# mheinz757/AgglomerationMultigrid1D

Hardware: AMD Instinct MI355X
Metric: fine_level_dof_updates_per_s_per_vcycle (higher is better)
Workload: dtype f64; 1 GPU; config 3/4 hierarchy: V(3,3) cycle, alpha=2/3, DG p=3 n=2^24 -> AggDG pAgg=1 4:1 -> 2:1 -> 2:1 (4 levels), uniform mesh, Neumann/Dirichlet, CDir=1000n (north-star 1-vs-8-GPU size; config 3's own 2^22 in config3_2p22); fine_dofs=67108864, nPre=3, nPost=3, parallelism=single GPU

## Files before the change

### agglomerationmultigrid1d_amd/_lib.py

```python
import ctypes
import os
from ctypes import POINTER, c_char_p, c_double, c_int, c_int32, c_int64, c_void_p

_HERE = os.path.dirname(os.path.abspath(__file__))
LIB_PATH = os.environ.get("AGGMG_HIP_LIB") or os.path.join(_HERE, "libaggmg_hip.so")

AGGMG_OK = 0
ERR_ARGUMENT, ERR_DIMENSION, ERR_SINGULAR, ERR_HIP, ERR_UNSUPPORTED = -1, -2, -3, -4, -5
OP_STIFFNESS, OP_TRANSFER = 0, 1
OPT_SYMMETRIC_PACKING = 1
OPT_COARSE_CHUNK_LOG2 = 2
OPT_DETECT_CHAIN = 3
OPT_PAIR_LEVELS = 4
OPT_MG_CHECKPOINT = 5
OPT_SYMMETRIC_RESIDUAL = 6
OPT_OPERATOR_DICTIONARY = 7
OPT_ELEMENT_THREADS = 8
OPT_PAIR_ELEMENT_THREADS = 9
OPT_REPLAY_PRESMOOTH = 10
OPT_PATCH_MULTI = 11
OPT_CHAIN_MULTI = 12
OPT_ELEMENT_RECORDS_LDS = 13
OPT_PATCH_SCHWARZ_MULTI = 14
PROFILE_NTAGS = 256
KIND_FUSED_DOWN, KIND_FUSED_UP, KIND_SMOOTH, KIND_RESIDUAL, KIND_RESTRICT, KIND_PROLONG, \
    KIND_JACOBI, KIND_BLOCK_APPLY, KIND_COARSE, KIND_FUSED_MID = range(10)
KIND_REPLAY_DOWN, KIND_REPLAY_UP = 10, 11
KIND_NAMES = ["fused_down", "fused_up", "smooth", "residual", "restrict", "prolong", "jacobi",
              "block_apply", "coarse", "fused_mid"]
COARSE_HOST_BANDED, COARSE_DEVICE_CR, COARSE_AUTO, COARSE_EXTERNAL = 0, 1, 2, 3
COARSE_DEVICE_CHAIN = 4
RESTRICT_EXPLICIT, RESTRICT_PRECONDITIONED = 0, 1
RESTRICT_PRECONDITIONED_MAX_ELEMS = 1 << 21
LEVEL_GENERIC, LEVEL_FUSED_BTD, LEVEL_FUSED_CHAIN, LEVEL_COARSEST = 0, 1, 2, 3
MAX_SWEEP_WEIGHTS = 8
FGMRES_MAX_RESTART = 64
RCCL_ID_BYTES = 128
DIST_X0_GHOSTS_VALID, DIST_OVERLAP_NEXT, DIST_GRAPH = 1, 2, 4
ALLGATHER_FN = ctypes.CFUNCTYPE(c_int, c_void_p, c_void_p, c_void_p, c_int64, c_void_p)
SENDRECV_FN = ctypes.CFUNCTYPE(c_int, c_void_p, c_int, POINTER(c_int), POINTER(c_int), POINTER(c_void_p), POINTER(c_int64),
                               c_void_p)
LEVEL_KIND_NAMES = ["generic", "fused_btd", "fused_chain", "coarsest"]


class AggmgError(RuntimeError):
    status = None


class ArgumentError(AggmgError, ValueError):
    status = ERR_ARGUMENT


class DimensionMismatch(AggmgError, ValueError):
    status = ERR_DIMENSION


class SingularException(AggmgError, ArithmeticError):
    status = ERR_SINGULAR


class HipError(AggmgError):
    status = ERR_HIP


class UnsupportedError(AggmgError):
    status = ERR_UNSUPPORTED


_ERR = {c.status: c for c in (ArgumentError, DimensionMismatch, SingularException, HipError,
                              UnsupportedError)}

_P = c_void_p
_PD = POINTER(c_double)
SYMBOLS = {
    "aggmg_create": (c_int, [c_int, POINTER(_P)]),
    "aggmg_destroy": (c_int, [_P]),
    "aggmg_last_error": (c_char_p, [_P]),
    "aggmg_set_stream": (c_int, [_P, _P]),
    "aggmg_reset_stream": (c_int, [_P]),
    "aggmg_synchronize": (c_int, [_P]),
    "aggmg_set_option": (c_int, [_P, c_int, c_int]),
    "aggmg_element_thread_launches": (c_int, [_P, POINTER(c_int64)]),
    "aggmg_pair_element_thread_launches": (c_int, [_P, POINTER(c_int64)]),
    "aggmg_replay_launches": (c_int, [_P, POINTER(c_int64)]),
    "aggmg_element_record_lds_launches": (c_int, [_P, POINTER(c_int64)]),
    "aggmg_element_record_lds_cap": (c_int, [_P, POINTER(c_int), POINTER(c_int)]),
    "aggmg_element_record_pack": (c_int, [c_int, _P, _P, _P, _P, _P, _P, c_int, _P, POINTER(c_int)]),
    "aggmg_patch_multi_launches": (c_int, [_P, POINTER(c_int64)]),
    "aggmg_patch_schwarz_multi_launches": (c_int, [_P, POINTER(c_int64)]),
    "aggmg_chain_multi_launches": (c_int, [_P, POINTER(c_int64)]),
    "aggmg_chain_multi_tile_plan": (c_int, [c_int, c_int, c_int, c_int, c_int, POINTER(c_int), POINTER(c_int), POINTER(c_int),
                                            POINTER(c_int), POINTER(c_int)]),
    "aggmg_dev_alloc": (c_int, [_P, c_int64, POINTER(_P)]),
    "aggmg_dev_free": (c_int, [_P, _P]),
    "aggmg_memcpy_h2d": (c_int, [_P, _P, _P, c_int64]),
    "aggmg_memcpy_d2h": (c_int, [_P, _P, _P, c_int64]),
    "aggmg_csc_upload": (c_int, [_P, c_int64, c_int64, POINTER(c_int64), POINTER(c_int64), _PD,
                                 c_int, c_int, POINTER(_P)]),
    "aggmg_op_free": (c_int, [_P, _P]),
    "aggmg_op_shape": (c_int, [_P, _P, POINTER(c_int64), POINTER(c_int64), POINTER(c_int64)]),
    "aggmg_op_download": (c_int, [_P, _P, c_int, POINTER(c_int32), POINTER(c_int32), _PD]),
    "aggmg_op_release_host": (c_int, [_P, _P]),
    "aggmg_bd_sp_apply": (c_int, [_P, _P, _P, c_int, POINTER(_P)]),
    "aggmg_sp_matmul": (c_int, [_P, _P, _P, c_int, POINTER(_P)]),
    "aggmg_sp_sub": (c_int, [_P, _P, _P, c_int, POINTER(_P)]),
    "aggmg_op_transpose": (c_int, [_P, _P, c_int, POINTER(_P)]),
    "aggmg_op_download_csc": (c_int, [_P, _P, POINTER(c_int32), POINTER(c_int32), _PD]),
    "aggmg_smoother_download_blocks": (c_int, [_P, _P, _PD]),
    "aggmg_debug_device_memory": (c_int, [POINTER(c_int64), POINTER(c_int64)]),
    "aggmg_debug_scan_counts": (c_int, [_P, POINTER(c_int32), c_int64, POINTER(c_int64)]),
    "aggmg_debug_stream_copy": (c_int, [_P, _P, _P, c_int64, c_int, c_int, POINTER(c_double)]),
    "aggmg_blockjacobi_setup": (c_int, [_P, _P, c_int64, c_int64, POINTER(c_int64), c_int, c_int,
                                        POINTER(_P)]),
    "aggmg_blockdiag_setup": (c_int, [_P, c_int64, c_int64, _PD, c_int, POINTER(_P)]),
    "aggmg_patch_schwarz_setup": (c_int, [_P, _P, c_int64, c_int64, c_int, c_int, POINTER(_P)]),
    "aggmg_smoother_patch_info": (c_int, [_P, _P, POINTER(c_int), POINTER(c_int), POINTER(c_int)]),
    "aggmg_smoother_patch_dictionary": (c_int, [_P, _P, POINTER(c_int)]),
    "aggmg_patch_tile_plan": (c_int, [c_int, c_int, POINTER(c_int), POINTER(c_int), POINTER(c_int)]),
    "aggmg_patch_gs_setup": (c_int, [_P, _P, c_int64, c_int64, POINTER(_P)]),
    "aggmg_smoother_patch_kind": (c_int, [_P, _P, POINTER(c_int)]),
    "aggmg_patch_gs_tile_plan": (c_int, [c_int, c_int, POINTER(c_int), POINTER(c_int), POINTER(c_int), POINTER(c_int)]),
    "aggmg_patch_gs_multi_tile_plan": (c_int, [c_int, c_int, c_int, POINTER(c_int), POINTER(c_int), POINTER(c_int),
                                               POINTER(c_int)]),
    "aggmg_patch_schwarz_multi_tile_plan": (c_int, [c_int, c_int, c_int, POINTER(c_int), POINTER(c_int), POINTER(c_int),
                                                    POINTER(c_int)]),
    "aggmg_jacobi_setup": (c_int, [_P, _P, POINTER(_P)]),
    "aggmg_jacobi_setup_elements": (c_int, [_P, _P, c_int64, c_int64, POINTER(c_int64), c_int, POINTER(_P)]),
    "aggmg_smoother_free": (c_int, [_P, _P]),
    "aggmg_smoother_apply": (c_int, [_P, _P, _PD, c_int64, c_int64, c_double, _PD]),
    "aggmg_smoother_is_structured": (c_int, [_P, _P, POINTER(c_int)]),
    "aggmg_smooth": (c_int, [_P, _P, _P, _PD, _PD, c_double, c_int]),
    "aggmg_residual": (c_int, [_P, _P, _PD, _PD, _PD]),
    "aggmg_restrict": (c_int, [_P, _P, _PD, _PD]),
    "aggmg_prolong_add": (c_int, [_P, _P, _PD, _PD]),
    "aggmg_smooth_dev": (c_int, [_P, _P, _P, _P, _P, c_double, c_int, _P]),
    "aggmg_smooth_weighted_dev": (c_int, [_P, _P, _P, _P, _P, _PD, c_int, _P]),
    "aggmg_smooth_multi_dev": (c_int, [_P, _P, _P, _P, _P, c_int64, c_int64, _PD, c_int, c_int, _P]),
    "aggmg_residual_dev": (c_int, [_P, _P, _P, _P, _P]),
    "aggmg_restrict_dev": (c_int, [_P, _P, _P, _P]),
    "aggmg_prolong_add_dev": (c_int, [_P, _P, _P, _P]),
    "aggmg_hier_create": (c_int, [_P, c_int, POINTER(_P), POINTER(_P), POINTER(_P), c_int,
                                  POINTER(_P)]),
    "aggmg_hier_free": (c_int, [_P, _P]),
    "aggmg_vcycle": (c_int, [_P, _P, _PD, _PD, c_int, c_int, c_double, _PD]),
    "aggmg_vcycle_dev": (c_int, [_P, _P, _P, _P, c_int, c_int, c_double, _P]),
    "aggmg_vcycle_multi_dev": (c_int, [_P, _P, _P, _P, c_int64, c_int64, c_int, c_int, c_double, _P]),
    "aggmg_hier_coarse_solve_multi_dev": (c_int, [_P, _P, _P, c_int64, c_int64, _P]),
    "aggmg_hier_multi_info": (c_int, [_P, _P, c_int64, c_int, c_int, POINTER(c_int), POINTER(c_int)]),
    "aggmg_vcycles_dev": (c_int, [_P, _P, _P, _P, c_int, c_int, c_int, c_double, _P]),
    "aggmg_hier_set_restriction": (c_int, [_P, _P, c_int]),
    "aggmg_hier_get_restriction": (c_int, [_P, _P, POINTER(c_int)]),
    "aggmg_vcycle_down_dev": (c_int, [_P, _P, _P, _P, c_int, c_double]),
    "aggmg_vcycle_up_dev": (c_int, [_P, _P, _P, c_int, c_double, _P]),
    "aggmg_vcycle_up_coarse_dev": (c_int, [_P, _P, _P, c_int, c_double, c_int, c_int64, c_int64]),
    "aggmg_vcycle_up_split_dev": (c_int, [_P, _P, _P, c_int, c_double, _P, c_int64, c_int64, c_int]),
    "aggmg_vcycle_up_split_ok": (c_int, [_P, _P, c_int, POINTER(c_int)]),
    "aggmg_hier_coarse_buffers": (c_int, [_P, _P, POINTER(_P), POINTER(_P), POINTER(c_int64)]),
    "aggmg_coarse_plan": (c_int, [_P, _P, POINTER(c_int), POINTER(c_int64), POINTER(c_int), POINTER(c_int64)]),
    "aggmg_coarse_chunk_forward_dev": (c_int, [_P, _P, _P, c_int64, c_int64, _P, _P]),
    "aggmg_coarse_boundary_solve_dev": (c_int, [_P, _P, _P, _P, _P]),
    "aggmg_coarse_chunk_backward_dev": (c_int, [_P, _P, _P, c_int64, c_int64, _P, _P]),
    "aggmg_hier_level_kind": (c_int, [_P, _P, c_int, POINTER(c_int)]),
    "aggmg_host_register": (c_int, [_P, _P, c_int64]),
    "aggmg_host_unregister": (c_int, [_P, _P]),
    "aggmg_host_alloc": (c_int, [_P, c_int64, POINTER(_P)]),
    "aggmg_host_free": (c_int, [_P, _P]),
    "aggmg_hier_level_paired": (c_int, [_P, _P, c_int, c_int, POINTER(c_int)]),
    "aggmg_hier_level_paired_up": (c_int, [_P, _P, c_int, c_int, POINTER(c_int)]),
    "aggmg_hier_level_sym_residual": (c_int, [_P, _P, c_int, POINTER(c_int)]),
    "aggmg_hier_level_dictionary": (c_int, [_P, _P, c_int, POINTER(c_int)]),
# ... 91 lines not shown
```

### agglomerationmultigrid1d_amd/api.py

```python
import ctypes

import numpy as np
import scipy.sparse as sp
import scipy.sparse.linalg as spla

from . import _lib
from ._lib import (ArgumentError, DimensionMismatch, check)

_PD = ctypes.POINTER(ctypes.c_double)
_PI64 = ctypes.POINTER(ctypes.c_int64)


def _f64(x):
    return np.ascontiguousarray(x, dtype=np.float64)


def _pd(a):
    return a.ctypes.data_as(_PD)


def device_memory():
    n, b = ctypes.c_int64(), ctypes.c_int64()
    check(_lib.load().aggmg_debug_device_memory(ctypes.byref(n), ctypes.byref(b)), None)
    return n.value, b.value


class Context:

    def __init__(self, device=0):
        self.lib = _lib.load()
        h = ctypes.c_void_p()
        check(self.lib.aggmg_create(int(device), ctypes.byref(h)), None)
        self.handle = h
        self.device = int(device)

    def close(self):
        if getattr(self, "handle", None):
            self.lib.aggmg_destroy(self.handle)
            self.handle = None

    def __del__(self):
        try:
            self.close()
        except Exception:
            pass

    def check(self, status):
        check(status, self.handle)

    def synchronize(self):
        self.check(self.lib.aggmg_synchronize(self.handle))

    def set_option(self, option, value):
        self.check(self.lib.aggmg_set_option(self.handle, int(option), int(value)))
        self.__dict__.setdefault("_options", {})[int(option)] = int(value)

    def element_thread_launches(self):
        n = ctypes.c_int64(0)
        self.check(self.lib.aggmg_element_thread_launches(self.handle, ctypes.byref(n)))
        return int(n.value)

    def pair_element_thread_launches(self):
        n = ctypes.c_int64(0)
        self.check(self.lib.aggmg_pair_element_thread_launches(self.handle, ctypes.byref(n)))
        return int(n.value)

    def replay_launches(self):
        n = ctypes.c_int64(0)
        self.check(self.lib.aggmg_replay_launches(self.handle, ctypes.byref(n)))
        return int(n.value)

    def element_record_lds_launches(self):
        n = ctypes.c_int64(0)
        self.check(self.lib.aggmg_element_record_lds_launches(self.handle, ctypes.byref(n)))
        return int(n.value)

    def element_record_lds_cap(self):
        c, m = ctypes.c_int(0), ctypes.c_int(0)
        self.check(self.lib.aggmg_element_record_lds_cap(self.handle, ctypes.byref(c), ctypes.byref(m)))
        return int(c.value), int(m.value)

    def patch_multi_launches(self):
        n = ctypes.c_int64(0)
        self.check(self.lib.aggmg_patch_multi_launches(self.handle, ctypes.byref(n)))
        return int(n.value)

    def patch_schwarz_multi_launches(self):
        n = ctypes.c_int64(0)
        self.check(self.lib.aggmg_patch_schwarz_multi_launches(self.handle, ctypes.byref(n)))
        return int(n.value)

    def chain_multi_launches(self):
        n = ctypes.c_int64(0)
        self.check(self.lib.aggmg_chain_multi_launches(self.handle, ctypes.byref(n)))
        return int(n.value)

    def option(self, option, default):
        return self.__dict__.get("_options", {}).get(int(option), default)

    def set_stream(self, hip_stream):
        self.check(self.lib.aggmg_set_stream(self.handle, ctypes.c_void_p(hip_stream or None)))

    def reset_stream(self):
        self.check(self.lib.aggmg_reset_stream(self.handle))

    def alloc(self, n):
        return DeviceVector(self, n)

    def to_device(self, x):
        x = _f64(x)
        v = DeviceVector(self, x.size)
        v.upload(x)
        return v

    def pin(self, x):
        x = np.asarray(x)
        if x.dtype != np.float64 or not x.flags["C_CONTIGUOUS"]:
            raise ArgumentError("Context.pin: a C-contiguous float64 array")
        self.check(self.lib.aggmg_host_register(self.handle, ctypes.c_void_p(x.ctypes.data), x.nbytes))
        self._pinned = getattr(self, "_pinned", {})
        self._pinned[x.ctypes.data] = x
        return x

    def unpin(self, x):
        self.check(self.lib.aggmg_host_unregister(self.handle, ctypes.c_void_p(x.ctypes.data)))
        getattr(self, "_pinned", {}).pop(x.ctypes.data, None)

    def pinned_empty(self, n):
        p = ctypes.c_void_p()
        self.check(self.lib.aggmg_host_alloc(self.handle, int(n) * 8, ctypes.byref(p)))
        buf = (ctypes.c_double * int(n)).from_address(p.value)
        return np.frombuffer(buf, dtype=np.float64, count=int(n))

    def dot_cols(self, X, Y, n=None, ncols=None, ld=None):
        n, ncols, ld = _cols_shape("dot_cols", X, n, ncols, ld)
        if isinstance(Y, DeviceMatrix) and Y.shape != (n, ncols):
            raise DimensionMismatch("dot_cols: X and Y differ in shape")
        out = np.zeros(max(1, int(ncols)))
        self.check(self.lib.aggmg_dot_cols_dev(self.handle, _ptr(X), _ptr(Y), int(n), int(ncols), int(ld), _pd(out)))
        return out

    def norm2_cols(self, X, n=None, ncols=None, ld=None):
        n, ncols, ld = _cols_shape("norm2_cols", X, n, ncols, ld)
        out = np.zeros(max(1, int(ncols)))
        self.check(self.lib.aggmg_norm2_cols_dev(self.handle, _ptr(X), int(n), int(ncols), int(ld), _pd(out)))
        return out

    def multi_dot(self, V, w, n=None, nvec=None, ld=None):
        n, nvec, ld = _cols_shape("multi_dot", V, n, nvec, ld)
        if isinstance(w, DeviceVector) and w.n < n:
            raise DimensionMismatch("multi_dot: w is shorter than the columns of V")
        out = np.zeros(max(1, int(nvec)))
        self.check(self.lib.aggmg_multi_dot_dev(self.handle, _ptr(V), int(n), int(nvec), int(ld), _ptr(w), _pd(out)))
        return out

    def multi_axpy_norm(self, V, coef, w, n=None, nvec=None, ld=None, norm=True):
        n, nvec, ld = _cols_shape("multi_axpy_norm", V, n, nvec, ld)
        if isinstance(w, DeviceVector) and w.n < n:
            raise DimensionMismatch("multi_axpy_norm: w is shorter than the columns of V")
        c = _f64(coef).ravel()
        if c.size != nvec:
            raise DimensionMismatch("multi_axpy_norm: one coefficient per column of V")
# ... 937 lines not shown

    def can_split_up(self, nPost=3):
        ok = ctypes.c_int(0)
        c = self.ctx
        c.check(c.lib.aggmg_vcycle_up_split_ok(c.handle, self.handle, int(nPost), ctypes.byref(ok)))
        return bool(ok.value)

    def set_restriction(self, mode):
        c = self.ctx
        c.check(c.lib.aggmg_hier_set_restriction(c.handle, self.handle, int(mode)))

    def set_sweep_weights(self, level, pre, post=None):
        pre = np.ascontiguousarray(np.atleast_1d(np.asarray(pre, dtype=np.float64)))
        post = pre[::-1].copy() if post is None else np.ascontiguousarray(np.atleast_1d(np.asarray(post, dtype=np.float64)))
        if pre.ndim != 1 or post.ndim != 1:
            raise ArgumentError("set_sweep_weights: pre and post are sequences of numbers")
        c = self.ctx
        c.check(c.lib.aggmg_hier_set_sweep_weights(c.handle, self.handle, int(level), _pd(pre), pre.size, _pd(post), post.size))

    def clear_sweep_weights(self, level=None):
        c = self.ctx
        for k in (range(self.nlevels - 1) if level is None else [int(level)]):
            c.check(c.lib.aggmg_hier_set_sweep_weights(c.handle, self.handle, k, None, 0, None, 0))

    def sweep_weights(self, level):
        pre, post = np.zeros(_lib.MAX_SWEEP_WEIGHTS), np.zeros(_lib.MAX_SWEEP_WEIGHTS)
        npre, npost = ctypes.c_int(0), ctypes.c_int(0)
        c = self.ctx
        c.check(c.lib.aggmg_hier_get_sweep_weights(c.handle, self.handle, int(level), _pd(pre), ctypes.byref(npre), _pd(post),
                                                   ctypes.byref(npost)))
        if npre.value + npost.value == 0:
            return None
        return pre[:npre.value].copy(), post[:npost.value].copy()

    def estimate_lambda_max(self, level, iters=40, v0=None):
        c = self.ctx
        keep = None
        if v0 is not None and isinstance(v0, (np.ndarray, list, tuple)):
            keep = c.to_device(v0)
            v0 = keep
        lam = ctypes.c_double(0.0)
        try:
            c.check(c.lib.aggmg_hier_estimate_lambda_max(c.handle, self.handle, int(level), None if v0 is None else _ptr(v0),
                                                         int(iters), ctypes.byref(lam)))
        finally:
            if keep is not None:
                keep.free()
        return lam.value

    def set_chebyshev_smoothing(self, levels=(0,), degree=3, ratio=10.0, iters=40):
        out = {}
        for k in levels:
            lam = self.estimate_lambda_max(k, iters=iters)
            self.set_sweep_weights(k, chebyshev_weights(lam, degree=degree, ratio=ratio))
            out[int(k)] = lam
        return out

    def get_restriction(self):
        v = ctypes.c_int(0)
        self.ctx.check(self.ctx.lib.aggmg_hier_get_restriction(self.ctx.handle, self.handle, ctypes.byref(v)))
        return v.value

    def coarse_buffers(self):
        r, s_, n = ctypes.c_void_p(), ctypes.c_void_p(), ctypes.c_int64(0)
        self.ctx.check(self.ctx.lib.aggmg_hier_coarse_buffers(self.ctx.handle, self.handle, ctypes.byref(r),
                                                              ctypes.byref(s_), ctypes.byref(n)))
        return r.value, s_.value, n.value

    def coarse_info(self):
        a, b, c = ctypes.c_int(0), ctypes.c_int(0), ctypes.c_double(0.0)
        self.ctx.check(self.ctx.lib.aggmg_hier_coarse_info(self.ctx.handle, self.handle, ctypes.byref(a),
                                                           ctypes.byref(b), ctypes.byref(c)))
        e = ctypes.c_double(0.0)
        self.ctx.check(self.ctx.lib.aggmg_hier_coarse_probe(self.ctx.handle, self.handle, ctypes.byref(e)))
        k, nb = ctypes.c_int(0), ctypes.c_int64(0)
        self.ctx.check(self.ctx.lib.aggmg_hier_coarse_tail(self.ctx.handle, self.handle, ctypes.byref(k), ctypes.byref(nb)))
        on, cm, cb = ctypes.c_int(0), ctypes.c_int(0), ctypes.c_int64(0)
        self.ctx.check(self.ctx.lib.aggmg_hier_coarse_chain(self.ctx.handle, self.handle, ctypes.byref(on), ctypes.byref(cm),
                                                            ctypes.byref(cb)))
        return dict(on_device=bool(a.value), block_size=b.value, cond_est=c.value, probe_backward_error=e.value,
                    tail=("none", "cyclic reduction", "parallel cyclic reduction")[k.value], tail_blocks=nb.value,
                    order="element chain" if on.value else "operator")

    def last_coarse_ms(self):
        ms = ctypes.c_double(0.0)
        self.ctx.check(self.ctx.lib.aggmg_hier_last_coarse_ms(self.ctx.handle, self.handle, ctypes.byref(ms)))
        return ms.value

    def free(self):
        if getattr(self, "handle", None) and self.ctx.handle:
            self.ctx.lib.aggmg_hier_free(self.ctx.handle, self.handle)
        self.handle = None

    def __del__(self):
        try:
            self.free()
        except Exception:
            pass


def multigrid_v_cycle(H, x0, b, nPre=3, nPost=3, alpha=2.0 / 3.0, out=None):
    if not isinstance(nPre, (int, np.integer)) or not isinstance(nPost, (int, np.integer)):
        raise TypeError("nPre / nPost must be integers (nPre::Integer, src/solvers.jl:20)")
    if isinstance(b, DeviceMatrix) or (not isinstance(b, DeviceVector) and np.ndim(b) == 2):
        return _multigrid_v_cycle_multi(H, x0, b, int(nPre), int(nPost), float(alpha))
    if x0 is None and isinstance(b, DeviceVector):
        out = H.ctx.alloc(b.n)
        H.vcycle_dev(None, b, out, int(nPre), int(nPost), float(alpha))
        return out
    if isinstance(x0, DeviceVector) and isinstance(b, DeviceVector):
        N = H._ops[0].shape[0]
        if x0.n != N or b.n != N:
            raise DimensionMismatch("multigrid_v_cycle: x0 / b do not match the fine operator")
        out = H.ctx.alloc(N)
        H.vcycle_dev(x0, b, out, int(nPre), int(nPost), float(alpha))
        return out
    x0 = None if x0 is None else _f64(x0)
    b = _f64(b)
    N = H._ops[0].shape[0]
    if (x0 is not None and x0.shape != (N,)) or b.shape != (N,):
        raise DimensionMismatch("multigrid_v_cycle: x0 / b do not match the fine operator")
    if out is None:
        out = np.empty(N)
    elif not (isinstance(out, np.ndarray) and out.dtype == np.float64 and out.shape == (N,) and out.flags["C_CONTIGUOUS"]):
        raise DimensionMismatch("multigrid_v_cycle: out must be a contiguous float64 array of the fine operator's size")
    elif (x0 is not None and np.shares_memory(out, x0)) or np.shares_memory(out, b):
        raise ArgumentError("multigrid_v_cycle: out must not alias x0 or b (they are not modified)")
    c = H.ctx
    c.check(c.lib.aggmg_vcycle(c.handle, H.handle, None if x0 is None else _pd(x0), _pd(b), int(nPre), int(nPost), float(alpha),
                               _pd(out)))
    return out


def _multigrid_v_cycle_multi(H, X0, B, nPre, nPost, alpha):
    N = H._ops[0].shape[0]
    c = H.ctx
    if isinstance(B, DeviceMatrix):
        if X0 is not None and not isinstance(X0, DeviceMatrix):
            raise ArgumentError("multigrid_v_cycle: X0 must be a DeviceMatrix (or None) when B is one")
        K = B.k
        if B.n != N or (X0 is not None and X0.shape != B.shape):
            raise DimensionMismatch("multigrid_v_cycle: X0 / B do not match (N, K) of the fine operator")
        X = DeviceMatrix(c, N, K)
        H.vcycle_multi_dev(X0, B, X, K, N, nPre, nPost, alpha)
        return X
    if isinstance(X0, (DeviceVector, DeviceMatrix)):
        raise ArgumentError("multigrid_v_cycle: X0 is on the device but B is a host array")
    B = np.asarray(B, dtype=np.float64)
    if B.ndim != 2 or B.shape[0] != N:
        raise DimensionMismatch(f"multigrid_v_cycle: B has shape {B.shape}, expected ({N}, K)")
    K = B.shape[1]
    if K < 1:
        raise ArgumentError("multigrid_v_cycle: B has no columns")
    if X0 is not None:
        X0 = np.asarray(X0, dtype=np.float64)
        if X0.shape != B.shape:
            raise DimensionMismatch(f"multigrid_v_cycle: X0 has shape {X0.shape}, B {B.shape}")
    dB = DeviceMatrix(c, N, K)
    dB.upload(B)
    dX0 = None
    if X0 is not None:
        dX0 = DeviceMatrix(c, N, K)
        dX0.upload(X0)
    dX = DeviceMatrix(c, N, K)
    H.vcycle_multi_dev(dX0, dB, dX, K, N, nPre, nPost, alpha)
    return dX.download()
# ... 374 lines not shown
```

### agglomerationmultigrid1d_amd/csrc/aggmg_hip.hip

```cpp
#include "internal.hpp"
#include "multi_kernels.hpp"
#include "multi_solve_kernels.hpp"
#include "pair_kernels.hpp"
#include "patch_kernels.hpp"
#include "patch_multi_kernels.hpp"
#include "patch_schwarz_multi_kernels.hpp"
#include "elem_kernels.hpp"
#include "pair_elem_kernels.hpp"
#include "krylov_kernels.hpp"
#include "host_gmres.hpp"
#include "host_gmres_cols.hpp"

extern "C" const char* aggmg_version(void) { return "aggmg_hip 0.1 gfx950 fp64"; }

extern "C" int aggmg_debug_device_memory(int64_t* live_allocations, int64_t* live_bytes) {
  if (live_allocations) *live_allocations = DevMemLive::allocations.load();
  if (live_bytes) *live_bytes = DevMemLive::bytes.load();
  return AGGMG_OK;
}

extern "C" int aggmg_create(int device_id, aggmg_ctx** out) {
  if (!out) return fail(nullptr, AGGMG_ERR_ARGUMENT, "aggmg_create: out is NULL");
  *out = nullptr;
  int ndev = 0;
// ... 70 lines not shown
    }
  return fail(ctx, AGGMG_ERR_ARGUMENT, "aggmg_host_unregister: not a range registered with this context");
}

extern "C" int aggmg_host_alloc(aggmg_ctx* ctx, int64_t nbytes, void** out) {
  if (!ctx || !out) return AGGMG_ERR_ARGUMENT;
  if (nbytes < 0) return fail(ctx, AGGMG_ERR_ARGUMENT, "aggmg_host_alloc: negative size");
  HIPCHK(hipSetDevice(ctx->device));
  void* p = nullptr;
  HIPCHK(hipHostMalloc(&p, (size_t)std::max<int64_t>(nbytes, 8), hipHostMallocDefault));
  ctx->pinned.push_back({static_cast<char*>(p), (size_t)std::max<int64_t>(nbytes, 8), true});
  *out = p;
  return AGGMG_OK;
}

extern "C" int aggmg_host_free(aggmg_ctx* ctx, void* ptr) {
  if (!ctx) return AGGMG_ERR_ARGUMENT;
  if (!ptr) return AGGMG_OK;
  for (size_t i = 0; i < ctx->pinned.size(); ++i)
    if (ctx->pinned[i].base == static_cast<char*>(ptr) && ctx->pinned[i].owned) {
      HIPCHK(hipStreamSynchronize(ctx->stream));
      HIPCHK(hipHostFree(ptr));
      ctx->pinned.erase(ctx->pinned.begin() + (long)i);
      return AGGMG_OK;
    }
  return fail(ctx, AGGMG_ERR_ARGUMENT, "aggmg_host_free: not an allocation of this context");
}

extern "C" const char* aggmg_last_error(aggmg_ctx* ctx) {
  return ctx ? ctx->err.c_str() : g_create_error.c_str();
}

extern "C" int aggmg_set_stream(aggmg_ctx* ctx, void* hip_stream) {
  if (!ctx) return AGGMG_ERR_ARGUMENT;
  ctx->stream = (hipStream_t)hip_stream;
  return AGGMG_OK;
}

extern "C" int aggmg_reset_stream(aggmg_ctx* ctx) {
  if (!ctx) return AGGMG_ERR_ARGUMENT;
  ctx->stream = ctx->own_stream;
  return AGGMG_OK;
}

extern "C" int aggmg_set_option(aggmg_ctx* ctx, int option, int value) {
  if (!ctx) return AGGMG_ERR_ARGUMENT;
  switch (option) {
    case AGGMG_OPT_SYMMETRIC_PACKING:
      ctx->sym_packing = value != 0;
      return AGGMG_OK;
    case AGGMG_OPT_COARSE_CHUNK_LOG2:
      if (value < 1 || value > kCrMaxStageLevels)
        return fail(ctx, AGGMG_ERR_ARGUMENT, "aggmg_set_option: AGGMG_OPT_COARSE_CHUNK_LOG2 takes 1 .. 12");
      ctx->cr_max_q = value;
      return AGGMG_OK;
    case AGGMG_OPT_DETECT_CHAIN:
      ctx->detect_chain = value != 0;
      return AGGMG_OK;
    case AGGMG_OPT_PAIR_LEVELS:
      ctx->pair_levels = value != 0;
      return AGGMG_OK;
    case AGGMG_OPT_MG_CHECKPOINT:
      ctx->mg_checkpoint = value != 0;
      return AGGMG_OK;
    case AGGMG_OPT_SYMMETRIC_RESIDUAL:
      ctx->sym_residual = value != 0;
      return AGGMG_OK;
    case AGGMG_OPT_OPERATOR_DICTIONARY:
      ctx->op_dict = value != 0;
      return AGGMG_OK;
    case AGGMG_OPT_ELEMENT_THREADS:
      ctx->elem_threads = value != 0;
      return AGGMG_OK;
    case AGGMG_OPT_PAIR_ELEMENT_THREADS:
      ctx->pair_elem_threads = value != 0;
      return AGGMG_OK;
    case AGGMG_OPT_REPLAY_PRESMOOTH:
      ctx->replay_presmooth = value != 0;
      return AGGMG_OK;
    case AGGMG_OPT_ELEMENT_RECORDS_LDS:
      if (value < 0 || value > kElemRecMaxClasses)
        return fail(ctx, AGGMG_ERR_ARGUMENT, "aggmg_set_option: AGGMG_OPT_ELEMENT_RECORDS_LDS takes 0 .. " + std::to_string(kElemRecMaxClasses));
      ctx->elem_rec_cap = value;
      return AGGMG_OK;
    case AGGMG_OPT_PATCH_MULTI:
      ctx->patch_multi = value != 0;
      return AGGMG_OK;
    case AGGMG_OPT_CHAIN_MULTI:
      ctx->chain_multi = value != 0;
      return AGGMG_OK;
    case AGGMG_OPT_PATCH_SCHWARZ_MULTI:
      ctx->patch_schwarz_multi = value != 0;
      return AGGMG_OK;
  }
  return fail(ctx, AGGMG_ERR_ARGUMENT, "aggmg_set_option: unknown option");
}

extern "C" int aggmg_synchronize(aggmg_ctx* ctx) {
  if (!ctx) return AGGMG_ERR_ARGUMENT;
  HIPCHK(hipStreamSynchronize(ctx->stream));
  return AGGMG_OK;
}

extern "C" int aggmg_dev_alloc(aggmg_ctx* ctx, int64_t nbytes, void** out) {
  if (!ctx || !out || nbytes < 0) return fail(ctx, AGGMG_ERR_ARGUMENT, "aggmg_dev_alloc: bad argument");
  HIPCHK(hipSetDevice(ctx->device));
  HIPCHK(hipMalloc(out, (size_t)std::max<int64_t>(nbytes, 8)));
  HIPCHK(hipMemsetAsync(*out, 0, (size_t)std::max<int64_t>(nbytes, 8), ctx->stream));
  return AGGMG_OK;
}

extern "C" int aggmg_dev_free(aggmg_ctx* ctx, void* ptr) {
  if (!ctx) return AGGMG_ERR_ARGUMENT;
  if (ptr) {
    HIPCHK(hipStreamSynchronize(ctx->stream));
    HIPCHK(hipFree(ptr));
  }
  return AGGMG_OK;
}

extern "C" int aggmg_memcpy_h2d(aggmg_ctx* ctx, void* dst, const void* src, int64_t nbytes) {
  if (!ctx) return AGGMG_ERR_ARGUMENT;
  HIPCHK(hipMemcpyAsync(dst, src, (size_t)nbytes, hipMemcpyHostToDevice, ctx->stream));
  HIPCHK(hipStreamSynchronize(ctx->stream));
  return AGGMG_OK;
}

extern "C" int aggmg_memcpy_d2h(aggmg_ctx* ctx, void* dst, const void* src, int64_t nbytes) {
  if (!ctx) return AGGMG_ERR_ARGUMENT;
  HIPCHK(hipMemcpyAsync(dst, src, (size_t)nbytes, hipMemcpyDeviceToHost, ctx->stream));
  HIPCHK(hipStreamSynchronize(ctx->stream));
  return AGGMG_OK;
}

extern "C" int aggmg_profile_enable(aggmg_ctx* ctx, int on) {
  if (!ctx) return AGGMG_ERR_ARGUMENT;
  ctx->profiling = on < 0 ? 0 : (on > 2 ? 1 : on);
  return AGGMG_OK;
}

extern "C" int aggmg_profile_collect(aggmg_ctx* ctx, double* total_ms, int64_t* counts) {
  if (!ctx || !total_ms || !counts) return fail(ctx, AGGMG_ERR_ARGUMENT, "aggmg_profile_collect: NULL");
  for (int t = 0; t < AGGMG_PROFILE_NTAGS; ++t) {
    total_ms[t] = 0.0;
    counts[t] = 0;
  }
  HIPCHK(hipStreamSynchronize(ctx->stream));
  for (auto& pe : ctx->prof) {
    float ms = 0.f;
    HIPCHK(hipEventElapsedTime(&ms, pe.a, pe.b));
    total_ms[pe.tag] += ms;
    counts[pe.tag] += 1;
    ctx->ev_pool.push_back(pe.a);
    ctx->ev_pool.push_back(pe.b);
  }
  ctx->prof.clear();
  return AGGMG_OK;
}

extern "C" int aggmg_csc_upload(aggmg_ctx* ctx, int64_t m, int64_t n, const int64_t* colptr,
                                const int64_t* rowval, const double* nzval, int one_based, int kind,
                                aggmg_op** out) {
  if (!ctx || !out || !colptr) return fail(ctx, AGGMG_ERR_ARGUMENT, "aggmg_csc_upload: NULL argument");
  *out = nullptr;
  if (m < 0 || n < 0) return fail(ctx, AGGMG_ERR_ARGUMENT, "aggmg_csc_upload: negative dimension");
  const int64_t base = one_based ? 1 : 0;
// ... 1400 lines not shown
  const CrDev& cr = h->cr;
  std::vector<CrMultiStage> ws;
  CrMultiStage wt;
  cr_multi_layout(cr.st, cr.tail, cr.m, h->crw_cols, &ws, &wt);
  double* const w = h->crw;
  auto at = [&](int64_t stride, int64_t off) -> double* { return stride ? w + off : nullptr; };
  CrRun run;
  run.kc = kc;
  run.st.reserve(ws.size());
  for (const CrMultiStage& W : ws) {
    double* const part = w + W.part_off;
    run.st.push_back({part, part + W.part / 3, part + 2 * (W.part / 3), at(W.stack, W.stack_off), at(W.mid, W.mid_off), W.part,
                      W.stack, W.mid});
  }
  run.tail.mid = at(wt.mid, wt.mid_off);
  run.tail.cs_mid = wt.mid;
  return run;
}

enum CrKind { kCrForward = 0, kCrTail = 1, kCrBackward = 2 };
static CrStageArgs cr_make_args(const CrDev& cr, const CrStagePlan& S, const CrRunStage& R, CrKind kind) {
  CrStageArgs A;
  std::memset(&A, 0, sizeof(A));
#ifdef AGGMG_CR_TRACE
  A.trace = g_cr_trace;
  A.trace_kind = kind;
#endif
  A.q = S.q;
  for (int l = 0; l < S.q; ++l) A.lv[l] = cr.lv[S.l0 + l];
  A.nsteps = S.nsteps;
  for (int s = 0; s <= kCrMaxSteps; ++s) {
    A.step_a[s] = S.step_a[s];
    A.lds_off[s] = S.lds_off[s];
    A.lds_xoff[s] = S.lds_xoff[s];
  }
  A.lds_total = S.lds_total;
  A.n_out = S.n_out;
  A.stack = R.stack;
  A.stack_stride = S.stack_stride;
  A.mid = R.mid;
  for (int s = 0; s <= kCrMaxSteps; ++s) A.mid_off[s] = S.mid_off[s];
  A.tail = kind == kCrTail ? 1 : 0;
  A.lu_last = cr.lu_last;
  A.perm_last = cr.perm_last;
  A.cs_o = A.cs_xq = R.cs_part;
  A.cs_stack = R.cs_stack;
  A.cs_mid = R.cs_mid;
  return A;
}

template <int M>
static void cr_launch_tail(aggmg_ctx* ctx, CrDev& cr, const CrStageArgs& T, size_t tail_lds, const double* d, const double* db,
                           double* x, int kc = 1) {
  if constexpr (M <= 2) {
    if (cr.pcr.valid) {
      PcrArgs P;
      std::memset(&P, 0, sizeof(P));
      P.mult = cr.pcr.mult;
      P.lu = cr.pcr.lu;
      P.perm = cr.pcr.perm;
      P.n = cr.pcr.n;
      P.L = cr.pcr.L;
      P.dstride = T.dstride;
      P.cs_d = T.cs_d;
      P.cs_x = T.cs_x;
#ifdef AGGMG_CR_TRACE
      P.trace = g_cr_trace;
#endif
      const unsigned threads = (unsigned)((cr.pcr.n + 63) / 64 * 64);
      const size_t lds = (size_t)2 * (cr.pcr.n + 1) * M * sizeof(double);
      if (cr.pcr.pre) {
        P.lv0 = cr.lv[cr.tail.l0];
        P.n_full = (int)cr.tail.n_in;
        hipLaunchKernelGGL((cr_pcr_tail_kernel<M, true>), dim3(1, kc), dim3(threads), lds, ctx->stream, P, d, db, x);
      } else {
        hipLaunchKernelGGL((cr_pcr_tail_kernel<M, false>), dim3(1, kc), dim3(threads), lds, ctx->stream, P, d, db, x);
      }
      return;
    }
  }
  hipLaunchKernelGGL((cr_tail_kernel<M>), dim3(1, kc), dim3(kCrThreads), tail_lds, ctx->stream, T, d, db, x);
}

template <int M, bool FUSE_TAIL = false>
static void cr_launch_forward(aggmg_ctx* ctx, const CrStageArgs& A, unsigned grid, int kc, const double* d, const double* db,
                              double* partR, double* partL, const CrStageArgs& T, size_t tail_lds = 0, double* xt = nullptr,
                              unsigned int* ticket = nullptr) {
  hipLaunchKernelGGL((cr_stage_forward_kernel<M, FUSE_TAIL>), dim3(grid, kc), dim3(cr_stage_threads()),
                     std::max((size_t)A.lds_total * sizeof(double), tail_lds), ctx->stream, A, d, db, partR, partL, T, xt, ticket);
}
template <int M>
static void cr_launch_backward(aggmg_ctx* ctx, const CrStageArgs& A, unsigned grid, int kc, const double* d, const double* db,
                               const double* xq, double* x) {
  hipLaunchKernelGGL((cr_stage_backward_kernel<M>), dim3(grid, kc), dim3(cr_stage_threads()), (size_t)A.lds_total * sizeof(double),
                     ctx->stream, A, d, db, xq, x);
}

template <int M>
static int cr_walk(aggmg_ctx* ctx, CrDev& cr, const CrRun& run, int s0, const double* d, const double* db, double* x,
                   int64_t cs_in, int64_t cs_out, int dstride) {
  const int ns = (int)cr.st.size(), kc = run.kc;
  CrStageArgs T = cr_make_args(cr, cr.tail, run.tail, kCrTail);
  const size_t tail_lds = (size_t)cr.tail.lds_total * sizeof(double);
  if (s0 >= ns) {
    T.dstride = dstride;
    T.cs_d = cs_in;
    T.cs_x = cs_out;
    cr_launch_tail<M>(ctx, cr, T, tail_lds, d, db, x, kc);
    HIPCHK(hipGetLastError());
    return AGGMG_OK;
  }
  struct Io {
    const double *d, *db;
    double* x;
    int64_t cs_d, cs_x;
    int dstride;
  };
  auto io = [&](int s) -> Io {
    if (s == s0) return {d, db, x, cs_in, cs_out, dstride};
    const CrRunStage& P = run.st[s - 1];
    return {P.partR, P.partL, P.xq, P.cs_part, P.cs_part, 0};
  };
  const bool fuse_tail = kc == 1 && cr_fuse_tail();
  for (int s = s0; s < ns; ++s) {
    const CrRunStage& R = run.st[s];
    const Io in = io(s);
    CrStageArgs A = cr_make_args(cr, cr.st[s], R, kCrForward);
    A.cs_d = in.cs_d;
    A.dstride = in.dstride;
    const unsigned grid = (unsigned)std::max<int64_t>(A.n_out, 1);
    if (s == ns - 1 && fuse_tail) {
      cr_launch_forward<M, true>(ctx, A, grid, kc, in.d, in.db, R.partR, R.partL, T, tail_lds, R.xq, cr.ticket);
    } else {
      cr_launch_forward<M>(ctx, A, grid, kc, in.d, in.db, R.partR, R.partL, T);
      if (s == ns - 1) {
        T.cs_d = T.cs_x = R.cs_part;
        cr_launch_tail<M>(ctx, cr, T, tail_lds, R.partR, R.partL, R.xq, kc);
      }
    }
  }
  for (int s = ns - 1; s >= s0; --s) {
    const Io in = io(s);
    CrStageArgs A = cr_make_args(cr, cr.st[s], run.st[s], kCrBackward);
    A.cs_d = in.cs_d;
    A.cs_x = in.cs_x;
    A.dstride = in.dstride;
    cr_launch_backward<M>(ctx, A, (unsigned)std::max<int64_t>(A.n_out, 1), kc, in.d, in.db, run.st[s].xq, in.x);
  }
  HIPCHK(hipGetLastError());
  return AGGMG_OK;
}

template <int M>
static int cr_chunks(aggmg_ctx* ctx, CrDev& cr, bool backward, const double* d_owned, int64_t blk_lo, int64_t blk_hi,
                     double* partR, double* partL, const double* xq, double* x_owned, int ostride) {
  const CrStage& S = cr.st[0];
  CrStageArgs A = cr_make_args(cr, S, cr_run_stage(S), backward ? kCrBackward : kCrForward);
  A.ostride = ostride;
  A.c0 = blk_lo >> S.q;
  const int64_t c1 = (blk_hi + ((int64_t)1 << S.q) - 1) >> S.q;
  const unsigned grid = (unsigned)std::max<int64_t>(c1 - A.c0, 0);
  if (!grid) return AGGMG_OK;
  const double* d0 = d_owned - blk_lo * M;
  if (backward) {
    cr_launch_backward<M>(ctx, A, grid, 1, d0, nullptr, xq, x_owned - blk_lo * M);
  } else {
    CrStageArgs T;
    std::memset(&T, 0, sizeof(T));
    cr_launch_forward<M>(ctx, A, grid, 1, d0, nullptr, partR, partL, T);
  }
  HIPCHK(hipGetLastError());
  return AGGMG_OK;
}

template <class F>
static int cr_with_m(aggmg_ctx* ctx, const CrDev& cr, F&& f) {
  int rc = AGGMG_OK;
  if (!with_block_size<cr_form>(cr.m, [&](auto m) { rc = f(m); }))
    return fail(ctx, AGGMG_ERR_UNSUPPORTED, "cyclic reduction block size not instantiated");
  return rc;
}

static int cr_phase(aggmg_ctx* ctx, CrDev& cr, int phase, const double* d_owned, int64_t blk_lo, int64_t blk_hi,
                    double* partR, double* partL, const double* xq, double* x_owned, int pstride = 0) {
  ProfScope ps(ctx, AGGMG_KIND_COARSE, 0);
  return cr_with_m(ctx, cr, [&](auto m) {
    constexpr int M = decltype(m)::value;
    if (phase == 1) return cr_walk<M>(ctx, cr, cr.run, 1, partR, partL, const_cast<double*>(xq), 0, 0, pstride);
    return cr_chunks<M>(ctx, cr, phase == 2, d_owned, blk_lo, blk_hi, partR, partL, xq, x_owned, pstride);
  });
}

static int cr_multi_workspace(aggmg_ctx* ctx, aggmg_hier* h, int64_t cols, bool staging) {
  const CrDev& cr = h->cr;
  if (h->crw_cols < cols) {
    HIPCHK(hipStreamSynchronize(ctx->stream));
    h->crw_cols = 0;
    std::vector<CrMultiStage> st;
    CrMultiStage tail;
    CHECK(h->crw.alloc(ctx, cr_multi_layout(cr.st, cr.tail, cr.m, cols, &st, &tail), true));
    h->crw_cols = cols;
  }
  if (staging && h->crw_stage_cols < cols) {
    HIPCHK(hipStreamSynchronize(ctx->stream));
    h->crw_stage_cols = 0;
    CHECK(h->crw_stage.alloc(ctx, 2 * cols * cr_even(cr.n0 * cr.m), true));
    h->crw_stage_cols = cols;
  }
  return AGGMG_OK;
}

static dim3 cr_cols_grid(int64_t n, int kc) { return dim3((unsigned)((n + kCrThreads - 1) / kCrThreads), kc); }
static void cr_chain_gather(aggmg_ctx* ctx, const CgtDev& g, int64_t n, int kc, const double* B, int64_t ldb, double* d0, int64_t sp) {
  hipLaunchKernelGGL(cr_chain_gather_kernel<kCrThreads>, cr_cols_grid(n, kc), dim3(kCrThreads), 0, ctx->stream, B, ldb,
                     (const int32_t*)g.perm, d0, sp, n);
}
static void cr_chain_scatter(aggmg_ctx* ctx, const CgtDev& g, int kc, const double* x0, int64_t sp, double* X, int64_t ldx) {
  hipLaunchKernelGGL(cr_chain_scatter_kernel<kCrThreads>, cr_cols_grid(g.N, kc), dim3(kCrThreads), 0, ctx->stream, x0, sp,
                     (const int32_t*)g.inv, X, ldx, g.N);
}
static void cr_cols_copy(aggmg_ctx* ctx, int64_t n, int kc, const double* src, int64_t ld_src, double* dst, int64_t ld_dst) {
  hipLaunchKernelGGL(cr_cols_copy_kernel<kCrThreads>, cr_cols_grid(n, kc), dim3(kCrThreads), 0, ctx->stream, src, ld_src, dst, ld_dst, n);
}

template <int M>
static int cr_solve_cols(aggmg_ctx* ctx, aggmg_hier* h, const double* B, int64_t ldb, double* X, int64_t ldx, int kc) {
  CrDev& cr = h->cr;
  const int64_t Npad = cr.n0 * M;
  const bool aligned = kc == 1 || ((((uintptr_t)B | (uintptr_t)X) & 15) == 0 && ldb % 2 == 0 && ldx % 2 == 0);
  const bool overlap = kc == 1 ? B == X : B < X + ((kc - 1) * ldx + cr.N) && X < B + ((kc - 1) * ldb + cr.N);
  const bool direct = !cr.chain && Npad == cr.N && aligned && !overlap;
  if (kc > 1) {
    CHECK(cr_multi_workspace(ctx, h, kc, !direct));
  } else if (!direct && !cr.d0) {
    for (DevArray<double>* p : {&cr.d0, &cr.x0}) CHECK(p->alloc(ctx, Npad));
  }
  const double* d = B;
  double* x = X;
  int64_t cs_in = ldb, cs_out = ldx;
  if (!direct) {
    const int64_t sp = kc == 1 ? 0 : cr_even(Npad);
    double* d0 = kc == 1 ? cr.d0.get() : h->crw_stage.get();
    x = kc == 1 ? cr.x0.get() : h->crw_stage + h->crw_stage_cols * sp;
    if (cr.chain) {
      cr_chain_gather(ctx, *cr.chain, Npad, kc, B, ldb, d0, sp);
    } else if (kc == 1) {
      if (Npad > cr.N) HIPCHK(hipMemsetAsync(d0 + cr.N, 0, (Npad - cr.N) * sizeof(double), ctx->stream));
      HIPCHK(hipMemcpyAsync(d0, B, cr.N * sizeof(double), hipMemcpyDeviceToDevice, ctx->stream));
    } else {
      cr_cols_copy(ctx, cr.N, kc, B, ldb, d0, sp);
    }
    d = d0;
// ... 387 lines not shown
                          int64_t gh_hi = 0) {
  const int n = (int)h->lv.size();
  Level& a = h->lv[k];
  Level& b = h->lv[k + 1];
  Level& c = h->lv[k + 2];
  PairArgs p = pair_args(h, k, nPost);
  const SweepWeights wa = a.damp_post(alpha).launch(nPost), wb = b.damp_post(alpha).launch(nPost);
  PairTilePlan plan = pair_up_plan(nPost, p.ab.rho, kPairTEA, kPairTEB);
  if (plan.own <= 0) return fail(ctx, AGGMG_ERR_UNSUPPORTED, "internal: paired tile too small");
  p.hb = plan.hb;
  p.own = plan.own;
  p.te_a = plan.te_a;
  p.te_b = plan.te_b;
  p.rhs_a = a.rhs;
  p.rhs_b_in = b.rhs;
  p.ua_in = a.u[0];
  p.ub_in = b.u[0];
  p.uc = (k + 2 == n - 1) ? c.u[0] : c.u[1];
  p.u_a = dst;
  p.ub_out = nullptr;
  int64_t ntiles = (p.A.ne + plan.own - 1) / plan.own;
  if (part != 0) {
    pair_up_split(&plan, nPost, p.ab.rho, p.bc.rho, p.A.ne, p.bc.nec, gh_lo, gh_hi);
    if (part == 1) {
      p.tile_split = (int)plan.tA;
      p.tile_skip = plan.all - plan.tA - plan.tB;
      ntiles = plan.tA + plan.tB;
    } else {
      p.tile_skip = plan.tA;
      ntiles = plan.all - plan.tA - plan.tB;
    }
  }
  if (ntiles == 0) return AGGMG_OK;
  const size_t lds = ((size_t)2 * (kPairTEA + 2) * kPairM + (size_t)kPairTEB * 2) * sizeof(double);
  PairDict d;
  const bool dict = part == 0 && pair_dictionary(p, d, a, b);
  PairElemDict ed;
  const bool elem = dict && pair_element_threads(ctx, p, ed, a, b, pair_up_plan(nPost, p.ab.rho, kPairElemTEA, kPairElemTEB));
  ProfScope ps(ctx, AGGMG_KIND_FUSED_UP, k);
  if (elem) {
    ntiles = (p.A.ne + p.own - 1) / p.own;
    hipLaunchKernelGGL((btd_pair_up_elem_kernel<kPairElemThreads>), dim3((unsigned)ntiles), dim3(kPairElemThreads),
                       pair_elem_lds_bytes(ed.nca, ed.ncb), ctx->stream, p, wa, wb, ed);
    ++ctx->pair_elem_launches;
  } else if (dict)
    hipLaunchKernelGGL((btd_pair_up_dict_kernel<kPairM, kPairNSA, kPairNSB, kThreads>), dim3((unsigned)ntiles), dim3(kThreads),
                       lds, ctx->stream, p, wa, wb, d);
  else
    hipLaunchKernelGGL((btd_pair_up_kernel<kPairM, kPairNSA, kPairNSB, kThreads>), dim3((unsigned)ntiles), dim3(kThreads), lds,
                       ctx->stream, p, wa, wb);
  HIPCHK(hipGetLastError());
  return AGGMG_OK;
}

extern "C" int aggmg_hier_level_paired(aggmg_ctx* ctx, const aggmg_hier* h, int level, int nsweeps, int* paired) {
  if (!ctx || !h || !paired) return fail(ctx, AGGMG_ERR_ARGUMENT, "aggmg_hier_level_paired: NULL argument");
  *paired = pair_ok(ctx, h, level, nsweeps, false) ? 1 : 0;
  return AGGMG_OK;
}

extern "C" int aggmg_hier_level_paired_up(aggmg_ctx* ctx, const aggmg_hier* h, int level, int nsweeps, int* paired) {
  if (!ctx || !h || !paired) return fail(ctx, AGGMG_ERR_ARGUMENT, "aggmg_hier_level_paired_up: NULL argument");
  *paired = pair_ok(ctx, h, level, nsweeps, true) ? 1 : 0;
  return AGGMG_OK;
}

extern "C" int aggmg_hier_level_sym_residual(aggmg_ctx* ctx, const aggmg_hier* h, int level, int* on) {
  if (!ctx || !h || !on) return fail(ctx, AGGMG_ERR_ARGUMENT, "aggmg_hier_level_sym_residual: NULL argument");
  if (level < 0 || level >= (int)h->lv.size()) return fail(ctx, AGGMG_ERR_ARGUMENT, "aggmg_hier_level_sym_residual: level out of range");
  const Level& l = h->lv[level];
  *on = (l.S && l.S->btd && l.S->btd->dup) ? 1 : 0;
  return AGGMG_OK;
}

extern "C" int aggmg_element_thread_launches(aggmg_ctx* ctx, int64_t* count) {
  if (!ctx || !count) return fail(ctx, AGGMG_ERR_ARGUMENT, "aggmg_element_thread_launches: NULL argument");
  *count = ctx->elem_launches;
  return AGGMG_OK;
}

extern "C" int aggmg_pair_element_thread_launches(aggmg_ctx* ctx, int64_t* count) {
  if (!ctx || !count) return fail(ctx, AGGMG_ERR_ARGUMENT, "aggmg_pair_element_thread_launches: NULL argument");
  *count = ctx->pair_elem_launches;
  return AGGMG_OK;
}

extern "C" int aggmg_element_record_lds_launches(aggmg_ctx* ctx, int64_t* count) {
  if (!ctx || !count) return fail(ctx, AGGMG_ERR_ARGUMENT, "aggmg_element_record_lds_launches: NULL argument");
  *count = ctx->elem_rec_launches;
  return AGGMG_OK;
}

extern "C" int aggmg_element_record_lds_cap(aggmg_ctx* ctx, int* cap, int* max_cap) {
  if (!ctx || !cap) return fail(ctx, AGGMG_ERR_ARGUMENT, "aggmg_element_record_lds_cap: NULL argument");
  *cap = ctx->elem_rec_cap;
  if (max_cap) *max_cap = kElemRecMaxClasses;
  return AGGMG_OK;
}

extern "C" int aggmg_element_record_pack(int nclasses, const double* bsym, const double* qrow, const double* qmir, const double* dup,
                                         const uint32_t* corr, const double* lf, int lf_unit, double* rec, int* words) {
  if (words) *words = kElemRecWords;
  if (nclasses < 0 || (nclasses > 0 && (!bsym || !qrow || !qmir || !lf || !rec || !dup != !corr))) return AGGMG_ERR_ARGUMENT;
  elem_record_pack(nclasses, bsym, qrow, qmir, dup, corr, lf, lf_unit != 0, rec);
  return AGGMG_OK;
}

extern "C" int aggmg_replay_launches(aggmg_ctx* ctx, int64_t* count) {
  if (!ctx || !count) return fail(ctx, AGGMG_ERR_ARGUMENT, "aggmg_replay_launches: NULL argument");
  *count = ctx->replay_launches;
  return AGGMG_OK;
}

extern "C" int aggmg_hier_level_dictionary(aggmg_ctx* ctx, const aggmg_hier* h, int level, int* nclasses) {
  if (!ctx || !h || !nclasses) return fail(ctx, AGGMG_ERR_ARGUMENT, "aggmg_hier_level_dictionary: NULL argument");
  if (level < 0 || level >= (int)h->lv.size()) return fail(ctx, AGGMG_ERR_ARGUMENT, "aggmg_hier_level_dictionary: level out of range");
  const Level& l = h->lv[level];
  *nclasses = l.dict ? l.dict->nclasses : (l.cdict ? l.cdict->nclasses : (l.pdict ? l.pdict->nclasses : 0));
  return AGGMG_OK;
}

extern "C" int aggmg_hier_set_sweep_weights(aggmg_ctx* ctx, aggmg_hier* h, int level, const double* pre, int npre,
                                            const double* post, int npost) {
  if (!ctx) return AGGMG_ERR_ARGUMENT;
  if (!h) return fail(ctx, AGGMG_ERR_ARGUMENT, "aggmg_hier_set_sweep_weights: NULL argument");
  if (level < 0 || level >= (int)h->lv.size() - 1)
    return fail(ctx, AGGMG_ERR_ARGUMENT, "aggmg_hier_set_sweep_weights: level out of range (the coarsest level is solved, not smoothed)");
  if (npre < 0 || npost < 0 || npre > AGGMG_MAX_SWEEP_WEIGHTS || npost > AGGMG_MAX_SWEEP_WEIGHTS)
    return fail(ctx, AGGMG_ERR_ARGUMENT, "aggmg_hier_set_sweep_weights: between 0 and AGGMG_MAX_SWEEP_WEIGHTS weights per half");
  if ((npre > 0 && !pre) || (npost > 0 && !post)) return fail(ctx, AGGMG_ERR_ARGUMENT, "aggmg_hier_set_sweep_weights: NULL argument");
  for (int i = 0; i < npre; ++i)
    if (!std::isfinite(pre[i])) return fail(ctx, AGGMG_ERR_ARGUMENT, "aggmg_hier_set_sweep_weights: weight is not finite");
  for (int i = 0; i < npost; ++i)
    if (!std::isfinite(post[i])) return fail(ctx, AGGMG_ERR_ARGUMENT, "aggmg_hier_set_sweep_weights: weight is not finite");
  Level& l = h->lv[level];
  l.scheduled = npre + npost > 0;
  l.w_pre.assign(pre, pre + npre);
  l.w_post.assign(post, post + npost);
  l.w_mid = l.w_post;
  l.w_mid.insert(l.w_mid.end(), l.w_pre.begin(), l.w_pre.end());
  l.w_replay = l.w_pre;
  l.w_replay.insert(l.w_replay.end(), l.w_post.begin(), l.w_post.end());
  return AGGMG_OK;
}

extern "C" int aggmg_hier_get_sweep_weights(aggmg_ctx* ctx, const aggmg_hier* h, int level, double* pre, int* npre,
                                            double* post, int* npost) {
  if (!ctx) return AGGMG_ERR_ARGUMENT;
  if (!h || !pre || !npre || !post || !npost) return fail(ctx, AGGMG_ERR_ARGUMENT, "aggmg_hier_get_sweep_weights: NULL argument");
  if (level < 0 || level >= (int)h->lv.size() - 1)
    return fail(ctx, AGGMG_ERR_ARGUMENT, "aggmg_hier_get_sweep_weights: level out of range");
  const Level& l = h->lv[level];
  *npre = (int)l.w_pre.size();
  *npost = (int)l.w_post.size();
  std::copy(l.w_pre.begin(), l.w_pre.end(), pre);
  std::copy(l.w_post.begin(), l.w_post.end(), post);
  return AGGMG_OK;
}

static int schedule_check(aggmg_ctx* ctx, const aggmg_hier* h, int nPre, int nPost, int k_first = 0) {
  for (int k = k_first; k < (int)h->lv.size() - 1; ++k) {
    const Level& l = h->lv[k];
    if (!l.scheduled) continue;
    if ((nPre >= 0 && nPre != (int)l.w_pre.size()) || (nPost >= 0 && nPost != (int)l.w_post.size()))
      return fail(ctx, AGGMG_ERR_ARGUMENT, "level " + std::to_string(k) + " has a sweep-weight schedule of " +
                  std::to_string(l.w_pre.size()) + " pre- and " + std::to_string(l.w_post.size()) +
// ... 2530 lines not shown
```

### agglomerationmultigrid1d_amd/csrc/cr_kernels.hpp

```cpp
#pragma once
#include <hip/hip_runtime.h>
#include <stdint.h>

#include "host_plan.hpp"

namespace aggmg {

constexpr int kCrThreads = 256;
#ifndef CR_WAVES_ATTR
#define CR_WAVES_ATTR
#endif

struct CrLevel {
  const double* fe;
  const double* fo;
  const double* lu;
  const int32_t* perm;
  int64_t n, n_even, n_odd;
};

template <int M>
struct CrRadix {
  static constexpr int Q = M <= 4 ? 3 : 2;
};
// ... 319 lines not shown
        double& r = v[(CrOff<QS, I>::blocks + 2 * jj + 1) * M + e];
        double& g = mid[(CrMidOff<QS, I>::blocks + jj) * M + e];
        if constexpr (STORE) g = r; else r = g;
      }
    cr_mid_move<M, QS, I + 1, STORE>(mid, v);
  }
}

template <int M, int QS>
struct CrSubFactorsB {
  double fo[CrOddOff<QS, QS>::rows][2 * M * M];
  double lu[CrOddOff<QS, QS>::rows][M * M];
  int32_t perm[CrOddOff<QS, QS>::rows][M];
};

template <int M, int QS, int I>
__device__ __forceinline__ void cr_pre_load_b(const CrLevel* lv, int64_t b, CrSubFactorsB<M, QS>& F) {
  if constexpr (I < QS) {
    const CrLevel& L = lv[I];
    constexpr int NB1 = 1 << (QS - I - 1);
    const int64_t tlo1 = b << (QS - I - 1);
#pragma unroll
    for (int jj = 0; jj < NB1; ++jj) {
      int64_t idx = tlo1 + jj;
      if (idx > L.n_odd - 1) idx = L.n_odd - 1;
      const double* lu = L.lu + idx * (M * M);
      const int32_t* pm = L.perm + idx * M;
      constexpr int o = CrOddOff<QS, I>::rows;
      cr_load_pair<M>(L.fo + idx * (2 * M * M), F.fo[o + jj]);
      if constexpr (M == 2) {
        const double2 t0 = reinterpret_cast<const double2*>(lu)[0], t1 = reinterpret_cast<const double2*>(lu)[1];
        const int2 pp = *reinterpret_cast<const int2*>(pm);
        F.lu[o + jj][0] = t0.x, F.lu[o + jj][1] = t0.y, F.lu[o + jj][2] = t1.x, F.lu[o + jj][3] = t1.y;
        F.perm[o + jj][0] = pp.x, F.perm[o + jj][1] = pp.y;
      } else {
#pragma unroll
        for (int k = 0; k < M * M; ++k) F.lu[o + jj][k] = lu[k];
#pragma unroll
        for (int k = 0; k < M; ++k) F.perm[o + jj][k] = pm[k];
      }
    }
    cr_pre_load_b<M, QS, I + 1>(lv, b, F);
  }
}

template <int M, int QS, int I>
__device__ __forceinline__ void cr_loc_bwd_pre(const CrLevel* lv, const CrSubFactorsB<M, QS>& F, int64_t b, double* v) {
  if constexpr (I >= 0) {
    const CrLevel& L = lv[I];
    constexpr int NB1 = 1 << (QS - I - 1);
    const int64_t tlo = b << (QS - I);
    double* d = v + CrOff<QS, I>::blocks * M;
    const double* xn = v + CrOff<QS, I + 1>::blocks * M;
#pragma unroll
    for (int jj = 0; jj < NB1; ++jj) {
      const int64_t r = tlo + 2 * jj + 1;
      const double* ac = F.fo[CrOddOff<QS, I>::rows + jj];
      double rhs[M], x[M];
      const bool has_next = r + 1 < L.n;
      double xr[M];
#pragma unroll
      for (int k = 0; k < M; ++k) xr[k] = has_next ? xn[(jj + 1) * M + k] : 0.0;
#pragma unroll
      for (int i = 0; i < M; ++i) {
        double s = d[(2 * jj + 1) * M + i];
#pragma unroll
        for (int k = 0; k < M; ++k) s -= ac[i * M + k] * xn[jj * M + k];
#pragma unroll
        for (int k = 0; k < M; ++k) s -= ac[M * M + i * M + k] * xr[k];
        rhs[i] = s;
      }
      cr_lu_solve_reg<M>(F.lu[CrOddOff<QS, I>::rows + jj], F.perm[CrOddOff<QS, I>::rows + jj], rhs, x);
#pragma unroll
      for (int e = 0; e < M; ++e) d[(2 * jj + 1) * M + e] = x[e];
    }
#pragma unroll
    for (int jj = 0; jj <= NB1; ++jj)
#pragma unroll
      for (int e = 0; e < M; ++e) d[(2 * jj) * M + e] = xn[jj * M + e];
    cr_loc_bwd_pre<M, QS, I - 1>(lv, F, b, v);
  }
}

struct CrStepGeom {
  int a, a1;
  int64_t lo_in, lo_out;
  int64_t n_in, n_out;
  int nb;
};

template <int QS>
__device__ __forceinline__ CrStepGeom cr_step_geom(const CrStageArgs& A, int s, int64_t c, bool wg_shared) {
  CrStepGeom g;
  g.a = A.step_a[s];
  g.a1 = g.a + QS;
  g.lo_in = c << (A.q - g.a);
  g.lo_out = c << (A.q - g.a1);
  g.n_in = cr_level_n(A, g.a);
  g.n_out = cr_level_n(A, g.a1);
  int64_t hi_out = (c + 1) << (A.q - g.a1);
  if (hi_out > g.n_out - 1) hi_out = g.n_out - 1;
  g.nb = (int)(hi_out - g.lo_out + 1) - (wg_shared ? 1 : 0);
  return g;
}

template <int M, int QS>
__device__ __forceinline__ void cr_loc_load(const CrStageArgs& A, int s, const CrStepGeom& g, int64_t b,
                                            const double* __restrict__ d0, const double* __restrict__ d0b,
                                            const double* sh, double* v, int64_t& thi, bool& tshared,
                                            bool carry_rb) {
  constexpr int NB = 1 << QS;
  const int64_t tlo = b << QS;
  thi = (b + 1) << QS;
  tshared = thi <= g.n_in - 1;
  if (!tshared) thi = g.n_in - 1;
  if (s == 0) {
    const int ds = A.dstride ? A.dstride : M;
    if (tshared && ds == M) {
      const double2* p = reinterpret_cast<const double2*>(d0 + tlo * M);
      if (d0b) {
        const double2* pb = reinterpret_cast<const double2*>(d0b + tlo * M);
#pragma unroll
        for (int k = 0; k < NB * M / 2; ++k) {
          const double2 t = p[k], u = pb[k];
          v[2 * k] = t.x + u.x;
          v[2 * k + 1] = t.y + u.y;
        }
      } else {
#pragma unroll
        for (int k = 0; k < NB * M / 2; ++k) {
          const double2 t = p[k];
          v[2 * k] = t.x;
          v[2 * k + 1] = t.y;
        }
      }
#pragma unroll
      for (int e = 0; e < M; ++e) v[NB * M + e] = 0.0;
    } else {
#pragma unroll
      for (int k = 0; k <= NB; ++k) {
        const int64_t gk = tlo + k <= thi ? tlo + k : thi;
#pragma unroll
        for (int e = 0; e < M; ++e) v[k * M + e] = d0[gk * ds + e];
      }
      if (d0b) {
#pragma unroll
        for (int k = 0; k <= NB; ++k) {
          const int64_t gk = tlo + k <= thi ? tlo + k : thi;
#pragma unroll
          for (int e = 0; e < M; ++e) v[k * M + e] += d0b[gk * ds + e];
        }
      }
#pragma unroll
      for (int k = 0; k <= NB; ++k) {
        const bool ok = tlo + k <= thi && !(tshared && k == NB);
#pragma unroll
        for (int e = 0; e < M; ++e) v[k * M + e] = ok ? v[k * M + e] : 0.0;
      }
    }
  } else {
    const int cnt = ((1 << (A.q - g.a)) + 1) * M;
    const double* R = sh + A.lds_off[s];
    const double* Lp = R + cnt;
#pragma unroll
    for (int k = 0; k <= NB; ++k) {
      const bool ok = tlo + k <= thi && !(tshared && k == NB && !carry_rb);
      const int idx = (int)((tlo + k <= thi ? tlo + k : thi) - g.lo_in) * M;
#pragma unroll
      for (int e = 0; e < M; ++e) {
        const double x = R[idx + e] + Lp[idx + e];
        v[k * M + e] = ok ? x : 0.0;
      }
    }
  }
}

template <int M, int QS>
__device__ __forceinline__ void cr_step_forward(const CrStageArgs& A, int s, int64_t c, bool wg_shared,
                                                const double* __restrict__ d0, const double* __restrict__ d0b,
                                                double* sh) {
  const CrStepGeom g = cr_step_geom<QS>(A, s, c, wg_shared);
  const int cnt_out = ((1 << (A.q - g.a1)) + 1) * M;
  double* Rout = sh + A.lds_off[s + 1];
  double* Lout = Rout + cnt_out;
  for (int i = threadIdx.x; i < g.nb; i += blockDim.x) {
    const int64_t b = g.lo_out + i;
    double v[CrOff<QS, QS + 1>::blocks * M];
    int64_t thi;
    bool tshared;
    if constexpr (M <= 2) {
      CrSubFactors<M, QS> F;
      cr_pre_load<M, QS, 0>(&A.lv[g.a], b, F);
      __builtin_amdgcn_sched_barrier(0);
      cr_loc_load<M, QS>(A, s, g, b, d0, d0b, sh, v, thi, tshared, wg_shared && s > 0 && i == g.nb - 1);
#ifdef AGGMG_CR_TRACE
      if (s == 0 && i == (int)threadIdx.x) CR_STAMP_WAIT(A, 2);
#endif
      cr_loc_fwd_pre<M, QS, 0>(&A.lv[g.a], F, b, v);
    } else {
      cr_loc_load<M, QS>(A, s, g, b, d0, d0b, sh, v, thi, tshared, wg_shared && s > 0 && i == g.nb - 1);
      cr_loc_fwd<M, QS, 0>(&A.lv[g.a], b, v);
    }
    if constexpr (QS >= 2) cr_mid_move<M, QS, 1, true>(cr_col_mid(A) + A.mid_off[s] + b * (cr_mid_blocks<QS>() * M), v);
    const double* top = v + CrOff<QS, QS>::blocks * M;
#ifdef AGGMG_CR_TRACE
    if (s == 0 && i == (int)threadIdx.x) {
      double t0 = top[0];
      asm volatile("" : "+v"(t0));
      CR_STAMP_WAIT(A, 3);
    }
#endif
#pragma unroll
    for (int e = 0; e < M; ++e) Rout[i * M + e] = top[e];
    if (b + 1 <= g.n_out - 1) {
#pragma unroll
      for (int e = 0; e < M; ++e) Lout[(i + 1) * M + e] = top[M + e];
    }
  }
}

template <int M, int QS>
__device__ __forceinline__ void cr_step_backward(const CrStageArgs& A, int s, int64_t c, bool wg_shared,
                                                 const double* __restrict__ d0, const double* __restrict__ d0b,
                                                 const double* xtop, int64_t xtop_lo, double* xout, int64_t xout_lo,
                                                 double* sh) {
  constexpr int NB = 1 << QS;
  const CrStepGeom g = cr_step_geom<QS>(A, s, c, wg_shared);
  for (int i = threadIdx.x; i < g.nb; i += blockDim.x) {
    const int64_t b = g.lo_out + i;
    double v[CrOff<QS, QS + 1>::blocks * M];
    int64_t thi;
    bool tshared;
    double* top = v + CrOff<QS, QS>::blocks * M;
    const bool has_right = b + 1 <= g.n_out - 1;
    const int64_t br = has_right ? b + 1 : b;
    if constexpr (M <= 2) {
      CrSubFactorsB<M, QS> F;
      cr_pre_load_b<M, QS, 0>(&A.lv[g.a], b, F);
      __builtin_amdgcn_sched_barrier(0);
      cr_loc_load<M, QS>(A, s, g, b, d0, d0b, sh, v, thi, tshared, wg_shared && s > 0 && i == g.nb - 1);
      if constexpr (QS >= 2) cr_mid_move<M, QS, 1, false>(cr_col_mid(A) + A.mid_off[s] + b * (cr_mid_blocks<QS>() * M), v);
#pragma unroll
      for (int e = 0; e < M; ++e) {
        top[e] = xtop[(b - xtop_lo) * M + e];
        const double xr = xtop[(br - xtop_lo) * M + e];
        top[M + e] = has_right ? xr : 0.0;
      }
      cr_loc_bwd_pre<M, QS, QS - 1>(&A.lv[g.a], F, b, v);
    } else {
      cr_loc_load<M, QS>(A, s, g, b, d0, d0b, sh, v, thi, tshared, wg_shared && s > 0 && i == g.nb - 1);
      if constexpr (QS >= 2) cr_mid_move<M, QS, 1, false>(cr_col_mid(A) + A.mid_off[s] + b * (cr_mid_blocks<QS>() * M), v);
#pragma unroll
      for (int e = 0; e < M; ++e) {
        top[e] = xtop[(b - xtop_lo) * M + e];
        const double xr = xtop[(br - xtop_lo) * M + e];
        top[M + e] = has_right ? xr : 0.0;
      }
      cr_loc_bwd<M, QS, QS - 1>(&A.lv[g.a], b, v);
    }
    const int64_t tlo = b << QS;
    double* o = xout + (tlo - xout_lo) * M;
    if (tshared && s == 0) {
      double2* o2 = reinterpret_cast<double2*>(o);
#pragma unroll
      for (int k = 0; k < NB * M / 2; ++k) o2[k] = make_double2(v[2 * k], v[2 * k + 1]);
    } else {
      const bool write_rb = tshared && s > 0 && i == g.nb - 1;
#pragma unroll
      for (int k = 0; k <= NB; ++k) {
        const bool w = k < NB ? (tlo + k <= thi) : (tshared ? write_rb : (tlo + k <= thi));
        if (w) {
#pragma unroll
          for (int e = 0; e < M; ++e) o[k * M + e] = v[k * M + e];
        }
      }
    }
  }
}

template <int M>
__device__ __forceinline__ void cr_forward_steps(const CrStageArgs& A, int64_t c, bool wg_shared,
                                                 const double* __restrict__ d0, const double* __restrict__ d0b,
                                                 double* sh) {
  constexpr int Q = CrRadix<M>::Q;
  for (int s = 0; s < A.nsteps; ++s) {
    const int qs = A.step_a[s + 1] - A.step_a[s];
    if (qs == 1) {
      cr_step_forward<M, 1>(A, s, c, wg_shared, d0, d0b, sh);
    } else if (qs == 2) {
      cr_step_forward<M, 2>(A, s, c, wg_shared, d0, d0b, sh);
    } else {
      if constexpr (Q >= 3) cr_step_forward<M, 3>(A, s, c, wg_shared, d0, d0b, sh);
    }
    __syncthreads();
    CR_STAMP(A, 4 + s);
  }
}

template <int M>
__device__ __forceinline__ void cr_backward_steps(const CrStageArgs& A, int64_t c, bool wg_shared,
                                                  const double* __restrict__ d0, const double* __restrict__ d0b,
                                                  const double* __restrict__ xq, double* __restrict__ x0, double* sh) {
  constexpr int Q = CrRadix<M>::Q;
  for (int s = A.nsteps - 1; s >= 0; --s) {
    const int a = A.step_a[s], a1 = A.step_a[s + 1];
    const int qs = a1 - a;
    const bool top_global = xq && s == A.nsteps - 1;
    const double* xtop = top_global ? xq : sh + A.lds_xoff[s + 1];
    const int64_t xtop_lo = top_global ? 0 : (c << (A.q - a1));
    double* xout = s ? sh + A.lds_xoff[s] : x0;
    const int64_t xout_lo = s ? (c << (A.q - a)) : 0;
    if (qs == 1) {
      cr_step_backward<M, 1>(A, s, c, wg_shared, d0, d0b, xtop, xtop_lo, xout, xout_lo, sh);
    } else if (qs == 2) {
      cr_step_backward<M, 2>(A, s, c, wg_shared, d0, d0b, xtop, xtop_lo, xout, xout_lo, sh);
    } else {
      if constexpr (Q >= 3) cr_step_backward<M, 3>(A, s, c, wg_shared, d0, d0b, xtop, xtop_lo, xout, xout_lo, sh);
    }
    __syncthreads();
    CR_STAMP(A, 8 + s);
  }
}

template <int M>
__device__ __forceinline__ void cr_tail_body(const CrStageArgs& T, const double* __restrict__ d0,
                                             const double* __restrict__ d0b, double* __restrict__ x0, double* sh) {
  CR_TRACE_BEGIN();
  CR_STAMP(T, 0);
  for (int t = threadIdx.x; t < T.lds_total; t += blockDim.x) sh[t] = 0.0;
  __syncthreads();
  CR_STAMP(T, 1);
  if (T.nsteps == 0) {
    if (threadIdx.x == 0) {
      double r[M], y[M];
#pragma unroll
      for (int e = 0; e < M; ++e) r[e] = d0b ? d0[e] + d0b[e] : d0[e];
      cr_lu_solve_reg<M>(T.lu_last, T.perm_last, r, y);
#pragma unroll
      for (int e = 0; e < M; ++e) x0[e] = y[e];
    }
    return;
  }
  cr_forward_steps<M>(T, 0, false, d0, d0b, sh);
  if (threadIdx.x == 0) {
    const double* R = sh + T.lds_off[T.nsteps];
    double r[M], y[M];
#pragma unroll
    for (int e = 0; e < M; ++e) r[e] = R[e] + R[2 * M + e];
    cr_lu_solve_reg<M>(T.lu_last, T.perm_last, r, y);
    double* X = sh + T.lds_xoff[T.nsteps];
#pragma unroll
    for (int e = 0; e < M; ++e) X[e] = y[e];
  }
  __syncthreads();
  CR_STAMP(T, 12);
  cr_backward_steps<M>(T, 0, false, d0, d0b, nullptr, x0, sh);
  CR_STAMP_WAIT(T, 15);
  CR_TRACE_FLUSH(T);
}

template <int M>
__global__ __launch_bounds__(kCrThreads) CR_WAVES_ATTR void cr_tail_kernel(CrStageArgs T, const double* __restrict__ d0,
                                                             const double* __restrict__ d0b,
                                                             double* __restrict__ x0) {
  extern __shared__ double sh[];
  const int64_t col = blockIdx.y;
  d0 += col * T.cs_d;
  if (d0b) d0b += col * T.cs_d;
  x0 += col * T.cs_x;
  cr_tail_body<M>(T, d0, d0b, x0, sh);
}

template <int M, bool FUSE_TAIL>
__global__ __launch_bounds__(kCrThreads) CR_WAVES_ATTR void cr_stage_forward_kernel(CrStageArgs A, const double* __restrict__ d0,
                                                                      const double* __restrict__ d0b, double* partR,
                                                                      double* partL, CrStageArgs T, double* xq,
                                                                      unsigned int* ticket) {
  extern __shared__ double sh[];
  __shared__ unsigned int s_ticket;
  const int64_t c = A.c0 + blockIdx.x;
  const int64_t col = blockIdx.y;
  d0 += col * A.cs_d;
  if (d0b) d0b += col * A.cs_d;
  partR += col * A.cs_o;
  partL += col * A.cs_o;
  const bool wg_shared = ((c + 1) << A.q) <= A.lv[0].n - 1;
  CR_TRACE_BEGIN();
  CR_STAMP(A, 0);
  for (int t = threadIdx.x; t < A.lds_total; t += blockDim.x) sh[t] = 0.0;
  __syncthreads();
  CR_STAMP(A, 1);
  cr_forward_steps<M>(A, c, wg_shared, d0, d0b, sh);
  {
    const double* R = sh + A.lds_off[A.nsteps];
    if (threadIdx.x < M) {
      const int os = A.ostride ? A.ostride : M;
      partR[c * os + threadIdx.x] = R[threadIdx.x];
      if (c + 1 <= A.n_out - 1) partL[(c + 1) * os + threadIdx.x] = R[2 * M + M + threadIdx.x];
    }
  }
  if (A.stack) {
    double* st = A.stack + col * A.cs_stack + c * (int64_t)A.stack_stride;
    int o = 0;
    for (int s = 1; s < A.nsteps; ++s) {
      const int cnt = ((1 << (A.q - A.step_a[s])) + 1) * M;
      const double* R = sh + A.lds_off[s];
      for (int t = threadIdx.x; t < cnt; t += blockDim.x) st[o + t] = R[t] + R[cnt + t];
      o += cnt;
    }
  }
  CR_STAMP_WAIT(A, 15);
  CR_TRACE_FLUSH(A);
  if constexpr (FUSE_TAIL) {
    __threadfence();
    __syncthreads();
    if (threadIdx.x == 0) s_ticket = atomicAdd(ticket, 1u);
    __syncthreads();
    if (s_ticket != gridDim.x - 1) return;
    __threadfence();
    cr_tail_body<M>(T, partR, partL, xq, sh);
    if (threadIdx.x == 0) *ticket = 0u;
  }
}

template <int M>
__global__ __launch_bounds__(kCrThreads) CR_WAVES_ATTR void cr_stage_backward_kernel(CrStageArgs A, const double* __restrict__ d0,
                                                                       const double* __restrict__ d0b,
                                                                       const double* __restrict__ xq,
                                                                       double* __restrict__ x0) {
  extern __shared__ double sh[];
  const int64_t c = A.c0 + blockIdx.x;
  const int64_t col = blockIdx.y;
  d0 += col * A.cs_d;
  if (d0b) d0b += col * A.cs_d;
  xq += col * A.cs_xq;
  x0 += col * A.cs_x;
  const bool wg_shared = ((c + 1) << A.q) <= A.lv[0].n - 1;
  CR_TRACE_BEGIN();
  CR_STAMP(A, 0);
  for (int t = threadIdx.x; t < A.lds_total; t += blockDim.x) sh[t] = 0.0;
  __syncthreads();
  CR_STAMP(A, 1);
  if (A.nsteps > 1) {
    if (A.stack) {
      const double* st = A.stack + col * A.cs_stack + c * (int64_t)A.stack_stride;
      int o = 0;
      for (int s = 1; s < A.nsteps; ++s) {
        const int cnt = ((1 << (A.q - A.step_a[s])) + 1) * M;
        double* R = sh + A.lds_off[s];
        for (int t = threadIdx.x; t < cnt; t += blockDim.x) R[t] = st[o + t];
        o += cnt;
      }
      __syncthreads();
      CR_STAMP(A, 2);
    } else {
      cr_forward_steps<M>(A, c, wg_shared, d0, d0b, sh);
    }
  }
  cr_backward_steps<M>(A, c, wg_shared, d0, d0b, xq, x0, sh);
  CR_STAMP_WAIT(A, 15);
  CR_TRACE_FLUSH(A);
}

constexpr int kPcrMaxLevels = 9;
struct PcrArgs {
  const double* mult;
  const double* lu;
  const int32_t* perm;
  int n, L;
  int dstride;
  int64_t cs_d, cs_x;
  CrLevel lv0;
  int n_full;
#ifdef AGGMG_CR_TRACE
  unsigned long long* trace;
#endif
};

template <int M, bool PRE>
__global__ __launch_bounds__(512) void cr_pcr_tail_kernel(PcrArgs P, const double* __restrict__ d0,
                                                           const double* __restrict__ d0b, double* __restrict__ x0) {
  extern __shared__ double sh[];
  constexpr int W = 2 * M * M, D = kPcrMaxLevels;
  const int i = threadIdx.x, n = P.n;
  d0 += (int64_t)blockIdx.y * P.cs_d;
  if (d0b) d0b += (int64_t)blockIdx.y * P.cs_d;
  x0 += (int64_t)blockIdx.y * P.cs_x;
  const bool act = i < n;
  const int ic = act ? i : n - 1;
#ifdef AGGMG_CR_TRACE
  unsigned long long t_in = 0;
  if (i == 0) t_in = wall_clock64();
#endif
  double f[D][W];
#pragma unroll
  for (int j = 0; j < D; ++j) {
    const int lv = j < P.L ? j : 0;
    const double* src = P.mult + ((int64_t)lv * n + ic) * W;
#pragma unroll
    for (int k = 0; k < W / 2; ++k) {
      const double2 t = reinterpret_cast<const double2*>(src)[k];
      f[j][2 * k] = t.x, f[j][2 * k + 1] = t.y;
    }
  }
  double luf[M * M];
  int32_t pf[M];
#pragma unroll
  for (int k = 0; k < M * M; ++k) luf[k] = P.lu[(int64_t)ic * (M * M) + k];
#pragma unroll
  for (int k = 0; k < M; ++k) pf[k] = P.perm[(int64_t)ic * M + k];
  const int ds = P.dstride ? P.dstride : M;
  double v[M];
  double fe0[PRE ? W : 1], fo0[PRE ? W : 1], lu0[PRE ? M * M : 1], dodd[M];
  int32_t p0[M];
  bool has_odd = false;
  if constexpr (PRE) {
    const int nf = P.n_full;
    const int64_t io = 2 * ic + 1 < nf ? ic : (P.lv0.n_odd > 0 ? P.lv0.n_odd - 1 : 0);
    has_odd = act && 2 * i + 1 < nf;
    cr_load_pair<M>(P.lv0.fe + (int64_t)ic * W, fe0);
    cr_load_pair<M>(P.lv0.fo + io * W, fo0);
#pragma unroll
    for (int k = 0; k < M * M; ++k) lu0[k] = P.lv0.lu[io * (M * M) + k];
#pragma unroll
    for (int k = 0; k < M; ++k) p0[k] = P.lv0.perm[io * M + k];
    const int64_t rl = 2 * ic - 1 >= 0 ? 2 * ic - 1 : 0, rr = 2 * ic + 1 < nf ? 2 * ic + 1 : nf - 1;
    double dl[M], dr[M];
#pragma unroll
    for (int e = 0; e < M; ++e) {
      v[e] = d0[(int64_t)(2 * ic) * ds + e];
      dl[e] = d0[rl * ds + e];
      dr[e] = d0[rr * ds + e];
    }
    if (d0b) {
#pragma unroll
      for (int e = 0; e < M; ++e) {
        v[e] += d0b[(int64_t)(2 * ic) * ds + e];
        dl[e] += d0b[rl * ds + e];
        dr[e] += d0b[rr * ds + e];
      }
    }
#pragma unroll
    for (int e = 0; e < M; ++e) dodd[e] = dr[e];
#pragma unroll
    for (int r = 0; r < M; ++r) {
      double t = v[r];
// ... 124 lines not shown
```

### agglomerationmultigrid1d_amd/csrc/forms.hpp

```cpp
#pragma once
#include <type_traits>
#include <utility>

namespace aggmg {

constexpr int kMaxBlock = 9;

constexpr bool btd_form(int m, bool cmp) { return cmp ? (m >= 2 && m <= 9) : (m >= 1 && m <= 5); }
constexpr bool btd_sym_form(int m, bool cmp) { return cmp ? (m == 2 || m == 4 || m == 8) : (m == 2 || m == 4); }
constexpr bool btd_sres_form(int m, bool cmp) { return cmp && m <= 4 && btd_sym_form(m, cmp); }
constexpr bool patch_form(int m, bool cmp) { return m <= 8 && btd_form(m, cmp); }
constexpr bool multi_form(int m, bool cmp) { return cmp ? (m == 2 || m == 4) : m == 2; }
constexpr bool multi_block_size(int m) { return multi_form(m, true) || multi_form(m, false); }
constexpr bool chain_form(int m) { return m >= 1 && m <= 8; }
constexpr bool chain_dict_form(int m) { return m == 1 || m == 2 || m == 4; }
constexpr bool cr_form(int m) { return m >= 1 && m <= 8; }
constexpr bool invert_form(int m) { return m >= 1 && m <= 8; }
constexpr bool csr_lanes_form(int l) { return l >= 1 && l <= 64 && (l & (l - 1)) == 0; }

constexpr int col_group(int kc, int ceiling = 8) {
  return kc <= 1 ? 1 : (kc <= 2 || ceiling == 2) ? 2 : (kc <= 4 || ceiling == 4) ? 4 : 8;
}
constexpr bool is_col_group(int kb) { return kb >= 1 && kb <= 8 && col_group(kb) == kb; }

template <int M, bool CMP>
struct Form {
  static constexpr int kM = M;
  static constexpr bool kCmp = CMP;
};

template <auto Pred, int M, class F>
bool with_block_size_at(int m, F& f) {
  if constexpr (Pred(M)) {
    if (m == M) {
      f(std::integral_constant<int, M>{});
      return true;
    }
  }
  return false;
}
template <auto Pred, class F, int... I>
bool with_block_size_in(int m, F& f, std::integer_sequence<int, I...>) {
  return (with_block_size_at<Pred, (int)sizeof...(I) - I>(m, f) || ...);
}
template <auto Pred, int Max = kMaxBlock, class F>
bool with_block_size(int m, F&& f) {
  return with_block_size_in<Pred>(m, f, std::make_integer_sequence<int, Max>{});
}

template <auto Pred, int M, bool CMP, class F>
bool with_form_at(int m, bool cmp, F& f) {
  if constexpr (Pred(M, CMP)) {
    if (m == M && cmp == CMP) {
      f(Form<M, CMP>{});
      return true;
    }
  }
  return false;
}
template <auto Pred, class F, int... I>
bool with_form_in(int m, bool cmp, F& f, std::integer_sequence<int, I...>) {
  return ((with_form_at<Pred, I + 1, true>(m, cmp, f) || with_form_at<Pred, I + 1, false>(m, cmp, f)) || ...);
}
template <auto Pred, class F>
bool with_form(int m, bool cmp, F&& f) {
  return with_form_in<Pred>(m, cmp, f, std::make_integer_sequence<int, kMaxBlock>{});
}

template <class F>
void with_col_group(int kc, int ceiling, F&& f) {
  with_block_size<is_col_group, 8>(col_group(kc, ceiling), f);
}
template <class F>
void with_col_group(int kc, F&& f) {
  with_col_group(kc, 8, f);
}

constexpr unsigned form_mask(bool (*pred)(int, bool), bool cmp) {
  unsigned s = 0;
  for (int m = 0; m < 32; ++m) s |= pred(m, cmp) ? 1u << m : 0u;
  return s;
}
constexpr unsigned size_mask(bool (*pred)(int)) {
  unsigned s = 0;
  for (int m = 0; m < 32; ++m) s |= pred(m) ? 1u << m : 0u;
  return s;
}
constexpr int count_bits(unsigned s) { return s ? (int)(s & 1u) + count_bits(s >> 1) : 0; }
constexpr int count_forms(bool (*pred)(int, bool)) { return count_bits(form_mask(pred, true)) + count_bits(form_mask(pred, false)); }

static_assert(form_mask(btd_form, true) == 0b1111111100 && form_mask(btd_form, false) == 0b111110 && count_forms(btd_form) == 13,
              "btd_form: compressed 2..9 and dense 1..5");
static_assert(form_mask(btd_sym_form, true) == 0b100010100 && form_mask(btd_sym_form, false) == 0b10100, "btd_sym_form: compressed 2, 4, 8; dense 2, 4");
static_assert(form_mask(btd_sres_form, true) == 0b10100 && form_mask(btd_sres_form, false) == 0, "btd_sres_form: compressed 2, 4");
static_assert(form_mask(patch_form, true) == 0b111111100 && form_mask(patch_form, false) == 0b111110 && count_forms(patch_form) == 12,
              "patch_form: compressed 2..8 and dense 1..5");
static_assert(form_mask(multi_form, true) == 0b10100 && form_mask(multi_form, false) == 0b100 && count_forms(multi_form) == 3,
              "multi_form: compressed 2, 4; dense 2");
static_assert(size_mask(multi_block_size) == 0b10100, "the K-column lane groups: 2, 4");
static_assert(size_mask(chain_form) == 0b111111110 && size_mask(cr_form) == 0b111111110 && size_mask(invert_form) == 0b111111110,
              "chain_form, cr_form, invert_form: 1..8");
static_assert(size_mask(chain_dict_form) == 0b10110 && count_bits(size_mask(chain_dict_form)) == 3, "chain_dict_form: 1, 2, 4");
static_assert(size_mask(is_col_group) == 0b100010110, "column groups: 1, 2, 4, 8");
static_assert(col_group(1) == 1 && col_group(2) == 2 && col_group(3) == 4 && col_group(4) == 4 && col_group(5) == 8 && col_group(8) == 8 &&
                  col_group(3, 2) == 2 && col_group(8, 4) == 4 && col_group(3, 4) == 4,
              "col_group: the smallest of 1, 2, 4, 8 that holds kc, never above a ceiling of 2 or 4");

}
```

### agglomerationmultigrid1d_amd/csrc/host_plan.hpp

```cpp
#pragma once
#include <algorithm>
#include <cmath>
#include <cstddef>
#include <cstdint>
#include <cstring>
#include <vector>

#include "forms.hpp"

namespace aggmg {

constexpr int kCrTailRows = 4096;
constexpr int kCrMaxLevels = 40;
constexpr int kCrMaxStageLevels = 12;
constexpr int kCrMaxSteps = 8;

struct CrStagePlan {
  int l0 = 0, q = 0;
  int64_t n_in = 0, n_out = 0;
  int nsteps = 0;
  int step_a[kCrMaxSteps + 1] = {0};
  int lds_off[kCrMaxSteps + 1] = {0}, lds_xoff[kCrMaxSteps + 1] = {0};
  int lds_total = 0;
  int stack_stride = 0;
// ... 41 lines not shown
  return (size_t)S.lds_total * sizeof(double);
}
inline int cr_max_stage_levels(int m) {
  int q = kCrMaxStageLevels;
  while (q > 1 && cr_stage_lds_bytes(q, m) > kCrLdsBudgetBytes) --q;
  return q;
}

struct CrSolvePlan {
  std::vector<CrStagePlan> stages;
  CrStagePlan tail;
};
inline bool cr_plan_solve(const std::vector<int64_t>& level_n, int m, int tail_rows, int max_q, int fill_max,
                          int min_workgroups, CrSolvePlan* out) {
  const int nl = (int)level_n.size();
  auto ln = [&](int l) -> int64_t { return l < nl ? level_n[l] : 1; };
  out->stages.clear();
  max_q = std::min(max_q, cr_max_stage_levels(m));
  int l0 = 0;
  while (l0 < nl && ln(l0) * m > tail_rows) {
    int need = 0;
    while (l0 + need < nl && ln(l0 + need) * m > tail_rows) ++need;
    int fill = 0;
    while (fill < fill_max && (ln(l0) >> (fill + 1)) >= min_workgroups) ++fill;
    CrStagePlan S;
    S.l0 = l0;
    S.q = std::min({max_q, std::max(need, fill), nl - l0});
    if (S.q < 1) break;
    S.n_in = ln(l0);
    S.n_out = ln(l0 + S.q);
    cr_plan_steps(&S, m);
    out->stages.push_back(S);
    l0 += S.q;
  }
  if (nl - l0 > kCrMaxStageLevels || ln(l0) * m > tail_rows) return false;
  out->tail = CrStagePlan();
  out->tail.l0 = l0;
  out->tail.q = nl - l0;
  out->tail.n_in = ln(l0);
  out->tail.n_out = 1;
  cr_plan_steps(&out->tail, m);
  return true;
}

struct CrStageBuffers {
  int64_t part = 0, stack = 0, mid = 0;
};
inline CrStageBuffers cr_stage_buffers(const CrStagePlan& S, int m) {
  CrStageBuffers b;
  b.part = (S.n_out * m + 31) & ~(int64_t)31;
  b.stack = S.stack_stride > 0 ? (S.n_out + 1) * (int64_t)S.stack_stride : 0;
  b.mid = S.mid_total;
  return b;
}

inline int64_t cr_even(int64_t v) { return (v + 1) & ~(int64_t)1; }
struct CrMultiStage {
  int64_t part = 0, stack = 0, mid = 0;
  int64_t part_off = 0, stack_off = 0, mid_off = 0;
};
template <class Stage>
inline int64_t cr_multi_layout(const std::vector<Stage>& stages, const CrStagePlan& tail_plan, int m, int64_t cols,
                               std::vector<CrMultiStage>* st, CrMultiStage* tail) {
  int64_t o = 0;
  auto region = [&](int64_t stride, int64_t* off) {
    *off = o;
    o += cols * stride;
  };
  st->assign(stages.size(), CrMultiStage());
  for (size_t s = 0; s < stages.size(); ++s) {
    const CrStageBuffers b = cr_stage_buffers(stages[s], m);
    CrMultiStage& W = (*st)[s];
    W.part = 3 * b.part;
    W.stack = cr_even(b.stack);
    W.mid = cr_even(b.mid);
    region(W.part, &W.part_off);
    region(W.stack, &W.stack_off);
    region(W.mid, &W.mid_off);
  }
  *tail = CrMultiStage();
  tail->mid = cr_even(cr_stage_buffers(tail_plan, m).mid);
  region(tail->mid, &tail->mid_off);
  return o;
}

inline std::vector<int32_t> stream_row_blocks(const int32_t* rowptr, int64_t nrows, int max_nnz, int max_rows) {
  std::vector<int32_t> blk;
  blk.push_back(0);
  int64_t r = 0;
  while (r < nrows) {
    int64_t e = r + 1;
    const int64_t b0 = rowptr[r];
    while (e < nrows && e - r < max_rows && rowptr[e + 1] - b0 <= max_nnz) ++e;
    if (rowptr[r + 1] - b0 > max_nnz) e = r + 1;
    blk.push_back((int32_t)e);
    r = e;
  }
  return blk;
}

inline bool band_row_blocks(const int32_t* rowptr, int64_t nrows, int bw, int sweeps, int max_nnz, int window, int max_rows,
                            std::vector<int32_t>* out) {
  const int64_t H = (int64_t)(sweeps - 1) * bw;
  out->clear();
  out->push_back(0);
  int64_t r = 0;
  while (r < nrows) {
    const int64_t lo = std::max<int64_t>(0, r - H);
    auto fits = [&](int64_t e) {
      const int64_t hi = std::min(nrows, e + H);
      return rowptr[hi] - rowptr[lo] <= max_nnz && (e - r) + 2 * (int64_t)sweeps * bw <= window;
    };
    int64_t e = r + 1;
    if (!fits(e)) return false;
    while (e < nrows && e - r < max_rows && fits(e + 1)) ++e;
    out->push_back((int32_t)e);
    r = e;
  }
  return true;
}

struct TileSubset {
  int64_t ntiles = 0;
  int split = 0;
  int64_t skip = 0;
};
inline TileSubset fused_tile_subset(int64_t ne, int owned, int mode, int64_t head_in, int64_t tail_in) {
  TileSubset t;
  t.ntiles = (ne + owned - 1) / owned;
  if (mode == 0) return t;
  const int64_t head = std::min(std::max<int64_t>(head_in, 0), ne);
  const int64_t tail = std::min(std::max(tail_in, head), ne);
  const int64_t all = t.ntiles;
  const int64_t tA = std::min(all, (head + owned - 1) / owned);
  const int64_t tB = std::min(all - tA, all - tail / owned);
  if (mode == 1) {
    t.split = (int)tA;
    t.skip = all - tA - tB;
    t.ntiles = tA + tB;
  } else {
    t.skip = tA;
    t.ntiles = all - tA - tB;
  }
  return t;
}


struct FusedTilePlan {
  int owned = 0, halo_left = 0;
  int agg_shift = -1;
};
inline FusedTilePlan fused_tile_plan(int te, int halo, int align, bool var_agg, int agg_shift) {
  FusedTilePlan p;
  const bool aligned = var_agg && agg_shift >= 0 && te - 2 * halo - agg_shift >= te / 2;
  const int shift = aligned ? agg_shift : 0;
  if (aligned) p.agg_shift = agg_shift;
  p.owned = std::max(0, ((te - 2 * halo - shift) / align) * align);
  p.halo_left = halo + shift;
  return p;
}

inline int multi_tile_owned(int te, int halo, int align) { return std::max(0, ((te - 2 * halo) / align) * align); }

struct PairTilePlan {
  int own = 0;
  int te_a = 0, te_b = 0;
// ... 273 lines not shown
```

### agglomerationmultigrid1d_amd/csrc/internal.hpp

```cpp
#pragma once
#include "../../include/aggmg_hip.h"

#include <hip/hip_runtime.h>

#include <algorithm>
#include <array>
#include <atomic>
#include <chrono>
#include <cmath>
#include <cstdio>
#include <cstdlib>
#include <cstring>
#include <memory>
#include <string>
#include <type_traits>
#include <vector>

#include "kernels.hpp"
#include "cr_kernels.hpp"
#include "cgt_kernels.hpp"

using namespace aggmg;

struct aggmg_ctx;
inline int fail(aggmg_ctx* ctx, int code, const std::string& msg);

#define HIPCHK(expr)                                                                        \
  do {                                                                                      \
    hipError_t _e = (expr);                                                                 \
    if (_e != hipSuccess)                                                                   \
      return fail(ctx, AGGMG_ERR_HIP,                                                       \
                  std::string(#expr) + ": " + hipGetErrorString(_e) + " (" + __FILE__ + ":" + \
                      std::to_string(__LINE__) + ")");                                      \
  } while (0)

#define CHECK(expr)             \
  do {                          \
    int _s = (expr);            \
    if (_s != AGGMG_OK) return _s; \
  } while (0)

#include "devmem.hpp"
#include "workspace.hpp"

inline thread_local std::string g_create_error;

struct ProfEvent {
  hipEvent_t a, b;
  int tag;
};

struct aggmg_ctx {
  int device = 0;
  hipStream_t own_stream = nullptr;
  hipStream_t stream = nullptr;
  std::string err;
  bool sym_packing = true;
  int cr_max_q = 12;
  bool detect_chain = true;
  bool mg_checkpoint = [] { const char* e = std::getenv("AGGMG_MG_CHECKPOINT"); return !(e && e[0] == '0'); }();
  bool pair_levels = [] { const char* e = std::getenv("AGGMG_PAIR"); return !(e && e[0] == '0'); }();
  bool sym_residual = [] { const char* e = std::getenv("AGGMG_SYM_RESIDUAL"); return !(e && e[0] == '0'); }();
  bool op_dict = [] { const char* e = std::getenv("AGGMG_OP_DICT"); return !(e && e[0] == '0'); }();
  bool elem_threads = [] { const char* e = std::getenv("AGGMG_ELEM_THREADS"); return !(e && e[0] == '0'); }();
  int64_t elem_launches = 0;
  bool pair_elem_threads = [] { const char* e = std::getenv("AGGMG_PAIR_ELEM_THREADS"); return !(e && e[0] == '0'); }();
  int64_t pair_elem_launches = 0;
  int elem_rec_cap = [] { const char* e = std::getenv("AGGMG_ELEM_RECORDS_LDS"); return (e && e[0] == '0') ? 0 : kElemRecMaxClasses; }();
  int64_t elem_rec_launches = 0;
  bool replay_presmooth = [] { const char* e = std::getenv("AGGMG_REPLAY_PRESMOOTH"); return !(e && e[0] == '0'); }();
  int64_t replay_launches = 0;
  bool patch_multi = [] { const char* e = std::getenv("AGGMG_PATCH_MULTI"); return e && e[0] == '1'; }();
  int64_t patch_multi_launches = 0;
  bool chain_multi = [] { const char* e = std::getenv("AGGMG_CHAIN_MULTI"); return e && e[0] == '1'; }();
  int64_t chain_multi_launches = 0;
  bool patch_schwarz_multi = [] { const char* e = std::getenv("AGGMG_PATCH_SCHWARZ_MULTI"); return e && e[0] == '1'; }();
  int64_t patch_schwarz_multi_launches = 0;
  int patch_schwarz_multi_cols = [] {
    const char* e = std::getenv("AGGMG_PATCH_SCHWARZ_MULTI_COLS");
    return e && e[0] == '4' && !e[1] ? 4 : e && e[0] == '8' && !e[1] ? 8 : kPatchSchwarzMultiCols;
  }();
  int profiling = 0;
  std::vector<ProfEvent> prof;
  std::vector<hipEvent_t> ev_pool;
  WorkVectors<kScratchSlots> scratch;
  WorkVectors<kSolvSlots> solv;
  DevArray<double> solv_part, solv_sc;
  DevArray<double> cols_part, cols_sc;
  DevArray<int> cols_map;
  int64_t cols_cap = 0;
  DevArray<double> kry_part, kry_sc, kry_work;
  DevArray<double> kryc_part, kryc_sc;
  DevArray<int> kryc_map;
  int64_t kryc_cap = 0;
  DevArray<double> own_part;
  struct StageLane {
    hipStream_t stream = nullptr;
    void* pin[2] = {nullptr, nullptr};
    hipEvent_t ev[2] = {nullptr, nullptr};
  };
  std::vector<StageLane> stage;
  bool stage_failed = false;
  struct Pinned {
    char* base;
    size_t bytes;
    bool owned;
  };
  std::vector<Pinned> pinned;
};

inline int fail(aggmg_ctx* ctx, int code, const std::string& msg) {
  if (ctx)
    ctx->err = msg;
  else
    g_create_error = msg;
  return code;
}

inline hipStream_t HipMem::stream_of(aggmg_ctx* ctx) { return ctx->stream; }

struct CsrDev {
  int64_t nrows = 0, ncols = 0, nnz = 0;
  DevArray<int32_t> rowptr, colind;
  DevArray<double> vals;
  int lpr = 1;
  DevArray<int32_t> rowblk;
  int64_t nblk = 0;
  DevArray<int32_t> bandblk;
  int64_t nbandblk = 0;
  int band_sweeps = 1;
  int bw = -1;
  int maxrow = -1;
  CsrView view() const { return CsrView{rowptr, colind, vals, nrows}; }
};

struct HostCsr {
  std::vector<int32_t> rowptr, colind;
  std::vector<double> vals;
};

struct BtdDev {
  int m = 0;
  int64_t ne = 0;
  bool cmp = false;
  int c_sub = 0, r_sup = 0;
  DevArray<double> binv, dblk, scol, pcol, qrow;
  DevArray<double> bsym;
  DevArray<double> dup;
  DevArray<uint32_t> corr;
  DevArray<double> sub, sup, P, Q;
};

// ... 68 lines not shown

struct DictDev {
  int nclasses = 0;
  DevArray<uint16_t> cls;
  DevArray<double> bsym, qrow, qmir, dup, scol, dblk;
  DevArray<uint32_t> corr;
  DevArray<double> lf;
  bool lf_unit = false;
  DevArray<double> rec;
};

struct PairDictDev {
  int nclasses = 0;
  DevArray<uint16_t> cls;
  DevArray<double> bsym, sup, sback, sub, dblk;
  DevArray<double> lf;
  bool lf_unit = false;
  DevArray<double> rec;
};

struct TransferCgt {
  int type = 0, mc = 0, rho = 1;
  int64_t nec = 0;
  DevArray<double> l, lp;
  DevArray<int32_t> cperm;
};

struct CgtDictDev {
  int nclasses = 0;
  DevArray<uint16_t> cls;
  DevArray<double> dblk, subrow, supcol;
  DevArray<double> l;
  DevArray<double> lp;
};

struct Damping {
  double alpha;
  const double* w;
  Damping(double a, const double* w_ = nullptr) : alpha(a), w(w_) {}
  double at(int s) const { return w ? w[s] : alpha; }
  Damping from(int s) const { return Damping(alpha, w ? w + s : nullptr); }
  SweepWeights launch(int n) const {
    SweepWeights r;
    for (int i = 0; i < kSweepWeights; ++i) r.w[i] = w ? (i < n ? w[i] : 0.0) : alpha;
    return r;
  }
};
static_assert(kSweepWeights == AGGMG_MAX_SWEEP_WEIGHTS, "the documented limit is the kernels' array");

struct Level {
  aggmg_op* A = nullptr;
  aggmg_smoother* S = nullptr;
  aggmg_op* L = nullptr;
  int64_t N = 0;
  DevArray<double> u[2], rhs, tmp;
  std::unique_ptr<TransferBtd> tb;
  std::unique_ptr<TransferCgt> tc;
  std::unique_ptr<DictDev> dict;
  std::unique_ptr<CgtDictDev> cdict;
  std::unique_ptr<PairDictDev> pdict;
  bool cgt_fused = false;
  bool native_io = false;
  int64_t Nalloc = 0;
  bool scheduled = false;
  std::vector<double> w_pre, w_post, w_mid, w_replay;
  Damping damp_pre(double alpha) const { return scheduled ? Damping(alpha, w_pre.data()) : Damping(alpha); }
  Damping damp_post(double alpha) const { return scheduled ? Damping(alpha, w_post.data()) : Damping(alpha); }
  Damping damp_mid(double alpha) const { return scheduled ? Damping(alpha, w_mid.data()) : Damping(alpha); }
  Damping damp_replay(double alpha) const { return scheduled ? Damping(alpha, w_replay.data()) : Damping(alpha); }
};

struct BandedLU {
  int64_t n = 0;
  int kl = 0, ku = 0, ldab = 0;
  std::vector<double> ab;
  std::vector<int32_t> ipiv;
};

struct CrStage : CrStagePlan {
  DevArray<double> partR;
  double *partL = nullptr, *xq = nullptr;
  DevArray<double> stack;
  DevArray<double> mid;
};

struct CrRunStage {
  double *partR = nullptr, *partL = nullptr, *xq = nullptr, *stack = nullptr, *mid = nullptr;
  int64_t cs_part = 0, cs_stack = 0, cs_mid = 0;
};
struct CrRun {
  int kc = 1;
  std::vector<CrRunStage> st;
  CrRunStage tail;
};
inline CrRunStage cr_run_stage(const CrStage& S) { return {S.partR, S.partL, S.xq, S.stack, S.mid}; }

struct CrDev {
  bool valid = false;
  int m = 0;
  int64_t n0 = 0, N = 0;
  std::vector<CrLevel> lv;
  struct Factors {
    DevArray<double> fe, fo, lu;
    DevArray<int32_t> perm;
  };
  std::vector<Factors> owned;
  DevArray<char> arena;
  const double* lu_last = nullptr;
  const int32_t* perm_last = nullptr;
  std::vector<CrStage> st;
  CrStage tail;
  CrRun run;
  DevArray<double> d0, x0;
  std::shared_ptr<CgtDev> chain;
  DevArray<unsigned int> ticket;
  double cond_est = 0.0;
  struct Pcr {
    bool valid = false;
    bool pre = false;
    int n = 0, L = 0;
    DevArray<double> mult, lu;
    DevArray<int32_t> perm;
  } pcr;
  struct Raw {
    int level;
    int64_t n;
    DevArray<double> a, b, c;
  };
  std::vector<Raw> raw;
};

struct aggmg_hier {
  std::vector<Level> lv;
  int coarse_mode = 0;
  BandedLU coarse;
  CrDev cr;
  DevArray<double> cyc[2];
  DevArray<double> io[3];
  std::vector<std::array<DevArray<double>, 4>> mu;
  int64_t multi_cols = 0;
  DevArray<double> crw;
  int64_t crw_cols = 0;
  DevArray<double> crw_stage;
  int64_t crw_stage_cols = 0;
  int restriction = 0;
  bool halves_used = false, fine_iterate_absent = false;
  std::vector<double> h_coarse;
  double last_coarse_ms = 0.0;
  double cr_probe_backward_error = -1.0;
};

inline int default_restriction() { return AGGMG_RESTRICT_EXPLICIT; }

enum class LevelPath {
  Coarsest,
  FusedChain,
  FusedBtd,
  BtdTransfer,
  Patch,
  Generic
};
inline const BtdDev* level_btd(const Level& l) {
  if (!l.S || l.S->A != l.A) return nullptr;
  if (l.S->btd) return l.S->btd.get();
  return l.S->patch ? l.S->patch->btd.get() : nullptr;
}
inline LevelPath level_path(const aggmg_hier* h, int k) {
  const Level& l = h->lv[k];
  if (k == (int)h->lv.size() - 1) return LevelPath::Coarsest;
  if (l.cgt_fused) return LevelPath::FusedChain;
  if (l.S && l.S->patch && l.S->A == l.A) return LevelPath::Patch;
  if (l.S && l.S->btd && l.S->A == l.A) return l.tb ? LevelPath::FusedBtd : LevelPath::BtdTransfer;
  return LevelPath::Generic;
}

template <int NSLOT>
inline int lease_work(aggmg_ctx* ctx, WorkVectors<NSLOT>& w, const char* family, int slot, int64_t len, const char* who,
                      WorkLease* lease) {
  const WorkTake t = w.take(ctx, slot, len, who, lease);
  if (t.refused())
    return fail(ctx, AGGMG_ERR_UNSUPPORTED, std::string("internal: work vector ") + family + "[" + std::to_string(slot) +
                                                "] wanted by " + t.wanted_by + " is held by " + t.held_by);
  return t.code;
}
inline int scratch_lease(aggmg_ctx* ctx, ScratchSlot slot, int64_t len, const char* who, WorkLease* lease) {
  return lease_work(ctx, ctx->scratch, "scratch", slot, len, who, lease);
}
inline int solv_lease(aggmg_ctx* ctx, SolvSlot slot, int64_t len, const char* who, WorkLease* lease) {
  return lease_work(ctx, ctx->solv, "solv", slot, len, who, lease);
}

inline bool any_schedule(const aggmg_hier* h) {
  for (const Level& l : h->lv)
// ... 86 lines not shown
```

### agglomerationmultigrid1d_amd/csrc/setup.hip

```cpp
#include <functional>

#include <hipcub/hipcub.hpp>

#include "internal.hpp"
#include "setup_kernels.hpp"
#include "pair_elem_kernels.hpp"

namespace {

inline unsigned grid_for(int64_t n) { return (unsigned)((n + kSetupThreads - 1) / kSetupThreads); }

struct Flags {
  DevArray<int> d;
  int n = 0;
  int init(aggmg_ctx* ctx, int count) {
    n = count;
    return d.alloc(ctx, count, true);
  }
  int read(aggmg_ctx* ctx, int* host) {
    HIPCHK(hipMemcpyAsync(host, d, n * sizeof(int), hipMemcpyDeviceToHost, ctx->stream));
    HIPCHK(hipStreamSynchronize(ctx->stream));
    return AGGMG_OK;
  }
  int clear(aggmg_ctx* ctx) {
// ... 400 lines not shown
    if (Nc % mc) continue;
    const int64_t nec = Nc / mc;
    if (nec == 0 || nef % nec) continue;
    const int64_t rho = nef / nec;
    if (rho > 64) continue;
    DevArray<double> lf;
    CHECK(lf.alloc(ctx, Nf * mc, true));
    CHECK(bad.clear(ctx));
    LAUNCH(transfer_scatter_kernel, Nc, Nc, mf, mc, rho, (const int32_t*)L->csc.rowptr, (const int32_t*)L->csc.colind,
           (const double*)L->csc.vals, lf, bad.d);
    int bf[2] = {0, 0};
    CHECK(bad.read(ctx, bf));
    const int b1 = bf[0];
    if (b1) continue;
    out->lf = std::move(lf);
    if (Abtd && Abtd->dblk) {
      CHECK(out->ld.alloc(ctx, Nf * mc));
      LAUNCH(transfer_ld_kernel, Nf, nef, mf, mc, (const double*)out->lf, (const double*)Abtd->dblk, out->ld);
    }
    out->mc = mc;
    out->rho = (int)rho;
    out->nec = nec;
    CHECK(setup_unit_column(ctx, out, Nf));
    *ok = true;
    HIPCHK(hipStreamSynchronize(ctx->stream));
    return AGGMG_OK;
  }
  if (nef >= ((int64_t)1 << 31)) return AGGMG_OK;
  for (int mc = 1; mc <= 16; ++mc) {
    if (hint_mc > 0 && mc != hint_mc) continue;
    if (Nc % mc) continue;
    const int64_t nec = Nc / mc;
    if (nec == 0 || nec > nef) continue;
    DevArray<double> lf;
    DevArray<int32_t> first, parent;
    CHECK(lf.alloc(ctx, Nf * mc, true));
    CHECK(first.alloc(ctx, nec + 1, true));
    CHECK(parent.alloc(ctx, nef, true));
    CHECK(bad.clear(ctx));
    LAUNCH(transfer_vr_kernel, nec, nec, nef, mf, mc, 64, (const int32_t*)L->csc.rowptr, (const int32_t*)L->csc.colind,
           (const double*)L->csc.vals, first, parent, lf, bad.d);
    int bf[2] = {0, 0};
    CHECK(bad.read(ctx, bf));
    const int b1 = bf[0];
    if (b1) continue;
    out->lf = std::move(lf);
    out->first = std::move(first);
    out->parent = std::move(parent);
    if (Abtd && Abtd->dblk) {
      CHECK(out->ld.alloc(ctx, Nf * mc));
      LAUNCH(transfer_ld_kernel, Nf, nef, mf, mc, (const double*)out->lf, (const double*)Abtd->dblk, out->ld);
    }
    out->mc = mc;
    out->rho = 0;
    out->maxagg = bf[1];
    out->nec = nec;
    CHECK(setup_unit_column(ctx, out, Nf));
    *ok = true;
    HIPCHK(hipStreamSynchronize(ctx->stream));
    return AGGMG_OK;
  }
  return AGGMG_OK;
}

namespace {
struct DictFields {
  DictView v;
  std::function<int(aggmg_ctx*, int64_t)> make[kDictMaxFields];
  DictFields(int64_t ne) {
    std::memset(&v, 0, sizeof(v));
    v.ne = ne;
  }
  template <typename T>
  void add(const DevArray<T>& full, DevArray<T>* dict, int n, bool back = false) {
    static_assert(sizeof(T) == 8 || sizeof(T) == 4, "records are made of 64- and 32-bit words");
    const int k = v.nf++;
    make[k] = [this, k, dict](aggmg_ctx* ctx, int64_t count) {
      CHECK(dict->alloc(ctx, count));
      v.f[k].dict = dict->get();
      return (int)AGGMG_OK;
    };
    v.f[k] = DictField{full.get(), nullptr, n, (int)sizeof(T), back ? 1 : 0};
  }
};

int dict_build(aggmg_ctx* ctx, DictFields& F, DevArray<uint16_t>* cls, int* nclasses) {
  *nclasses = 0;
  DictView& v = F.v;
  const int64_t ne = v.ne;
  DevArray<unsigned long long> table;
  CHECK(table.alloc(ctx, kDictSlots, true));
  Flags stat;
  CHECK(stat.init(ctx, 2));
  LAUNCH(dict_collect_kernel, ne, v, table.get(), stat.d);
  int st[2] = {0, 0};
  CHECK(stat.read(ctx, st));
  if (st[1] || st[0] > kDictMaxClasses || st[0] < 1) return AGGMG_OK;
  std::vector<unsigned long long> slots(kDictSlots), hashes;
  HIPCHK(hipMemcpyAsync(slots.data(), table, slots.size() * sizeof(unsigned long long), hipMemcpyDeviceToHost, ctx->stream));
  HIPCHK(hipStreamSynchronize(ctx->stream));
  for (unsigned long long s : slots)
    if (s) hashes.push_back(s);
  std::sort(hashes.begin(), hashes.end());
  const int nc = (int)hashes.size();
  if (nc != st[0]) return AGGMG_OK;
  DevArray<unsigned long long> sorted, rep;
  CHECK(sorted.alloc(ctx, nc));
  CHECK(rep.alloc(ctx, nc));
  HIPCHK(hipMemcpyAsync(sorted, hashes.data(), (size_t)nc * sizeof(unsigned long long), hipMemcpyHostToDevice, ctx->stream));
  const std::vector<unsigned long long> none((size_t)nc, (unsigned long long)ne);
  HIPCHK(hipMemcpyAsync(rep, none.data(), (size_t)nc * sizeof(unsigned long long), hipMemcpyHostToDevice, ctx->stream));
  HIPCHK(hipStreamSynchronize(ctx->stream));
  CHECK(cls->alloc(ctx, ne));
  for (int k = 0; k < v.nf; ++k) CHECK(F.make[k](ctx, (int64_t)nc * v.f[k].n));
  Flags bad;
  CHECK(bad.init(ctx, 1));
  LAUNCH(dict_assign_kernel, ne, v, nc, (const unsigned long long*)sorted, cls->get(),
         rep.get(), bad.d);
  LAUNCH(dict_gather_kernel, nc, v, nc, (const unsigned long long*)rep);
  LAUNCH(dict_verify_kernel, ne, v, (const uint16_t*)*cls, bad.d);
  int b1 = 0;
  CHECK(bad.read(ctx, &b1));
  if (!b1) *nclasses = nc;
  return AGGMG_OK;
}
}

int setup_op_dictionary(aggmg_ctx* ctx, const BtdDev& b, const TransferBtd& t, std::unique_ptr<DictDev>* out) {
  out->reset();
  const int m = b.m;
  if (!(btd_sres_form(m, b.cmp) && b.bsym && b.scol && b.dblk && b.qrow)) return AGGMG_OK;
  if (!(t.rho > 0 && t.mc == 2 && t.lf) || b.ne < 1) return AGGMG_OK;
  const int T = m * (m + 1) / 2;
  auto d = std::make_unique<DictDev>();
  d->lf_unit = t.lf1 != nullptr;
  DictFields F(b.ne);
  F.add(b.bsym, &d->bsym, T);
  F.add(b.qrow, &d->qrow, m);
  F.add(b.qrow, &d->qmir, m, true);
  if (b.dup) {
    F.add(b.dup, &d->dup, T);
    F.add(b.corr, &d->corr, m);
  }
  F.add(b.scol, &d->scol, m);
  F.add(b.dblk, &d->dblk, m * m);
  F.add(t.lf1 ? t.lf1 : t.lf, &d->lf, m * (t.lf1 ? 1 : 2));
  CHECK(dict_build(ctx, F, &d->cls, &d->nclasses));
  if (m == 4 && d->nclasses > 0 && d->nclasses <= kElemRecMaxClasses) {
    const int nc = d->nclasses, nl = d->lf_unit ? m : 2 * m;
    std::vector<double> hb((size_t)T * nc), hq((size_t)m * nc), hm((size_t)m * nc), hd(b.dup ? (size_t)T * nc : 0), hl((size_t)nl * nc);
    std::vector<uint32_t> hc(b.dup ? (size_t)m * nc : 0);
    std::vector<double> rec((size_t)nc * kElemRecWords);
    auto down = [&](auto& v, const auto* src) {
      return hipMemcpyAsync(v.data(), src, v.size() * sizeof(v[0]), hipMemcpyDeviceToHost, ctx->stream);
    };
    HIPCHK(down(hb, d->bsym.get()));
    HIPCHK(down(hq, d->qrow.get()));
    HIPCHK(down(hm, d->qmir.get()));
    if (b.dup) {
      HIPCHK(down(hd, d->dup.get()));
      HIPCHK(down(hc, d->corr.get()));
    }
    HIPCHK(down(hl, d->lf.get()));
    HIPCHK(hipStreamSynchronize(ctx->stream));
    elem_record_pack(nc, hb.data(), hq.data(), hm.data(), b.dup ? hd.data() : nullptr, b.dup ? hc.data() : nullptr, hl.data(),
                     d->lf_unit, rec.data());
// ... 124 lines not shown
    CHECK(c2.alloc(ctx, ne * mm2));
    double *lu = F.lu, *fe = nullptr, *fo = nullptr;
    int32_t* perm = F.perm;
    LAUNCH((cr_factor_odd_kernel<M>), no, no, (const double*)a, (const double*)b, (const double*)c, lu, perm, Za.get(), Zc.get(),
           cond_dev, bad_dev);
    LAUNCH((cr_schur_even_kernel<M>), ne, n, ne, (const double*)a, (const double*)b, (const double*)c, (const double*)Za,
           (const double*)Zc, a2, b2, c2);
    HIPCHK(hipStreamSynchronize(ctx->stream));
    CHECK(F.fe.alloc(ctx, ne * 2 * mm2));
    CHECK(F.fo.alloc(ctx, std::max<int64_t>(no, 1) * 2 * mm2));
    fe = F.fe, fo = F.fo;
    LAUNCH(cr_split_kernel, n * 2 * mm2, n, mm2, (const double*)a, (const double*)c, fe, fo);
    LAUNCH((cr_even_multipliers_kernel<M>), no, no, ne, (const double*)lu, (const int32_t*)perm, fe);
    HIPCHK(hipStreamSynchronize(ctx->stream));
    CrLevel L;
    L.n = n;
    L.n_even = ne;
    L.n_odd = no;
    L.fe = fe;
    L.fo = fo;
    L.lu = lu;
    L.perm = perm;
    cr->lv.push_back(L);
    cr->owned.push_back(std::move(F));
    a = std::move(a2);
    b = std::move(b2);
    c = std::move(c2);
    n = ne;
    if ((int)cr->lv.size() > kCrMaxLevels) return AGGMG_ERR_UNSUPPORTED;
  }
  CrDev::Factors F;
  CHECK(F.lu.alloc(ctx, mm2));
  CHECK(F.perm.alloc(ctx, M));
  hipLaunchKernelGGL((cr_factor_last_kernel<M>), dim3(1), dim3(64), 0, ctx->stream, (const double*)b, F.lu.get(), F.perm.get(),
                     cond_dev, bad_dev);
  HIPCHK(hipGetLastError());
  HIPCHK(hipStreamSynchronize(ctx->stream));
  cr->lu_last = F.lu;
  cr->perm_last = F.perm;
  cr->owned.push_back(std::move(F));
  return AGGMG_OK;
}

template <int M>
static int setup_pcr_t(aggmg_ctx* ctx, CrDev* cr, const CrDev::Raw& R) {
  const int64_t n = R.n;
  constexpr int MM = M * M;
  int L = 0;
  while (((int64_t)1 << L) < n) ++L;
  if (L < 1 || L > kPcrMaxLevels) return AGGMG_OK;
  DevArray<double> mult, lu, ta, tb, tc;
  DevArray<int32_t> perm;
  CHECK(mult.alloc(ctx, (int64_t)L * n * 2 * MM, true));
  CHECK(lu.alloc(ctx, n * MM));
  CHECK(perm.alloc(ctx, n * M));
  CHECK(ta.alloc(ctx, n * MM));
  CHECK(tb.alloc(ctx, n * MM));
  CHECK(tc.alloc(ctx, n * MM));
  double *a2 = ta, *b2 = tb, *c2 = tc;
  Flags bad;
  CHECK(bad.init(ctx, 1));
  double *a = R.a, *b = R.b, *c = R.c;
  for (int k = 0; k < L; ++k) {
    LAUNCH((pcr_factor_kernel<M>), n, n, (const double*)b, lu.get(), perm.get(), bad.d);
    LAUNCH((pcr_reduce_kernel<M>), n, n, (int64_t)1 << k, (const double*)a, (const double*)b, (const double*)c,
           (const double*)lu, (const int32_t*)perm, mult.get() + (int64_t)k * n * 2 * MM, a2, b2, c2);
    std::swap(a, a2), std::swap(b, b2), std::swap(c, c2);
  }
  LAUNCH((pcr_factor_kernel<M>), n, n, (const double*)b, lu.get(), perm.get(), bad.d);
  int b1 = 0;
  CHECK(bad.read(ctx, &b1));
  if (b1) return AGGMG_OK;
  cr->pcr.n = (int)n;
  cr->pcr.L = L;
  cr->pcr.mult = std::move(mult);
  cr->pcr.lu = std::move(lu);
  cr->pcr.perm = std::move(perm);
  cr->pcr.valid = true;
  return AGGMG_OK;
}

void cr_discard(CrDev* c) { *c = CrDev(); }

__global__ __launch_bounds__(kSetupThreads) void probe_vector_kernel(int64_t n, double* __restrict__ w) {
  const int64_t i = (int64_t)blockIdx.x * kSetupThreads + threadIdx.x;
  if (i >= n) return;
  uint64_t z = (uint64_t)i * 0x9E3779B97F4A7C15ull + 0xD1B54A32D192ED03ull;
  z = (z ^ (z >> 30)) * 0xBF58476D1CE4E5B9ull;
  z = (z ^ (z >> 27)) * 0x94D049BB133111EBull;
  z ^= z >> 31;
  w[i] = (double)(int64_t)(z >> 11) * (1.0 / 4503599627370496.0) - 1.0;
}

__global__ __launch_bounds__(kSetupThreads) void csc_band_gather_kernel(int64_t n, int m, const int32_t* __restrict__ cp,
                                                                        const int32_t* __restrict__ rv,
                                                                        const double* __restrict__ vv,
                                                                        const double* __restrict__ x, double sign,
                                                                        double* __restrict__ y) {
  const int64_t i = (int64_t)blockIdx.x * kSetupThreads + threadIdx.x;
  if (i >= n) return;
  const int64_t bi = i / m;
  const int64_t j0 = bi > 0 ? (bi - 1) * m : 0;
  const int64_t j1 = (bi + 2) * m < n ? (bi + 2) * m : n;
  double acc = 0.0;
  for (int64_t j = j0; j < j1; ++j) {
    int32_t lo = cp[j], hi = cp[j + 1];
    while (lo < hi) {
      const int32_t mid = lo + (hi - lo) / 2;
      if (rv[mid] < (int32_t)i) lo = mid + 1; else hi = mid;
    }
    if (lo < cp[j + 1] && rv[lo] == (int32_t)i) acc += vv[lo] * x[j];
  }
  y[i] += sign * acc;
}

int setup_probe_vector(aggmg_ctx* ctx, int64_t n, double* w) {
  LAUNCH(probe_vector_kernel, n, n, w);
  return AGGMG_OK;
}

__global__ __launch_bounds__(kSetupThreads) void smooth_vector_kernel(int64_t n, double* __restrict__ w) {
  const int64_t i = (int64_t)blockIdx.x * kSetupThreads + threadIdx.x;
  if (i >= n) return;
  w[i] = 1.0 + 0.5 * cos(3.141592653589793 * (double)i / (double)n);
}

int setup_smooth_vector(aggmg_ctx* ctx, int64_t n, double* w) {
  LAUNCH(smooth_vector_kernel, n, n, w);
  return AGGMG_OK;
}

int setup_band_matvec_add(aggmg_ctx* ctx, const aggmg_op* A, int m, const double* x, double sign, double* y) {
  LAUNCH(csc_band_gather_kernel, A->m, A->m, m, (const int32_t*)A->csc.rowptr, (const int32_t*)A->csc.colind,
         (const double*)A->csc.vals, x, sign, y);
  return AGGMG_OK;
}

static int cr_factor_blocks(aggmg_ctx* ctx, CrDev* cr, DevArray<double> a, DevArray<double> b, DevArray<double> c);

int setup_cr(aggmg_ctx* ctx, const aggmg_op* Ac, int hint_m, CrDev* cr, int* band_out) {
  cr->valid = false;
  if (band_out) band_out[0] = band_out[1] = 0;
  const int64_t N = Ac->m;
  if (N == 0) return AGGMG_OK;
  const int32_t* cp = Ac->csc.rowptr;
  const int32_t* rv = Ac->csc.colind;
  const double* vv = Ac->csc.vals;
  Flags f;
  CHECK(f.init(ctx, 4));
  LAUNCH(band_kernel, N, N, cp, rv, f.d);
  int band[4];
  CHECK(f.read(ctx, band));
  const int kl = band[0], ku = band[1];
  if (band_out) band_out[0] = kl, band_out[1] = ku;
  Flags bad;
  CHECK(bad.init(ctx, 1));
  auto fits = [&](int mm_, bool* out) -> int {
    CHECK(bad.clear(ctx));
    LAUNCH(block_fit_kernel, N, N, mm_, cp, rv, bad.d);
    int b1 = 0;
    CHECK(bad.read(ctx, &b1));
    *out = !b1;
    return AGGMG_OK;
  };
  int m = 0;
  bool okm = false;
// ... 83 lines not shown
  const int tail_rows = env_int("AGGMG_CR_TAIL_ROWS", kCrTailRows, 8, kCrTailRows);
  const int max_q = env_int("AGGMG_CR_MAX_Q", ctx->cr_max_q, 1, kCrMaxStageLevels);
  CrSolvePlan plan;
  {
    const char* e = std::getenv("AGGMG_CR_FILL");
    const int fmax = e && *e ? std::atoi(e) : 12;
    const char* w = std::getenv("AGGMG_CR_MINWG");
    const int minwg = w && *w ? std::atoi(w) : 256;
    std::vector<int64_t> ln(nl);
    for (int l = 0; l < nl; ++l) ln[l] = cr->lv[l].n;
    if (!cr_plan_solve(ln, m, tail_rows, max_q, fmax, minwg, &plan)) {
      cr_discard(cr);
      return AGGMG_OK;
    }
  }
  for (const CrStagePlan& P : plan.stages) {
    CrStage S;
    static_cast<CrStagePlan&>(S) = P;
    const CrStageBuffers b = cr_stage_buffers(P, m);
    CHECK(dz(3 * b.part, &S.partR));
    S.partL = S.partR + b.part;
    S.xq = S.partL + b.part;
    if (b.stack > 0) CHECK(dz(b.stack, &S.stack));
    if (b.mid > 0) CHECK(dz(b.mid, &S.mid));
    cr->st.push_back(std::move(S));
  }
  static_cast<CrStagePlan&>(cr->tail) = plan.tail;
  if (const int64_t mid = cr_stage_buffers(plan.tail, m).mid; mid > 0) CHECK(dz(mid, &cr->tail.mid));
  {
    int pf = cr->tail.l0;
    while (pf > 0 && level_n(pf - 1) * m <= 8 * kCrTailRows) --pf;
    auto al = [](size_t b) { return (b + 255) & ~(size_t)255; };
    const size_t mm = (size_t)m * m;
    size_t total = al(mm * sizeof(double)) + al(m * sizeof(int32_t));
    for (int l = pf; l < nl; ++l) {
      const CrLevel& L = cr->lv[l];
      const size_t no = (size_t)std::max<int64_t>(L.n_odd, 1);
      total += al(L.n_even * 2 * mm * sizeof(double)) + al(no * 2 * mm * sizeof(double)) + al(no * mm * sizeof(double)) +
               al(no * m * sizeof(int32_t));
    }
    DevArray<char>& arena = cr->arena;
    CHECK(arena.alloc(ctx, (int64_t)total));
    size_t off = 0;
    auto move = [&](const void* src, size_t bytes) -> void* {
      void* dst = arena + off;
      (void)hipMemcpyAsync(dst, src, bytes, hipMemcpyDeviceToDevice, ctx->stream);
      off += al(bytes);
      return dst;
    };
    for (int l = pf; l < nl; ++l) {
      CrLevel& L = cr->lv[l];
      const size_t no = (size_t)std::max<int64_t>(L.n_odd, 1);
      L.fe = (const double*)move(L.fe, L.n_even * 2 * mm * sizeof(double));
      L.fo = (const double*)move(L.fo, no * 2 * mm * sizeof(double));
      L.lu = (const double*)move(L.lu, no * mm * sizeof(double));
      L.perm = (const int32_t*)move(L.perm, no * m * sizeof(int32_t));
    }
    cr->lu_last = (const double*)move(cr->lu_last, mm * sizeof(double));
    cr->perm_last = (const int32_t*)move(cr->perm_last, m * sizeof(int32_t));
    HIPCHK(hipGetLastError());
    HIPCHK(hipStreamSynchronize(ctx->stream));
    for (int l = pf; l <= nl; ++l) cr->owned[l] = CrDev::Factors();
  }
  if (m <= 2 && cr->tail.nsteps >= 1 && env_int("AGGMG_CR_PCR", 1, 0, 1)) {
    const bool pre = cr->tail.n_in > 512;
    const int want_level = cr->tail.l0 + (pre ? 1 : 0);
    const int64_t want_n = pre ? (cr->tail.n_in + 1) / 2 : cr->tail.n_in;
    if (cr->tail.n_in <= 1024 && (!pre || cr->tail.q >= 2))
      for (const auto& R : cr->raw)
        if (R.level == want_level && R.n == want_n) {
          if (m == 1) CHECK(setup_pcr_t<1>(ctx, cr, R));
          if (m == 2) CHECK(setup_pcr_t<2>(ctx, cr, R));
          cr->pcr.pre = pre;
        }
  }
  HIPCHK(hipStreamSynchronize(ctx->stream));
  cr->raw.clear();
  if (n * m != N) {
    CHECK(dz(n * m, &cr->d0));
    CHECK(dz(n * m, &cr->x0));
  }
  CHECK(cr->ticket.alloc(ctx, 1, true));
  HIPCHK(hipStreamSynchronize(ctx->stream));
  cr->run = CrRun();
  for (const CrStage& S : cr->st) cr->run.st.push_back(cr_run_stage(S));
  cr->run.tail = cr_run_stage(cr->tail);
  cr->valid = true;
  return AGGMG_OK;
}

static int cgt_build_impl(aggmg_ctx* ctx, aggmg_smoother* sm, const int64_t* elems, int64_t m1, int64_t nel, int one_based,
                          bool generate);

int cgt_build(aggmg_ctx* ctx, aggmg_smoother* sm, const int64_t* elems, int64_t m1, int64_t nel, int one_based) {
  return cgt_build_impl(ctx, sm, elems, m1, nel, one_based, false);
}

int cgt_detect(aggmg_ctx* ctx, aggmg_smoother* sm) {
  const aggmg_op* A = sm->A;
  const int64_t N = A->m;
  if (N < 3 || A->m != A->n) return AGGMG_OK;
  for (int64_t p = 8; p >= 1 && !sm->cgt; --p) {
    if ((N - 1) % p) continue;
    const int64_t nel = (N - 1) / p;
    const double full = (double)nel * (double)((p + 1) * (p + 1));
    if ((double)A->nnz > full || (double)A->nnz < 0.5 * full) continue;
    CHECK(cgt_build_impl(ctx, sm, nullptr, p + 1, nel, 0, true));
  }
  return AGGMG_OK;
}

static int cgt_build_impl(aggmg_ctx* ctx, aggmg_smoother* sm, const int64_t* elems, int64_t m1, int64_t nel, int one_based,
                          bool generate) {
  aggmg_op* A = sm->A;
  const int64_t N = A->m;
  const int64_t p = m1 - 1;
  if (p < 1 || p > 8 || nel < 1) return AGGMG_OK;
  if (N != nel * p + 1) return AGGMG_OK;
  const int64_t base = one_based ? 1 : 0;
  const int m = (int)p;
  const int64_t ne = nel + 1, Np = ne * m;
  if (Np >= ((int64_t)1 << 31)) return AGGMG_OK;
  auto g = std::make_shared<CgtDev>();
  g->m = m;
  g->ne = ne;
  g->N = N;
  DevArray<int64_t> el64;
  CHECK(el64.alloc(ctx, nel * m1));
  if (generate) {
    LAUNCH(chain_generate_elements_kernel, nel, nel, m, el64.get());
  } else {
    HIPCHK(hipMemcpyAsync(el64, elems, (size_t)nel * m1 * 8, hipMemcpyHostToDevice, ctx->stream));
  }
  CHECK(g->perm.alloc(ctx, Np));
  CHECK(g->inv.alloc(ctx, N));
  HIPCHK(hipMemsetAsync(g->perm, 0xFF, (size_t)Np * 4, ctx->stream));
  HIPCHK(hipMemsetAsync(g->inv, 0xFF, (size_t)N * 4, ctx->stream));
  Flags f;
  CHECK(f.init(ctx, 4));
  LAUNCH(chain_perm_kernel, nel, nel, m, N, el64.get(), base, g->perm, f.d);
  LAUNCH(perm_invert_kernel, Np, Np, (const int32_t*)g->perm, g->inv, f.d);
  LAUNCH(perm_cover_kernel, N, N, (const int32_t*)g->inv, f.d);
  LAUNCH(chain_affine_check_kernel, Np, ne, m, (const int32_t*)g->perm, f.d);
  int h[4];
  CHECK(f.read(ctx, h));
  if (h[0]) return fail(ctx, AGGMG_ERR_DIMENSION, "aggmg_jacobi_setup_elements: node index out of range");
  if (h[1]) return AGGMG_OK;
  g->affine = !h[3];
  CHECK(g->dblk.alloc(ctx, Np * m, true));
  CHECK(g->subrow.alloc(ctx, Np, true));
  CHECK(g->supcol.alloc(ctx, Np, true));
  LAUNCH(chain_scatter_kernel, N, N, m, (const int32_t*)g->inv, (const int32_t*)A->csc.rowptr, (const int32_t*)A->csc.colind,
         (const double*)A->csc.vals, g->dblk, g->subrow, g->supcol, f.d);
  LAUNCH(chain_pad_kernel, Np, Np, m, (const int32_t*)g->perm, g->dblk);
  CHECK(f.read(ctx, h));
  if (h[2]) return AGGMG_OK;
  sm->cgt = g;
  A->cgt = g;
  return AGGMG_OK;
}

int cgt_attach_schwarz(aggmg_ctx* ctx, aggmg_smoother* sm, int sw) {
  if (!sm->cgt || !sm->binv) return AGGMG_OK;
  CgtDev& g = *sm->cgt;
  const int M = g.m;
  const int64_t nel = g.ne - 1;
// ... 98 lines not shown
```

### agglomerationmultigrid1d_amd/csrc/setup_kernels.hpp

```cpp
#pragma once
#include <hip/hip_runtime.h>
#include <stdint.h>

namespace aggmg {

constexpr int kSetupThreads = 256;

__global__ __launch_bounds__(kSetupThreads) void csc_convert_colptr_kernel(int64_t n, const int64_t* __restrict__ colptr64,
                                                                           int64_t base, int64_t nnz,
                                                                           int32_t* __restrict__ colptr,
                                                                           int* __restrict__ err) {
  const int64_t j = (int64_t)blockIdx.x * kSetupThreads + threadIdx.x;
  if (j > n) return;
  const int64_t v = colptr64[j] - base;
  if (v < 0 || v > nnz || (j > 0 && v < colptr64[j - 1] - base)) err[0] = 1;
  if (j == 0 && v != 0) err[3] = 1;
  colptr[j] = (int32_t)v;
}

__global__ __launch_bounds__(kSetupThreads) void csc_convert_rows_kernel(int64_t n, int64_t m,
                                                                         const int32_t* __restrict__ colptr,
                                                                         const int64_t* __restrict__ rowval64,
                                                                         int64_t base, int32_t* __restrict__ rowval,
                                                                         int* __restrict__ err) {
// ... 812 lines not shown
  for (int r = 0; r < M; ++r)
#pragma unroll
    for (int q = 0; q < M; ++q) {
      B[r][q] = b[i * M * M + r * M + q];
      tb[r][q] = B[r][q];
      A_[r][q] = a[i * M * M + r * M + q];
      C_[r][q] = c[i * M * M + r * M + q];
    }
  const double nb1 = norm1_block<M>(B);
  if (!lu_invert<M>(tb, tinv) || !lu_perm_dev<M>(B, perm)) {
    bad[0] = 1;
    return;
  }
  atomic_max_pos(cond, nb1 * norm1_block<M>(tinv));
#pragma unroll
  for (int r = 0; r < M; ++r) {
    perm_out[j * M + r] = perm[r];
#pragma unroll
    for (int q = 0; q < M; ++q) lu_out[j * M * M + r * M + q] = r == q ? 1.0 / B[r][r] : B[r][q];
  }
  lu_perm_solve_dev<M>(B, perm, A_, X);
#pragma unroll
  for (int r = 0; r < M; ++r)
#pragma unroll
    for (int q = 0; q < M; ++q) Za[j * M * M + r * M + q] = X[r][q];
  lu_perm_solve_dev<M>(B, perm, C_, X);
#pragma unroll
  for (int r = 0; r < M; ++r)
#pragma unroll
    for (int q = 0; q < M; ++q) Zc[j * M * M + r * M + q] = X[r][q];
}

template <int M>
__global__ __launch_bounds__(kSetupThreads) void cr_even_multipliers_kernel(int64_t n_odd, int64_t n_even,
                                                                            const double* __restrict__ lu,
                                                                            const int32_t* __restrict__ perm,
                                                                            double* __restrict__ fe) {
  const int64_t k = (int64_t)blockIdx.x * kSetupThreads + threadIdx.x;
  if (k >= n_odd) return;
  double F[M][M];
  int pm[M];
#pragma unroll
  for (int r = 0; r < M; ++r) {
    pm[r] = perm[k * M + r];
#pragma unroll
    for (int q = 0; q < M; ++q) F[r][q] = lu[k * M * M + r * M + q];
  }
#pragma unroll
  for (int side = 0; side < 2; ++side) {
    const int64_t row = k + side;
    if (row >= n_even) continue;
    double* blk = fe + row * 2 * M * M + (side == 0 ? M * M : 0);
#pragma unroll
    for (int r = 0; r < M; ++r) {
      double z[M], w[M];
#pragma unroll
      for (int q = 0; q < M; ++q) {
        double t = blk[r * M + q];
#pragma unroll
        for (int p2 = 0; p2 < q; ++p2) t -= z[p2] * F[p2][q];
        z[q] = t * F[q][q];
      }
#pragma unroll
      for (int q = M - 1; q >= 0; --q) {
        double t = z[q];
#pragma unroll
        for (int p2 = q + 1; p2 < M; ++p2) t -= w[p2] * F[p2][q];
        w[q] = t;
      }
      double out[M];
#pragma unroll
      for (int c2 = 0; c2 < M; ++c2) {
        double t = 0.0;
#pragma unroll
        for (int q = 0; q < M; ++q) t = (pm[q] == c2) ? w[q] : t;
        out[c2] = t;
      }
#pragma unroll
      for (int c2 = 0; c2 < M; ++c2) blk[r * M + c2] = out[c2];
    }
  }
}

template <int M>
__device__ __forceinline__ void lu_rowsolve_dev(const double (&F)[M][M], const int (&pm)[M], const double (&blk)[M][M],
                                                double (&out)[M][M]) {
#pragma unroll
  for (int r = 0; r < M; ++r) {
    double z[M], w[M];
#pragma unroll
    for (int q = 0; q < M; ++q) {
      double t = blk[r][q];
#pragma unroll
      for (int p2 = 0; p2 < q; ++p2) t -= z[p2] * F[p2][q];
      z[q] = t * F[q][q];
    }
#pragma unroll
    for (int q = M - 1; q >= 0; --q) {
      double t = z[q];
#pragma unroll
      for (int p2 = q + 1; p2 < M; ++p2) t -= w[p2] * F[p2][q];
      w[q] = t;
    }
#pragma unroll
    for (int c2 = 0; c2 < M; ++c2) {
      double t = 0.0;
#pragma unroll
      for (int q = 0; q < M; ++q) t = (pm[q] == c2) ? w[q] : t;
      out[r][c2] = t;
    }
  }
}

template <int M>
__global__ __launch_bounds__(kSetupThreads) void pcr_factor_kernel(int64_t n, const double* __restrict__ b,
                                                                   double* __restrict__ lu, int32_t* __restrict__ perm,
                                                                   int* __restrict__ bad) {
  const int64_t i = (int64_t)blockIdx.x * kSetupThreads + threadIdx.x;
  if (i >= n) return;
  double B[M][M];
  int pm[M];
#pragma unroll
  for (int r = 0; r < M; ++r)
#pragma unroll
    for (int q = 0; q < M; ++q) B[r][q] = b[i * M * M + r * M + q];
  if (!lu_perm_dev<M>(B, pm)) {
    bad[0] = 1;
    return;
  }
#pragma unroll
  for (int r = 0; r < M; ++r) {
    perm[i * M + r] = pm[r];
#pragma unroll
    for (int q = 0; q < M; ++q) lu[i * M * M + r * M + q] = r == q ? 1.0 / B[r][r] : B[r][q];
  }
}

template <int M>
__global__ __launch_bounds__(kSetupThreads) void pcr_reduce_kernel(int64_t n, int64_t s, const double* __restrict__ a,
                                                                   const double* __restrict__ b, const double* __restrict__ c,
                                                                   const double* __restrict__ lu, const int32_t* __restrict__ perm,
                                                                   double* __restrict__ mult, double* __restrict__ a2,
                                                                   double* __restrict__ b2, double* __restrict__ c2) {
  const int64_t i = (int64_t)blockIdx.x * kSetupThreads + threadIdx.x;
  if (i >= n) return;
  constexpr int MM = M * M;
  double Bn[M][M], An[M][M], Cn[M][M];
#pragma unroll
  for (int r = 0; r < M; ++r)
#pragma unroll
    for (int q = 0; q < M; ++q) {
      Bn[r][q] = b[i * MM + r * M + q];
      An[r][q] = 0.0;
      Cn[r][q] = 0.0;
    }
#pragma unroll
  for (int side = 0; side < 2; ++side) {
    const int64_t j = side == 0 ? i - s : i + s;
    double X[M][M];
#pragma unroll
    for (int r = 0; r < M; ++r)
#pragma unroll
      for (int q = 0; q < M; ++q) X[r][q] = 0.0;
    if (j >= 0 && j < n) {
      double F[M][M], blk[M][M], aj[M][M], cj[M][M];
      int pm[M];
// ... 359 lines not shown
```

### include/aggmg_hip.h

```cpp
#ifndef AGGMG_HIP_H
#define AGGMG_HIP_H

#include <stdint.h>

#ifdef __cplusplus
extern "C" {
#endif

#define AGGMG_OK 0
#define AGGMG_ERR_ARGUMENT (-1)
#define AGGMG_ERR_DIMENSION (-2)
#define AGGMG_ERR_SINGULAR (-3)
#define AGGMG_ERR_HIP (-4)
#define AGGMG_ERR_UNSUPPORTED (-5)

typedef struct aggmg_ctx aggmg_ctx;
typedef struct aggmg_op aggmg_op;
typedef struct aggmg_smoother aggmg_smoother;
typedef struct aggmg_hier aggmg_hier;

int aggmg_create(int device_id, aggmg_ctx** out);
int aggmg_destroy(aggmg_ctx* ctx);
const char* aggmg_last_error(aggmg_ctx* ctx);
int aggmg_set_stream(aggmg_ctx* ctx, void* hip_stream);
int aggmg_reset_stream(aggmg_ctx* ctx);
int aggmg_synchronize(aggmg_ctx* ctx);
#define AGGMG_OPT_SYMMETRIC_PACKING 1
#define AGGMG_OPT_COARSE_CHUNK_LOG2 2
#define AGGMG_OPT_DETECT_CHAIN 3
#define AGGMG_OPT_PAIR_LEVELS 4
#define AGGMG_OPT_MG_CHECKPOINT 5
#define AGGMG_OPT_SYMMETRIC_RESIDUAL 6
#define AGGMG_OPT_OPERATOR_DICTIONARY 7
#define AGGMG_OPT_ELEMENT_THREADS 8
#define AGGMG_OPT_PAIR_ELEMENT_THREADS 9
#define AGGMG_OPT_REPLAY_PRESMOOTH 10
#define AGGMG_OPT_PATCH_MULTI 11
#define AGGMG_OPT_CHAIN_MULTI 12
#define AGGMG_OPT_ELEMENT_RECORDS_LDS 13
#define AGGMG_OPT_PATCH_SCHWARZ_MULTI 14
int aggmg_set_option(aggmg_ctx* ctx, int option, int value);
int aggmg_element_record_lds_launches(aggmg_ctx* ctx, int64_t* count);
int aggmg_element_record_lds_cap(aggmg_ctx* ctx, int* cap, int* max_cap);
int aggmg_element_record_pack(int nclasses, const double* bsym, const double* qrow, const double* qmir, const double* dup,
                              const uint32_t* corr, const double* lf, int lf_unit, double* rec, int* words);
int aggmg_element_thread_launches(aggmg_ctx* ctx, int64_t* count);
int aggmg_pair_element_thread_launches(aggmg_ctx* ctx, int64_t* count);
int aggmg_replay_launches(aggmg_ctx* ctx, int64_t* count);
int aggmg_patch_multi_launches(aggmg_ctx* ctx, int64_t* count);
int aggmg_patch_schwarz_multi_launches(aggmg_ctx* ctx, int64_t* count);
int aggmg_chain_multi_launches(aggmg_ctx* ctx, int64_t* count);
int aggmg_chain_multi_tile_plan(int m, int nsweeps, int restrict_kind, int rho, int kb, int* tile_blocks, int* owned,
                                int* halo_left, int* halo_right, int* max_sweeps);
int aggmg_dev_alloc(aggmg_ctx* ctx, int64_t nbytes, void** out);
int aggmg_dev_free(aggmg_ctx* ctx, void* ptr);
int aggmg_memcpy_h2d(aggmg_ctx* ctx, void* dst_dev, const void* src_host, int64_t nbytes);
int aggmg_memcpy_d2h(aggmg_ctx* ctx, void* dst_host, const void* src_dev, int64_t nbytes);
int aggmg_host_register(aggmg_ctx* ctx, void* ptr, int64_t nbytes);
int aggmg_host_unregister(aggmg_ctx* ctx, void* ptr);
int aggmg_host_alloc(aggmg_ctx* ctx, int64_t nbytes, void** out);
int aggmg_host_free(aggmg_ctx* ctx, void* ptr);

#define AGGMG_OP_STIFFNESS 0
#define AGGMG_OP_TRANSFER 1
int aggmg_csc_upload(aggmg_ctx* ctx, int64_t m, int64_t n, const int64_t* colptr,
                     const int64_t* rowval, const double* nzval, int one_based, int kind,
                     aggmg_op** out);
int aggmg_op_free(aggmg_ctx* ctx, aggmg_op* op);
int aggmg_op_shape(aggmg_ctx* ctx, const aggmg_op* op, int64_t* m, int64_t* n, int64_t* nnz);
int aggmg_op_download(aggmg_ctx* ctx, const aggmg_op* op, int transposed, int32_t* rowptr,
                      int32_t* colind, double* vals);
int aggmg_op_release_host(aggmg_ctx* ctx, aggmg_op* op);

int aggmg_blockjacobi_setup(aggmg_ctx* ctx, aggmg_op* A, int64_t m, int64_t nb,
                            const int64_t* blockinds, int one_based, int kind,
                            aggmg_smoother** out);
int aggmg_jacobi_setup(aggmg_ctx* ctx, aggmg_op* A, aggmg_smoother** out);
int aggmg_jacobi_setup_elements(aggmg_ctx* ctx, aggmg_op* A, int64_t nodes_per_element, int64_t n_elements,
                                const int64_t* element_nodes, int one_based, aggmg_smoother** out);
int aggmg_blockdiag_setup(aggmg_ctx* ctx, int64_t m, int64_t nb, const double* blocks, int factorize,
                          aggmg_smoother** out);
int aggmg_patch_schwarz_setup(aggmg_ctx* ctx, aggmg_op* A, int64_t m, int64_t ne, int width, int hybrid,
                              aggmg_smoother** out);
int aggmg_smoother_patch_info(aggmg_ctx* ctx, const aggmg_smoother* sm, int* width, int* hybrid, int* fused);
int aggmg_smoother_patch_dictionary(aggmg_ctx* ctx, const aggmg_smoother* sm, int* nclasses);
int aggmg_patch_tile_plan(int m, int nsweeps, int* tile_elems, int* owned, int* max_sweeps);
int aggmg_patch_gs_setup(aggmg_ctx* ctx, aggmg_op* A, int64_t m, int64_t ne, aggmg_smoother** out);
int aggmg_smoother_patch_kind(aggmg_ctx* ctx, const aggmg_smoother* sm, int* kind);
int aggmg_patch_gs_tile_plan(int m, int nsweeps, int* tile_elems, int* owned, int* halo, int* max_sweeps);
int aggmg_patch_gs_multi_tile_plan(int m, int nsweeps, int kb, int* tile_elems, int* owned, int* halo, int* max_sweeps);
int aggmg_patch_schwarz_multi_tile_plan(int m, int nsweeps, int kb, int* tile_elems, int* owned, int* halo, int* max_sweeps);
int aggmg_smooth_multi_dev(aggmg_ctx* ctx, aggmg_op* A, aggmg_smoother* sm, const double* U0, const double* B,
                           int64_t ncols, int64_t ld, const double* weights, int nsweeps, int reverse, double* U);
int aggmg_smoother_free(aggmg_ctx* ctx, aggmg_smoother* sm);
int aggmg_smoother_apply(aggmg_ctx* ctx, aggmg_smoother* sm, const double* B, int64_t N,
                         int64_t ncols, double alpha, double* Y);
int aggmg_smoother_is_structured(aggmg_ctx* ctx, const aggmg_smoother* sm, int* out);

int aggmg_bd_sp_apply(aggmg_ctx* ctx, aggmg_smoother* bd, aggmg_op* S, int kind, aggmg_op** out);
int aggmg_sp_matmul(aggmg_ctx* ctx, aggmg_op* A, aggmg_op* B, int kind, aggmg_op** out);
int aggmg_sp_sub(aggmg_ctx* ctx, aggmg_op* A, aggmg_op* B, int kind, aggmg_op** out);
int aggmg_op_transpose(aggmg_ctx* ctx, aggmg_op* A, int kind, aggmg_op** out);
int aggmg_op_download_csc(aggmg_ctx* ctx, const aggmg_op* op, int32_t* colptr, int32_t* rowval, double* nzval);
int aggmg_smoother_download_blocks(aggmg_ctx* ctx, const aggmg_smoother* sm, double* out);
int aggmg_debug_scan_counts(aggmg_ctx* ctx, const int32_t* counts_host, int64_t n, int64_t* total);
int aggmg_debug_stream_copy(aggmg_ctx* ctx, void* dst, const void* src, int64_t nbytes, int workgroups, int mode,
                            double* ms_out);
int aggmg_debug_device_memory(int64_t* live_allocations, int64_t* live_bytes);

int aggmg_smooth(aggmg_ctx* ctx, aggmg_op* A, aggmg_smoother* sm, double* u_inout,
                 const double* b, double alpha, int nsweeps);
int aggmg_residual(aggmg_ctx* ctx, aggmg_op* A, const double* u, const double* b, double* r_out);
int aggmg_restrict(aggmg_ctx* ctx, aggmg_op* L, const double* r, double* rc_out);
int aggmg_prolong_add(aggmg_ctx* ctx, aggmg_op* L, const double* uc, double* u_inout);
int aggmg_smooth_dev(aggmg_ctx* ctx, aggmg_op* A, aggmg_smoother* sm, const double* u_in,
                     const double* b, double alpha, int nsweeps, double* u_out);
int aggmg_smooth_weighted_dev(aggmg_ctx* ctx, aggmg_op* A, aggmg_smoother* sm, const double* u_in,
                              const double* b, const double* w, int nsweeps, double* u_out);
int aggmg_residual_dev(aggmg_ctx* ctx, aggmg_op* A, const double* u, const double* b,
                       double* r_out);
int aggmg_restrict_dev(aggmg_ctx* ctx, aggmg_op* L, const double* r, double* rc_out);
int aggmg_prolong_add_dev(aggmg_ctx* ctx, aggmg_op* L, const double* uc, double* u_inout);

#define AGGMG_COARSE_HOST_BANDED 0
#define AGGMG_COARSE_DEVICE_CR 1
#define AGGMG_COARSE_EXTERNAL 3
#define AGGMG_COARSE_AUTO 2
#define AGGMG_COARSE_DEVICE_CHAIN 4
int aggmg_hier_create(aggmg_ctx* ctx, int nlevels, aggmg_op* const* stiffness,
                      aggmg_smoother* const* smoothers, aggmg_op* const* interpolation,
                      int coarse_mode, aggmg_hier** out);
int aggmg_hier_free(aggmg_ctx* ctx, aggmg_hier* h);
int aggmg_vcycle(aggmg_ctx* ctx, aggmg_hier* h, const double* x0, const double* b, int nPre,
                 int nPost, double alpha, double* x_out);
int aggmg_vcycle_dev(aggmg_ctx* ctx, aggmg_hier* h, const double* x0, const double* b, int nPre,
                     int nPost, double alpha, double* x_out);
int aggmg_vcycle_multi_dev(aggmg_ctx* ctx, aggmg_hier* h, const double* X0, const double* B, int64_t ncols, int64_t ld,
                           int nPre, int nPost, double alpha, double* X);
int aggmg_hier_coarse_solve_multi_dev(aggmg_ctx* ctx, aggmg_hier* h, const double* B, int64_t ncols, int64_t ld, double* X);
int aggmg_hier_multi_info(aggmg_ctx* ctx, const aggmg_hier* h, int64_t ncols, int nPre, int nPost, int* fused, int* group);
int aggmg_residual_multi_dev(aggmg_ctx* ctx, aggmg_op* A, const double* X, const double* B, int64_t ncols, int64_t ld,
                             double* R);
int aggmg_vcycles_dev(aggmg_ctx* ctx, aggmg_hier* h, const double* x0, const double* b, int ncycles,
                      int nPre, int nPost, double alpha, double* x_out);
#define AGGMG_RESTRICT_EXPLICIT 0
#define AGGMG_RESTRICT_PRECONDITIONED 1
#define AGGMG_RESTRICT_PRECONDITIONED_MAX_ELEMS (1 << 21)
int aggmg_hier_set_restriction(aggmg_ctx* ctx, aggmg_hier* h, int mode);
int aggmg_hier_get_restriction(aggmg_ctx* ctx, const aggmg_hier* h, int* mode);
int aggmg_vcycle_down_dev(aggmg_ctx* ctx, aggmg_hier* h, const double* x0, const double* b, int nPre,
                          double alpha);
int aggmg_vcycle_up_dev(aggmg_ctx* ctx, aggmg_hier* h, const double* b, int nPost, double alpha,
                        double* x_out);
int aggmg_vcycle_up_split_dev(aggmg_ctx* ctx, aggmg_hier* h, const double* b, int nPost, double alpha,
                              double* x_out, int64_t head_elems, int64_t tail_elem, int part);
int aggmg_vcycle_up_split_ok(aggmg_ctx* ctx, const aggmg_hier* h, int nPost, int* ok);
int aggmg_vcycle_up_coarse_dev(aggmg_ctx* ctx, aggmg_hier* h, const double* b, int nPost, double alpha, int part,
                               int64_t ghosts_lo, int64_t ghosts_hi);
int aggmg_hier_coarse_buffers(aggmg_ctx* ctx, aggmg_hier* h, void** rhs_dev, void** sol_dev,
                              int64_t* n);
int aggmg_coarse_plan(aggmg_ctx* ctx, const aggmg_hier* h, int* chunk_log2, int64_t* n_boundary,
                      int* block_size, int64_t* n_blocks);
int aggmg_coarse_chunk_forward_dev(aggmg_ctx* ctx, aggmg_hier* h, const double* rhs_owned, int64_t blk_lo,
                                   int64_t blk_hi, double* partR, double* partL);
int aggmg_coarse_boundary_solve_dev(aggmg_ctx* ctx, aggmg_hier* h, const double* partR, const double* partL,
                                    double* xq);
int aggmg_coarse_chunk_backward_dev(aggmg_ctx* ctx, aggmg_hier* h, const double* rhs_owned, int64_t blk_lo,
                                    int64_t blk_hi, const double* xq, double* x_owned);
#define AGGMG_LEVEL_GENERIC 0
#define AGGMG_LEVEL_FUSED_BTD 1
#define AGGMG_LEVEL_FUSED_CHAIN 2
#define AGGMG_LEVEL_COARSEST 3
int aggmg_hier_level_kind(aggmg_ctx* ctx, const aggmg_hier* h, int level, int* kind);
int aggmg_hier_level_paired(aggmg_ctx* ctx, const aggmg_hier* h, int level, int nsweeps, int* paired);
int aggmg_hier_level_paired_up(aggmg_ctx* ctx, const aggmg_hier* h, int level, int nsweeps, int* paired);
int aggmg_hier_level_sym_residual(aggmg_ctx* ctx, const aggmg_hier* h, int level, int* on);
int aggmg_hier_level_dictionary(aggmg_ctx* ctx, const aggmg_hier* h, int level, int* nclasses);
#define AGGMG_MAX_SWEEP_WEIGHTS 8
int aggmg_hier_set_sweep_weights(aggmg_ctx* ctx, aggmg_hier* h, int level, const double* pre, int npre,
                                 const double* post, int npost);
int aggmg_hier_get_sweep_weights(aggmg_ctx* ctx, const aggmg_hier* h, int level, double* pre, int* npre, double* post,
                                 int* npost);
int aggmg_hier_estimate_lambda_max(aggmg_ctx* ctx, aggmg_hier* h, int level, const double* v0, int iters,
                                   double* lambda_max);
int aggmg_hier_coarse_info(aggmg_ctx* ctx, const aggmg_hier* h, int* on_device, int* block_size,
                           double* cond_est);
int aggmg_hier_coarse_probe(aggmg_ctx* ctx, const aggmg_hier* h, double* backward_error);
int aggmg_hier_coarse_chain(aggmg_ctx* ctx, const aggmg_hier* h, int* on, int* m, int64_t* blocks);
int aggmg_hier_coarse_tail(aggmg_ctx* ctx, const aggmg_hier* h, int* kind, int64_t* blocks);
int aggmg_hier_last_coarse_ms(aggmg_ctx* ctx, const aggmg_hier* h, double* ms);

int aggmg_copy_segments_dev(aggmg_ctx* ctx, int nseg, const double* const* src, double* const* dst,
                            const int64_t* rows, const int64_t* cols, const int64_t* src_ld,
                            const int64_t* dst_ld);

typedef struct aggmg_dist aggmg_dist;
int aggmg_dist_create(aggmg_ctx* ctx, aggmg_hier* local, aggmg_hier* coarse_global, int world, int rank, int nlevels,
                      const int64_t* own_lo, const int64_t* own_hi, const int64_t* loc_lo, const int64_t* loc_hi,
                      const int64_t* ne, const int32_t* m, const int32_t* W, aggmg_dist** out);
int aggmg_dist_free(aggmg_ctx* ctx, aggmg_dist* d);
#define AGGMG_RCCL_ID_BYTES 128
typedef int (*aggmg_allgather_fn)(void* user, const double* send_dev, double* recv_dev, int64_t count, void* hip_stream);
int aggmg_rccl_unique_id(aggmg_ctx* ctx, void* id_out, int nbytes);
int aggmg_rccl_available(char* why, int nbytes);
int aggmg_dist_init_rccl(aggmg_ctx* ctx, aggmg_dist* d, const void* id, int nbytes, int* nranks_out);
int aggmg_dist_set_allgather(aggmg_ctx* ctx, aggmg_dist* d, aggmg_allgather_fn fn, void* user);
typedef int (*aggmg_sendrecv_fn)(void* user, int nops, const int* peer, const int* is_send, double* const* dev_ptr,
                                 const int64_t* count, void* hip_stream);
int aggmg_dist_set_sendrecv(aggmg_ctx* ctx, aggmg_dist* d, aggmg_sendrecv_fn fn);
int aggmg_dist_set_neighbor_layout(aggmg_ctx* ctx, aggmg_dist* d, int level, int nto_left, const int64_t* to_left_off,
                                   const int64_t* to_left_len, int nto_right, const int64_t* to_right_off,
                                   const int64_t* to_right_len, int nfrom_left, const int64_t* from_left_off,
                                   const int64_t* from_left_len, int nfrom_right, const int64_t* from_right_off,
                                   const int64_t* from_right_len);
int aggmg_dist_set_loopback(aggmg_ctx* ctx, aggmg_dist* d);
int aggmg_dist_set_exchange_layout(aggmg_ctx* ctx, aggmg_dist* d, int level, int64_t count, int nsend,
                                   const int64_t* send_src, const int64_t* send_dst, const int64_t* send_len,
                                   int nleft, const int64_t* left_src, const int64_t* left_dst, const int64_t* left_len,
                                   int nright, const int64_t* right_src, const int64_t* right_dst,
                                   const int64_t* right_len);
int aggmg_dist_allgather_dev(aggmg_ctx* ctx, aggmg_dist* d, const double* send_dev, double* recv_dev, int64_t count);
int aggmg_dist_exchange_ghosts_dev(aggmg_ctx* ctx, aggmg_dist* d, double* x_local, int level);
#define AGGMG_DIST_X0_GHOSTS_VALID 1
#define AGGMG_DIST_OVERLAP_NEXT 2
#define AGGMG_DIST_GRAPH 4
int aggmg_dist_vcycle_dev(aggmg_ctx* ctx, aggmg_dist* d, double* x0, const double* b, double* x_out, int nPre,
                          int nPost, double alpha, int flags);
int aggmg_dist_set_coarse_overlap(aggmg_ctx* ctx, aggmg_dist* d, int on);
int aggmg_dist_info(aggmg_ctx* ctx, const aggmg_dist* d, int64_t* exchanges, int* chunked, int* backend);
int aggmg_dist_graph_info(aggmg_ctx* ctx, const aggmg_dist* d, int64_t* replays, int* captured, int* broken);

int aggmg_dot_dev(aggmg_ctx* ctx, const double* x, const double* y, int64_t n, double* out);
int aggmg_norm2_dev(aggmg_ctx* ctx, const double* x, int64_t n, double* out);
int aggmg_residual_norm_dev(aggmg_ctx* ctx, aggmg_op* A, const double* x, const double* b, double* out);
int aggmg_multigrid_dev(aggmg_ctx* ctx, aggmg_hier* h, const double* x0, const double* b, int maxiter,
                        double tol, int check_every, int nPre, int nPost, double alpha, double* x_out,
                        double* res_hist, int* n_cycles, int* n_checks, const double* u_exact, double* err_hist);
int aggmg_smoother_solve_dev(aggmg_ctx* ctx, aggmg_op* A, aggmg_smoother* sm, const double* x0,
                             const double* b, int maxiter, double tol, double alpha, int check_every,
                             double* x_out, double* res_hist, int* n_iters, int* n_checks, const double* u_exact,
                             double* err_hist);
int aggmg_pcg_dev(aggmg_ctx* ctx, aggmg_hier* h, const double* b, double* x_inout, int maxiter, double tol,
                  int nPre, int nPost, double alpha, double* res_hist, int* n_iters);
int aggmg_multi_dot_dev(aggmg_ctx* ctx, const double* V, int64_t n, int64_t nvec, int64_t ld, const double* w,
                        double* out_host);
int aggmg_multi_axpy_norm_dev(aggmg_ctx* ctx, const double* V, int64_t n, int64_t nvec, int64_t ld, const double* coef_host,
                              double* w_inout, double* norm_out_host);
#define AGGMG_FGMRES_MAX_RESTART 64
int aggmg_fgmres_dev(aggmg_ctx* ctx, aggmg_hier* h, const double* b, double* x_inout, int restart, int maxiter, double tol,
                     int nPre, int nPost, double alpha, double* res_hist, int* n_iters);
int aggmg_multi_dot_cols_dev(aggmg_ctx* ctx, const double* V, int64_t n, int64_t nvec, int64_t ncols, int64_t bstride,
                             int64_t cstride, const double* W, int64_t ldw, double* out_host);
int aggmg_multi_axpy_norm_cols_dev(aggmg_ctx* ctx, const double* V, int64_t n, int64_t nvec, int64_t ncols, int64_t bstride,
                                   int64_t cstride, const double* coef_host, double* W_inout, int64_t ldw,
                                   double* norm_out_host);
int aggmg_fgmres_multi_dev(aggmg_ctx* ctx, aggmg_hier* h, const double* B, double* X_inout, int64_t ncols, int64_t ld,
                           int restart, int maxiter, double tol, int nPre, int nPost, double alpha, double* res_hist,
                           int* n_iters, int64_t* work_cols);
int aggmg_dot_cols_dev(aggmg_ctx* ctx, const double* X, const double* Y, int64_t n, int64_t ncols, int64_t ld,
                       double* out_host);
int aggmg_norm2_cols_dev(aggmg_ctx* ctx, const double* X, int64_t n, int64_t ncols, int64_t ld, double* out_host);
int aggmg_pcg_multi_dev(aggmg_ctx* ctx, aggmg_hier* h, const double* B, double* X_inout, int64_t ncols, int64_t ld,
                        int maxiter, double tol, int nPre, int nPost, double alpha, double* res_hist, int* n_iters,
                        int64_t* work_cols);
int aggmg_owned_dot_dev(aggmg_ctx* ctx, const double* x, const double* y, int nranges, const int64_t* lo,
                        const int64_t* hi, double* out);
int aggmg_pcg_xr_owned_dev(aggmg_ctx* ctx, int64_t n, double* x, double* r, const double* p, const double* q, double a,
// ... 38 lines not shown
```

Before: 521.4 billion DoF-updates/s.

## Deduplicate coarse cyclic-reduction factors into per-stage LDS dictionaries

At setup, the per-block even/odd cyclic-reduction factors (fe, fo, LU, perm) of the coarse tridiagonal solve are grouped into classes of identical blocks. Each stage gets a packed table plus per-chunk uint16 class indices. New forward/backward CR kernels load that table into LDS and read factors from it instead of streaming the full per-block factor arrays from global memory. This targets memory traffic in the coarsest-level solve. In exchange it adds setup cost, LDS pressure and a dependence on the mesh producing few distinct classes; it falls back to the old kernels when class counts exceed the cap.

```diff
diff --git a/agglomerationmultigrid1d_amd/_lib.py b/agglomerationmultigrid1d_amd/_lib.py
--- a/agglomerationmultigrid1d_amd/_lib.py
+++ b/agglomerationmultigrid1d_amd/_lib.py
@@ -22,6 +22,7 @@
 OPT_CHAIN_MULTI = 12
 OPT_ELEMENT_RECORDS_LDS = 13
 OPT_PATCH_SCHWARZ_MULTI = 14
+OPT_COARSE_DICTIONARY = 15
 PROFILE_NTAGS = 256
 KIND_FUSED_DOWN, KIND_FUSED_UP, KIND_SMOOTH, KIND_RESIDUAL, KIND_RESTRICT, KIND_PROLONG, \
     KIND_JACOBI, KIND_BLOCK_APPLY, KIND_COARSE, KIND_FUSED_MID = range(10)
@@ -86,6 +87,9 @@
     "aggmg_element_record_lds_launches": (c_int, [_P, POINTER(c_int64)]),
     "aggmg_element_record_lds_cap": (c_int, [_P, POINTER(c_int), POINTER(c_int)]),
     "aggmg_element_record_pack": (c_int, [c_int, _P, _P, _P, _P, _P, _P, c_int, _P, POINTER(c_int)]),
+    "aggmg_coarse_dictionary_launches": (c_int, [_P, POINTER(c_int64)]),
+    "aggmg_coarse_dictionary_cap": (c_int, [_P, POINTER(c_int), POINTER(c_int)]),
+    "aggmg_hier_coarse_dictionary": (c_int, [_P, _P, c_int, POINTER(c_int), _P, _P, _P, _P, _P]),
     "aggmg_patch_multi_launches": (c_int, [_P, POINTER(c_int64)]),
     "aggmg_patch_schwarz_multi_launches": (c_int, [_P, POINTER(c_int64)]),
     "aggmg_chain_multi_launches": (c_int, [_P, POINTER(c_int64)]),
diff --git a/agglomerationmultigrid1d_amd/api.py b/agglomerationmultigrid1d_amd/api.py
--- a/agglomerationmultigrid1d_amd/api.py
+++ b/agglomerationmultigrid1d_amd/api.py
@@ -78,6 +78,16 @@
     def element_record_lds_cap(self):
         c, m = ctypes.c_int(0), ctypes.c_int(0)
         self.check(self.lib.aggmg_element_record_lds_cap(self.handle, ctypes.byref(c), ctypes.byref(m)))
+        return int(c.value), int(m.value)
+
+    def coarse_dictionary_launches(self):
+        n = ctypes.c_int64(0)
+        self.check(self.lib.aggmg_coarse_dictionary_launches(self.handle, ctypes.byref(n)))
+        return int(n.value)
+
+    def coarse_dictionary_cap(self):
+        c, m = ctypes.c_int(0), ctypes.c_int(0)
+        self.check(self.lib.aggmg_coarse_dictionary_cap(self.handle, ctypes.byref(c), ctypes.byref(m)))
         return int(c.value), int(m.value)
 
     def patch_multi_launches(self):
@@ -1181,6 +1191,16 @@
                     tail=("none", "cyclic reduction", "parallel cyclic reduction")[k.value], tail_blocks=nb.value,
                     order="element chain" if on.value else "operator")
 
+    def coarse_dictionary(self):
+        cap = 64
+        arr = [(ctypes.c_int * cap)() for _ in range(5)]
+        ns = ctypes.c_int(0)
+        self.ctx.check(self.ctx.lib.aggmg_hier_coarse_dictionary(self.ctx.handle, self.handle, cap, ctypes.byref(ns), *arr))
+        taken, first, nlv, ev, od = arr
+        stages = [dict(taken=bool(taken[s]), first_level=int(first[s]), levels=int(nlv[s])) for s in range(ns.value)]
+        nl = max((s["first_level"] + s["levels"] for s in stages), default=0)
+        return dict(stages=stages, even_classes=[int(ev[l]) for l in range(nl)], odd_classes=[int(od[l]) for l in range(nl)])
+
     def last_coarse_ms(self):
         ms = ctypes.c_double(0.0)
         self.ctx.check(self.ctx.lib.aggmg_hier_last_coarse_ms(self.ctx.handle, self.handle, ctypes.byref(ms)))
diff --git a/agglomerationmultigrid1d_amd/csrc/aggmg_hip.hip b/agglomerationmultigrid1d_amd/csrc/aggmg_hip.hip
--- a/agglomerationmultigrid1d_amd/csrc/aggmg_hip.hip
+++ b/agglomerationmultigrid1d_amd/csrc/aggmg_hip.hip
@@ -176,6 +176,11 @@
       if (value < 0 || value > kElemRecMaxClasses)
         return fail(ctx, AGGMG_ERR_ARGUMENT, "aggmg_set_option: AGGMG_OPT_ELEMENT_RECORDS_LDS takes 0 .. " + std::to_string(kElemRecMaxClasses));
       ctx->elem_rec_cap = value;
+      return AGGMG_OK;
+    case AGGMG_OPT_COARSE_DICTIONARY:
+      if (value < 0 || value > kCrDictMaxClasses)
+        return fail(ctx, AGGMG_ERR_ARGUMENT, "aggmg_set_option: AGGMG_OPT_COARSE_DICTIONARY takes 0 .. " + std::to_string(kCrDictMaxClasses));
+      ctx->coarse_dict_cap = value;
       return AGGMG_OK;
     case AGGMG_OPT_PATCH_MULTI:
       ctx->patch_multi = value != 0;
@@ -1742,16 +1747,51 @@
   hipLaunchKernelGGL((cr_tail_kernel<M>), dim3(1, kc), dim3(kCrThreads), tail_lds, ctx->stream, T, d, db, x);
 }
 
+static CrDictArgs cr_make_dict_args(const CrStage& S) {
+  CrDictArgs D;
+  std::memset(&D, 0, sizeof(D));
+  D.tab = S.dict_tab;
+  D.cidx = S.dict_idx;
+  for (int l = 0; l < S.q; ++l) {
+    D.tab_e[l] = S.dict.tab_e[l];
+    D.tab_o[l] = S.dict.tab_o[l];
+    D.idx_e[l] = S.dict.idx_e[l];
+    D.idx_o[l] = S.dict.idx_o[l];
+  }
+  D.tab_words = S.dict.tab_words;
+  D.idx_count = S.dict.idx_count;
+  D.tab_off = S.dict.tab_off;
+  D.idx_off = S.dict.idx_off;
+  return D;
+}
+
 template <int M, bool FUSE_TAIL = false>
-static void cr_launch_forward(aggmg_ctx* ctx, const CrStageArgs& A, unsigned grid, int kc, const double* d, const double* db,
-                              double* partR, double* partL, const CrStageArgs& T, size_t tail_lds = 0, double* xt = nullptr,
-                              unsigned int* ticket = nullptr) {
+static void cr_launch_forward(aggmg_ctx* ctx, const CrStage& S, const CrStageArgs& A, unsigned grid, int kc, const double* d,
+                              const double* db, double* partR, double* partL, const CrStageArgs& T, size_t tail_lds = 0,
+                              double* xt = nullptr, unsigned int* ticket = nullptr) {
+  if constexpr (cr_dict_form(M)) {
+    if (S.dict.take) {
+      hipLaunchKernelGGL((cr_stage_forward_dict_kernel<M, FUSE_TAIL>), dim3(grid, kc), dim3(cr_stage_threads()),
+                         std::max(S.dict.lds_bytes, tail_lds), ctx->stream, A, cr_make_dict_args(S), d, db, partR, partL, T, xt,
+                         ticket);
+      ++ctx->coarse_dict_launches;
+      return;
+    }
+  }
   hipLaunchKernelGGL((cr_stage_forward_kernel<M, FUSE_TAIL>), dim3(grid, kc), dim3(cr_stage_threads()),
                      std::max((size_t)A.lds_total * sizeof(double), tail_lds), ctx->stream, A, d, db, partR, partL, T, xt, ticket);
 }
 template <int M>
-static void cr_launch_backward(aggmg_ctx* ctx, const CrStageArgs& A, unsigned grid, int kc, const double* d, const double* db,
-                               const double* xq, double* x) {
+static void cr_launch_backward(aggmg_ctx* ctx, const CrStage& S, const CrStageArgs& A, unsigned grid, int kc, const double* d,
+                               const double* db, const double* xq, double* x) {
+  if constexpr (cr_dict_form(M)) {
+    if (S.dict.take) {
+      hipLaunchKernelGGL((cr_stage_backward_dict_kernel<M>), dim3(grid, kc), dim3(cr_stage_threads()), S.dict.lds_bytes,
+                         ctx->stream, A, cr_make_dict_args(S), d, db, xq, x);
+      ++ctx->coarse_dict_launches;
+      return;
+    }
+  }
   hipLaunchKernelGGL((cr_stage_backward_kernel<M>), dim3(grid, kc), dim3(cr_stage_threads()), (size_t)A.lds_total * sizeof(double),
                      ctx->stream, A, d, db, xq, x);
 }
@@ -1790,9 +1830,9 @@
     A.dstride = in.dstride;
     const unsigned grid = (unsigned)std::max<int64_t>(A.n_out, 1);
     if (s == ns - 1 && fuse_tail) {
-      cr_launch_forward<M, true>(ctx, A, grid, kc, in.d, in.db, R.partR, R.partL, T, tail_lds, R.xq, cr.ticket);
+      cr_launch_forward<M, true>(ctx, cr.st[s], A, grid, kc, in.d, in.db, R.partR, R.partL, T, tail_lds, R.xq, cr.ticket);
     } else {
-      cr_launch_forward<M>(ctx, A, grid, kc, in.d, in.db, R.partR, R.partL, T);
+      cr_launch_forward<M>(ctx, cr.st[s], A, grid, kc, in.d, in.db, R.partR, R.partL, T);
       if (s == ns - 1) {
         T.cs_d = T.cs_x = R.cs_part;
         cr_launch_tail<M>(ctx, cr, T, tail_lds, R.partR, R.partL, R.xq, kc);
@@ -1805,7 +1845,7 @@
     A.cs_d = in.cs_d;
     A.cs_x = in.cs_x;
     A.dstride = in.dstride;
-    cr_launch_backward<M>(ctx, A, (unsigned)std::max<int64_t>(A.n_out, 1), kc, in.d, in.db, run.st[s].xq, in.x);
+    cr_launch_backward<M>(ctx, cr.st[s], A, (unsigned)std::max<int64_t>(A.n_out, 1), kc, in.d, in.db, run.st[s].xq, in.x);
   }
   HIPCHK(hipGetLastError());
   return AGGMG_OK;
@@ -1823,11 +1863,11 @@
   if (!grid) return AGGMG_OK;
   const double* d0 = d_owned - blk_lo * M;
   if (backward) {
-    cr_launch_backward<M>(ctx, A, grid, 1, d0, nullptr, xq, x_owned - blk_lo * M);
+    cr_launch_backward<M>(ctx, S, A, grid, 1, d0, nullptr, xq, x_owned - blk_lo * M);
   } else {
     CrStageArgs T;
     std::memset(&T, 0, sizeof(T));
-    cr_launch_forward<M>(ctx, A, grid, 1, d0, nullptr, partR, partL, T);
+    cr_launch_forward<M>(ctx, S, A, grid, 1, d0, nullptr, partR, partL, T);
   }
   HIPCHK(hipGetLastError());
   return AGGMG_OK;
@@ -2381,6 +2421,39 @@
 extern "C" int aggmg_pair_element_thread_launches(aggmg_ctx* ctx, int64_t* count) {
   if (!ctx || !count) return fail(ctx, AGGMG_ERR_ARGUMENT, "aggmg_pair_element_thread_launches: NULL argument");
   *count = ctx->pair_elem_launches;
+  return AGGMG_OK;
+}
+
+extern "C" int aggmg_coarse_dictionary_launches(aggmg_ctx* ctx, int64_t* count) {
+  if (!ctx || !count) return fail(ctx, AGGMG_ERR_ARGUMENT, "aggmg_coarse_dictionary_launches: NULL argument");
+  *count = ctx->coarse_dict_launches;
+  return AGGMG_OK;
+}
+
+extern "C" int aggmg_coarse_dictionary_cap(aggmg_ctx* ctx, int* cap, int* max_cap) {
+  if (!ctx || !cap) return fail(ctx, AGGMG_ERR_ARGUMENT, "aggmg_coarse_dictionary_cap: NULL argument");
+  *cap = ctx->coarse_dict_cap;
+  if (max_cap) *max_cap = kCrDictMaxClasses;
+  return AGGMG_OK;
+}
+
+extern "C" int aggmg_hier_coarse_dictionary(aggmg_ctx* ctx, const aggmg_hier* h, int capacity, int* nstages, int* taken,
+                                            int* first_level, int* nlevels, int* even_classes, int* odd_classes) {
+  if (!ctx || !h || !nstages || !taken || !first_level || !nlevels || !even_classes || !odd_classes || capacity < kCrMaxLevels)
+    return fail(ctx, AGGMG_ERR_ARGUMENT, "aggmg_hier_coarse_dictionary: NULL argument or capacity below " + std::to_string(kCrMaxLevels));
+  const CrDev& cr = h->cr;
+  *nstages = cr.valid ? (int)cr.st.size() : 0;
+  for (int i = 0; i < capacity; ++i) taken[i] = first_level[i] = nlevels[i] = 0, even_classes[i] = odd_classes[i] = -1;
+  if (!cr.valid) return AGGMG_OK;
+  for (size_t s = 0; s < cr.st.size(); ++s) {
+    taken[s] = cr.st[s].dict.take ? 1 : 0;
+    first_level[s] = cr.st[s].l0;
+    nlevels[s] = cr.st[s].q;
+  }
+  for (size_t l = 0; l < cr.dict_even.size() && l < (size_t)capacity; ++l) {
+    even_classes[l] = cr.dict_even[l];
+    odd_classes[l] = cr.dict_odd[l];
+  }
   return AGGMG_OK;
 }
 
diff --git a/agglomerationmultigrid1d_amd/csrc/cr_kernels.hpp b/agglomerationmultigrid1d_amd/csrc/cr_kernels.hpp
--- a/agglomerationmultigrid1d_amd/csrc/cr_kernels.hpp
+++ b/agglomerationmultigrid1d_amd/csrc/cr_kernels.hpp
@@ -425,6 +425,17 @@
   }
 }
 
+struct CrGlobalFactors {
+  template <int M, int QS>
+  __device__ __forceinline__ void even(const CrStageArgs& A, int a, int64_t b, CrSubFactors<M, QS>& F) const {
+    cr_pre_load<M, QS, 0>(&A.lv[a], b, F);
+  }
+  template <int M, int QS>
+  __device__ __forceinline__ void odd(const CrStageArgs& A, int a, int64_t b, CrSubFactorsB<M, QS>& F) const {
+    cr_pre_load_b<M, QS, 0>(&A.lv[a], b, F);
+  }
+};
+
 struct CrStepGeom {
   int a, a1;
   int64_t lo_in, lo_out;
@@ -518,10 +529,10 @@
   }
 }
 
-template <int M, int QS>
+template <int M, int QS, class Src = CrGlobalFactors>
 __device__ __forceinline__ void cr_step_forward(const CrStageArgs& A, int s, int64_t c, bool wg_shared,
                                                 const double* __restrict__ d0, const double* __restrict__ d0b,
-                                                double* sh) {
+                                                double* sh, const Src& src = Src()) {
   const CrStepGeom g = cr_step_geom<QS>(A, s, c, wg_shared);
   const int cnt_out = ((1 << (A.q - g.a1)) + 1) * M;
   double* Rout = sh + A.lds_off[s + 1];
@@ -533,7 +544,7 @@
     bool tshared;
     if constexpr (M <= 2) {
       CrSubFactors<M, QS> F;
-      cr_pre_load<M, QS, 0>(&A.lv[g.a], b, F);
+      src.template even<M, QS>(A, g.a, b, F);
       __builtin_amdgcn_sched_barrier(0);
       cr_loc_load<M, QS>(A, s, g, b, d0, d0b, sh, v, thi, tshared, wg_shared && s > 0 && i == g.nb - 1);
 #ifdef AGGMG_CR_TRACE
@@ -562,11 +573,11 @@
   }
 }
 
-template <int M, int QS>
+template <int M, int QS, class Src = CrGlobalFactors>
 __device__ __forceinline__ void cr_step_backward(const CrStageArgs& A, int s, int64_t c, bool wg_shared,
                                                  const double* __restrict__ d0, const double* __restrict__ d0b,
                                                  const double* xtop, int64_t xtop_lo, double* xout, int64_t xout_lo,
-                                                 double* sh) {
+                                                 double* sh, const Src& src = Src()) {
   constexpr int NB = 1 << QS;
   const CrStepGeom g = cr_step_geom<QS>(A, s, c, wg_shared);
   for (int i = threadIdx.x; i < g.nb; i += blockDim.x) {
@@ -579,7 +590,7 @@
     const int64_t br = has_right ? b + 1 : b;
     if constexpr (M <= 2) {
       CrSubFactorsB<M, QS> F;
-      cr_pre_load_b<M, QS, 0>(&A.lv[g.a], b, F);
+      src.template odd<M, QS>(A, g.a, b, F);
       __builtin_amdgcn_sched_barrier(0);
       cr_loc_load<M, QS>(A, s, g, b, d0, d0b, sh, v, thi, tshared, wg_shared && s > 0 && i == g.nb - 1);
       if constexpr (QS >= 2) cr_mid_move<M, QS, 1, false>(cr_col_mid(A) + A.mid_off[s] + b * (cr_mid_blocks<QS>() * M), v);
@@ -621,29 +632,30 @@
   }
 }
 
-template <int M>
+template <int M, class Src = CrGlobalFactors>
 __device__ __forceinline__ void cr_forward_steps(const CrStageArgs& A, int64_t c, bool wg_shared,
                                                  const double* __restrict__ d0, const double* __restrict__ d0b,
-                                                 double* sh) {
+                                                 double* sh, const Src& src = Src()) {
   constexpr int Q = CrRadix<M>::Q;
   for (int s = 0; s < A.nsteps; ++s) {
     const int qs = A.step_a[s + 1] - A.step_a[s];
     if (qs == 1) {
-      cr_step_forward<M, 1>(A, s, c, wg_shared, d0, d0b, sh);
+      cr_step_forward<M, 1>(A, s, c, wg_shared, d0, d0b, sh, src);
     } else if (qs == 2) {
-      cr_step_forward<M, 2>(A, s, c, wg_shared, d0, d0b, sh);
+      cr_step_forward<M, 2>(A, s, c, wg_shared, d0, d0b, sh, src);
     } else {
-      if constexpr (Q >= 3) cr_step_forward<M, 3>(A, s, c, wg_shared, d0, d0b, sh);
+      if constexpr (Q >= 3) cr_step_forward<M, 3>(A, s, c, wg_shared, d0, d0b, sh, src);
     }
     __syncthreads();
     CR_STAMP(A, 4 + s);
   }
 }
 
-template <int M>
+template <int M, class Src = CrGlobalFactors>
 __device__ __forceinline__ void cr_backward_steps(const CrStageArgs& A, int64_t c, bool wg_shared,
                                                   const double* __restrict__ d0, const double* __restrict__ d0b,
-                                                  const double* __restrict__ xq, double* __restrict__ x0, double* sh) {
+                                                  const double* __restrict__ xq, double* __restrict__ x0, double* sh,
+                                                  const Src& src = Src()) {
   constexpr int Q = CrRadix<M>::Q;
   for (int s = A.nsteps - 1; s >= 0; --s) {
     const int a = A.step_a[s], a1 = A.step_a[s + 1];
@@ -654,11 +666,11 @@
     double* xout = s ? sh + A.lds_xoff[s] : x0;
     const int64_t xout_lo = s ? (c << (A.q - a)) : 0;
     if (qs == 1) {
-      cr_step_backward<M, 1>(A, s, c, wg_shared, d0, d0b, xtop, xtop_lo, xout, xout_lo, sh);
+      cr_step_backward<M, 1>(A, s, c, wg_shared, d0, d0b, xtop, xtop_lo, xout, xout_lo, sh, src);
     } else if (qs == 2) {
-      cr_step_backward<M, 2>(A, s, c, wg_shared, d0, d0b, xtop, xtop_lo, xout, xout_lo, sh);
+      cr_step_backward<M, 2>(A, s, c, wg_shared, d0, d0b, xtop, xtop_lo, xout, xout_lo, sh, src);
     } else {
-      if constexpr (Q >= 3) cr_step_backward<M, 3>(A, s, c, wg_shared, d0, d0b, xtop, xtop_lo, xout, xout_lo, sh);
+      if constexpr (Q >= 3) cr_step_backward<M, 3>(A, s, c, wg_shared, d0, d0b, xtop, xtop_lo, xout, xout_lo, sh, src);
     }
     __syncthreads();
     CR_STAMP(A, 8 + s);
@@ -805,6 +817,204 @@
   CR_TRACE_FLUSH(A);
 }
 
+struct CrDictArgs {
+  const double* tab;
+  const uint16_t* cidx;
+  int tab_e[kCrMaxStageLevels], tab_o[kCrMaxStageLevels];
+  int idx_e[kCrMaxStageLevels], idx_o[kCrMaxStageLevels];
+  int tab_words, idx_count;
+  int tab_off, idx_off;
+};
+
+__device__ __forceinline__ void cr_dict_fill(const CrDictArgs& D, int64_t c, int lds_total, double* sh) {
+  constexpr int kRounds = 6;
+  const double2* st = reinterpret_cast<const double2*>(D.tab);
+  const double2* si = reinterpret_cast<const double2*>(D.cidx + c * D.idx_count);
+  double2* dt = reinterpret_cast<double2*>(sh + D.tab_off);
+  double2* di = reinterpret_cast<double2*>(sh + D.idx_off);
+  const int nt = D.tab_words / 2, ni = D.idx_count / 8;
+  double2 rt[kRounds], ri[kRounds];
+#pragma unroll
+  for (int k = 0; k < kRounds; ++k) {
+    const int t = (int)threadIdx.x + k * (int)blockDim.x;
+    rt[k] = st[t < nt ? t : nt - 1];
+  }
+#pragma unroll
+  for (int k = 0; k < kRounds; ++k) {
+    const int t = (int)threadIdx.x + k * (int)blockDim.x;
+    ri[k] = si[t < ni ? t : ni - 1];
+  }
+  for (int t = threadIdx.x; t < lds_total; t += blockDim.x) sh[t] = 0.0;
+#pragma unroll
+  for (int k = 0; k < kRounds; ++k) {
+    const int t = (int)threadIdx.x + k * (int)blockDim.x;
+    if (t < nt) dt[t] = rt[k];
+    if (t < ni) di[t] = ri[k];
+  }
+  for (int t = (int)threadIdx.x + kRounds * (int)blockDim.x; t < nt; t += blockDim.x) dt[t] = st[t];
+  for (int t = (int)threadIdx.x + kRounds * (int)blockDim.x; t < ni; t += blockDim.x) di[t] = si[t];
+}
+
+template <int M, int QS, int I>
+__device__ __forceinline__ void cr_pre_load_dict(const CrDictArgs& D, const double* tab, const uint16_t* idx, int q, int a,
+                                                 int64_t c, int64_t b, CrSubFactors<M, QS>& F) {
+  if constexpr (I < QS) {
+    const int l = a + I;
+    constexpr int NB1 = 1 << (QS - I - 1);
+    const int t0 = (int)((b << (QS - I - 1)) - (c << (q - l - 1)));
+    const uint16_t* ix = idx + D.idx_e[l] + t0;
+    const double* T = tab + D.tab_e[l];
+#pragma unroll
+    for (int jj = 0; jj <= NB1; ++jj) cr_load_pair<M>(T + (int)ix[jj] * (2 * M * M), F.fe[CrEvenOff<QS, I>::rows + jj]);
+    cr_pre_load_dict<M, QS, I + 1>(D, tab, idx, q, a, c, b, F);
+  }
+}
+
+template <int M, int QS, int I>
+__device__ __forceinline__ void cr_pre_load_b_dict(const CrDictArgs& D, const double* tab, const uint16_t* idx, int q, int a,
+                                                   int64_t c, int64_t b, CrSubFactorsB<M, QS>& F) {
+  if constexpr (I < QS) {
+    const int l = a + I;
+    constexpr int NB1 = 1 << (QS - I - 1);
+    constexpr int W = (3 * M * M + (M + 1) / 2 + 1) & ~1;
+    const int t0 = (int)((b << (QS - I - 1)) - (c << (q - l - 1)));
+    const uint16_t* ix = idx + D.idx_o[l] + t0;
+    const double* T = tab + D.tab_o[l];
+#pragma unroll
+    for (int jj = 0; jj < NB1; ++jj) {
+      const double* r = T + (int)ix[jj] * W;
+      constexpr int o = CrOddOff<QS, I>::rows;
+      cr_load_pair<M>(r, F.fo[o + jj]);
+      if constexpr (M == 2) {
+        const double2 t0v = reinterpret_cast<const double2*>(r + 2 * M * M)[0], t1v = reinterpret_cast<const double2*>(r + 2 * M * M)[1];
+        const int2 pp = *reinterpret_cast<const int2*>(r + 3 * M * M);
+        F.lu[o + jj][0] = t0v.x, F.lu[o + jj][1] = t0v.y, F.lu[o + jj][2] = t1v.x, F.lu[o + jj][3] = t1v.y;
+        F.perm[o + jj][0] = pp.x, F.perm[o + jj][1] = pp.y;
+      } else {
+#pragma unroll
+        for (int k = 0; k < M * M; ++k) F.lu[o + jj][k] = r[2 * M * M + k];
+#pragma unroll
+        for (int k = 0; k < M; ++k) F.perm[o + jj][k] = reinterpret_cast<const int32_t*>(r + 3 * M * M)[k];
+      }
+    }
+    cr_pre_load_b_dict<M, QS, I + 1>(D, tab, idx, q, a, c, b, F);
+  }
+}
+
+struct CrDictLds {
+  const CrDictArgs& D;
+  const double* tab;
+  const uint16_t* idx;
+  int64_t c;
+  template <int M, int QS>
+  __device__ __forceinline__ void even(const CrStageArgs& A, int a, int64_t b, CrSubFactors<M, QS>& F) const {
+    cr_pre_load_dict<M, QS, 0>(D, tab, idx, A.q, a, c, b, F);
+  }
+  template <int M, int QS>
+  __device__ __forceinline__ void odd(const CrStageArgs& A, int a, int64_t b, CrSubFactorsB<M, QS>& F) const {
+    cr_pre_load_b_dict<M, QS, 0>(D, tab, idx, A.q, a, c, b, F);
+  }
+};
+
+template <int M, bool FUSE_TAIL>
+__global__ __launch_bounds__(kCrThreads) CR_WAVES_ATTR void cr_stage_forward_dict_kernel(CrStageArgs A, CrDictArgs D,
+                                                                           const double* __restrict__ d0,
+                                                                           const double* __restrict__ d0b, double* partR,
+                                                                           double* partL, CrStageArgs T, double* xq,
+                                                                           unsigned int* ticket) {
+  static_assert(M <= 2, "the batched factor fetch: block sizes 1 and 2");
+  extern __shared__ double2 sh_dict[];
+  double* const sh = reinterpret_cast<double*>(sh_dict);
+  __shared__ unsigned int s_ticket;
+  const int64_t c = A.c0 + blockIdx.x;
+  const int64_t col = blockIdx.y;
+  d0 += col * A.cs_d;
+  if (d0b) d0b += col * A.cs_d;
+  partR += col * A.cs_o;
+  partL += col * A.cs_o;
+  const bool wg_shared = ((c + 1) << A.q) <= A.lv[0].n - 1;
+  CR_TRACE_BEGIN();
+  CR_STAMP(A, 0);
+  cr_dict_fill(D, c, A.lds_total, sh);
+  __syncthreads();
+  CR_STAMP(A, 1);
+  const CrDictLds src{D, sh + D.tab_off, reinterpret_cast<const uint16_t*>(sh + D.idx_off), c};
+  cr_forward_steps<M>(A, c, wg_shared, d0, d0b, sh, src);
+  {
+    const double* R = sh + A.lds_off[A.nsteps];
+    if (threadIdx.x < M) {
+      const int os = A.ostride ? A.ostride : M;
+      partR[c * os + threadIdx.x] = R[threadIdx.x];
+      if (c + 1 <= A.n_out - 1) partL[(c + 1) * os + threadIdx.x] = R[2 * M + M + threadIdx.x];
+    }
+  }
+  if (A.stack) {
+    double* st = A.stack + col * A.cs_stack + c * (int64_t)A.stack_stride;
+    int o = 0;
+    for (int s = 1; s < A.nsteps; ++s) {
+      const int cnt = ((1 << (A.q - A.step_a[s])) + 1) * M;
+      const double* R = sh + A.lds_off[s];
+      for (int t = threadIdx.x; t < cnt; t += blockDim.x) st[o + t] = R[t] + R[cnt + t];
+      o += cnt;
+    }
+  }
+  CR_STAMP_WAIT(A, 15);
+  CR_TRACE_FLUSH(A);
+  if constexpr (FUSE_TAIL) {
+    __threadfence();
+    __syncthreads();
+    if (threadIdx.x == 0) s_ticket = atomicAdd(ticket, 1u);
+    __syncthreads();
+    if (s_ticket != gridDim.x - 1) return;
+    __threadfence();
+    cr_tail_body<M>(T, partR, partL, xq, sh);
+    if (threadIdx.x == 0) *ticket = 0u;
+  }
+}
+
+template <int M>
+__global__ __launch_bounds__(kCrThreads) CR_WAVES_ATTR void cr_stage_backward_dict_kernel(CrStageArgs A, CrDictArgs D,
+                                                                            const double* __restrict__ d0,
+                                                                            const double* __restrict__ d0b,
+                                                                            const double* __restrict__ xq,
+                                                                            double* __restrict__ x0) {
+  static_assert(M <= 2, "the batched factor fetch: block sizes 1 and 2");
+  extern __shared__ double2 sh_dict[];
+  double* const sh = reinterpret_cast<double*>(sh_dict);
+  const int64_t c = A.c0 + blockIdx.x;
+  const int64_t col = blockIdx.y;
+  d0 += col * A.cs_d;
+  if (d0b) d0b += col * A.cs_d;
+  xq += col * A.cs_xq;
+  x0 += col * A.cs_x;
+  const bool wg_shared = ((c + 1) << A.q) <= A.lv[0].n - 1;
+  CR_TRACE_BEGIN();
+  CR_STAMP(A, 0);
+  cr_dict_fill(D, c, A.lds_total, sh);
+  __syncthreads();
+  CR_STAMP(A, 1);
+  const CrDictLds src{D, sh + D.tab_off, reinterpret_cast<const uint16_t*>(sh + D.idx_off), c};
+  if (A.nsteps > 1) {
+    if (A.stack) {
+      const double* st = A.stack + col * A.cs_stack + c * (int64_t)A.stack_stride;
+      int o = 0;
+      for (int s = 1; s < A.nsteps; ++s) {
+        const int cnt = ((1 << (A.q - A.step_a[s])) + 1) * M;
+        double* R = sh + A.lds_off[s];
+        for (int t = threadIdx.x; t < cnt; t += blockDim.x) R[t] = st[o + t];
+        o += cnt;
+      }
+      __syncthreads();
+      CR_STAMP(A, 2);
+    } else {
+      cr_forward_steps<M>(A, c, wg_shared, d0, d0b, sh, src);
+    }
+  }
+  cr_backward_steps<M>(A, c, wg_shared, d0, d0b, xq, x0, sh, src);
+  CR_STAMP_WAIT(A, 15);
+  CR_TRACE_FLUSH(A);
+}
+
 constexpr int kPcrMaxLevels = 9;
 struct PcrArgs {
   const double* mult;
diff --git a/agglomerationmultigrid1d_amd/csrc/forms.hpp b/agglomerationmultigrid1d_amd/csrc/forms.hpp
--- a/agglomerationmultigrid1d_amd/csrc/forms.hpp
+++ b/agglomerationmultigrid1d_amd/csrc/forms.hpp
@@ -16,6 +16,7 @@
 constexpr bool chain_dict_form(int m) { return m == 1 || m == 2 || m == 4; }
 constexpr bool cr_form(int m) { return m >= 1 && m <= 8; }
 constexpr bool invert_form(int m) { return m >= 1 && m <= 8; }
+constexpr bool cr_dict_form(int m) { return m == 1 || m == 2; }
 constexpr bool csr_lanes_form(int l) { return l >= 1 && l <= 64 && (l & (l - 1)) == 0; }
 
 constexpr int col_group(int kc, int ceiling = 8) {
@@ -101,6 +102,7 @@
 static_assert(size_mask(chain_form) == 0b111111110 && size_mask(cr_form) == 0b111111110 && size_mask(invert_form) == 0b111111110,
               "chain_form, cr_form, invert_form: 1..8");
 static_assert(size_mask(chain_dict_form) == 0b10110 && count_bits(size_mask(chain_dict_form)) == 3, "chain_dict_form: 1, 2, 4");
+static_assert(size_mask(cr_dict_form) == 0b110, "cr_dict_form: 1, 2");
 static_assert(size_mask(is_col_group) == 0b100010110, "column groups: 1, 2, 4, 8");
 static_assert(col_group(1) == 1 && col_group(2) == 2 && col_group(3) == 4 && col_group(4) == 4 && col_group(5) == 8 && col_group(8) == 8 &&
                   col_group(3, 2) == 2 && col_group(8, 4) == 4 && col_group(3, 4) == 4,
diff --git a/agglomerationmultigrid1d_amd/csrc/host_plan.hpp b/agglomerationmultigrid1d_amd/csrc/host_plan.hpp
--- a/agglomerationmultigrid1d_amd/csrc/host_plan.hpp
+++ b/agglomerationmultigrid1d_amd/csrc/host_plan.hpp
@@ -147,6 +147,58 @@
   tail->mid = cr_even(cr_stage_buffers(tail_plan, m).mid);
   region(tail->mid, &tail->mid_off);
   return o;
+}
+
+constexpr int kCrDictMaxClasses = 56;
+constexpr int cr_dict_even_words(int m) { return 2 * m * m; }
+constexpr int cr_dict_odd_words(int m) { return (3 * m * m + (m + 1) / 2 + 1) & ~1; }
+constexpr int cr_dict_index_count(int q) { return ((2 << q) - 2 + q + 7) & ~7; }
+struct CrDictPlan {
+  bool take = false;
+  int tab_e[kCrMaxStageLevels] = {0}, tab_o[kCrMaxStageLevels] = {0};
+  int tab_words = 0;
+  int idx_e[kCrMaxStageLevels] = {0}, idx_o[kCrMaxStageLevels] = {0};
+  int idx_count = 0;
+  int tab_off = 0, idx_off = 0;
+  size_t lds_bytes = 0;
+};
+inline CrDictPlan cr_dict_plan(int m, int q, int lds_total, const int* n_even_cls, const int* n_odd_cls, int cap,
+                               size_t lds_limit = kCrLdsBudgetBytes) {
+  CrDictPlan P;
+  if (!cr_dict_form(m) || q < 1 || q > kCrMaxStageLevels || cap < 1) return P;
+  for (int l = 0; l < q; ++l)
+    if (n_even_cls[l] < 1 || n_even_cls[l] > cap || n_odd_cls[l] < 1 || n_odd_cls[l] > cap) return P;
+  int o = 0;
+  for (int l = 0; l < q; ++l) {
+    P.tab_e[l] = o;
+    o += n_even_cls[l] * cr_dict_even_words(m);
+    P.tab_o[l] = o;
+    o += n_odd_cls[l] * cr_dict_odd_words(m);
+  }
+  P.tab_words = o;
+  int i = 0;
+  for (int l = 0; l < q; ++l) {
+    P.idx_e[l] = i;
+    i += (1 << (q - l - 1)) + 1;
+    P.idx_o[l] = i;
+    i += 1 << (q - l - 1);
+  }
+  P.idx_count = (i + 7) & ~7;
+  P.tab_off = (lds_total + 1) & ~1;
+  P.idx_off = P.tab_off + P.tab_words;
+  P.lds_bytes = (size_t)P.idx_off * sizeof(double) + (size_t)P.idx_count * sizeof(uint16_t);
+  P.take = P.lds_bytes <= lds_limit;
+  return P;
+}
+inline void cr_dict_pack_odd(int m, int nc, const double* fo, const double* lu, const int32_t* perm, double* rec) {
+  const int mm = m * m, w = cr_dict_odd_words(m);
+  for (int c = 0; c < nc; ++c) {
+    double* r = rec + (size_t)c * w;
+    std::memset(r, 0, (size_t)w * sizeof(double));
+    std::memcpy(r, fo + (size_t)c * 2 * mm, (size_t)2 * mm * sizeof(double));
+    std::memcpy(r + 2 * mm, lu + (size_t)c * mm, (size_t)mm * sizeof(double));
+    std::memcpy(r + 3 * mm, perm + (size_t)c * m, (size_t)m * sizeof(int32_t));
+  }
 }
 
 inline std::vector<int32_t> stream_row_blocks(const int32_t* rowptr, int64_t nrows, int max_nnz, int max_rows) {
diff --git a/agglomerationmultigrid1d_amd/csrc/internal.hpp b/agglomerationmultigrid1d_amd/csrc/internal.hpp
--- a/agglomerationmultigrid1d_amd/csrc/internal.hpp
+++ b/agglomerationmultigrid1d_amd/csrc/internal.hpp
@@ -68,6 +68,8 @@
   int64_t pair_elem_launches = 0;
   int elem_rec_cap = [] { const char* e = std::getenv("AGGMG_ELEM_RECORDS_LDS"); return (e && e[0] == '0') ? 0 : kElemRecMaxClasses; }();
   int64_t elem_rec_launches = 0;
+  int coarse_dict_cap = [] { const char* e = std::getenv("AGGMG_COARSE_DICT"); return (e && e[0] == '0') ? 0 : kCrDictMaxClasses; }();
+  int64_t coarse_dict_launches = 0;
   bool replay_presmooth = [] { const char* e = std::getenv("AGGMG_REPLAY_PRESMOOTH"); return !(e && e[0] == '0'); }();
   int64_t replay_launches = 0;
   bool patch_multi = [] { const char* e = std::getenv("AGGMG_PATCH_MULTI"); return e && e[0] == '1'; }();
@@ -302,6 +304,9 @@
   double *partL = nullptr, *xq = nullptr;
   DevArray<double> stack;
   DevArray<double> mid;
+  CrDictPlan dict;
+  DevArray<double> dict_tab;
+  DevArray<uint16_t> dict_idx;
 };
 
 struct CrRunStage {
@@ -329,6 +334,7 @@
   const double* lu_last = nullptr;
   const int32_t* perm_last = nullptr;
   std::vector<CrStage> st;
+  std::vector<int> dict_even, dict_odd;
   CrStage tail;
   CrRun run;
   DevArray<double> d0, x0;
diff --git a/agglomerationmultigrid1d_amd/csrc/setup.hip b/agglomerationmultigrid1d_amd/csrc/setup.hip
--- a/agglomerationmultigrid1d_amd/csrc/setup.hip
+++ b/agglomerationmultigrid1d_amd/csrc/setup.hip
@@ -506,6 +506,17 @@
     };
     v.f[k] = DictField{full.get(), nullptr, n, (int)sizeof(T), back ? 1 : 0};
   }
+  template <typename T>
+  void add_view(const T* full, DevArray<T>* dict, int n) {
+    static_assert(sizeof(T) == 8 || sizeof(T) == 4, "records are made of 64- and 32-bit words");
+    const int k = v.nf++;
+    make[k] = [this, k, dict](aggmg_ctx* ctx, int64_t count) {
+      CHECK(dict->alloc(ctx, count));
+      v.f[k].dict = dict->get();
+      return (int)AGGMG_OK;
+    };
+    v.f[k] = DictField{full, nullptr, n, (int)sizeof(T), 0};
+  }
 };
 
 int dict_build(aggmg_ctx* ctx, DictFields& F, DevArray<uint16_t>* cls, int* nclasses) {
@@ -796,6 +807,73 @@
 
 void cr_discard(CrDev* c) { *c = CrDev(); }
 
+static int setup_cr_dictionary(aggmg_ctx* ctx, CrDev* cr) {
+  const int m = cr->m, cap = ctx->coarse_dict_cap, mm = m * m;
+  cr->dict_even.assign(cr->lv.size(), -1);
+  cr->dict_odd.assign(cr->lv.size(), -1);
+  if (!cr_dict_form(m) || cap < 1) return AGGMG_OK;
+  for (CrStage& S : cr->st) {
+    int ne[kCrMaxStageLevels] = {0}, no[kCrMaxStageLevels] = {0};
+    std::vector<DevArray<uint16_t>> ce(S.q), co(S.q);
+    std::vector<DevArray<double>> fe(S.q), fo(S.q), lu(S.q);
+    std::vector<DevArray<int32_t>> pm(S.q);
+    bool ok = true;
+    for (int l = 0; l < S.q && ok; ++l) {
+      const CrLevel& L = cr->lv[S.l0 + l];
+      ok = L.n_odd >= 1;
+      if (!ok) break;
+      DictFields E(L.n_even);
+      E.add_view(L.fe, &fe[l], 2 * mm);
+      CHECK(dict_build(ctx, E, &ce[l], &ne[l]));
+      cr->dict_even[S.l0 + l] = ne[l];
+      ok = ne[l] >= 1 && ne[l] <= cap;
+      if (!ok) break;
+      DictFields O(L.n_odd);
+      O.add_view(L.fo, &fo[l], 2 * mm);
+      O.add_view(L.lu, &lu[l], mm);
+      O.add_view(L.perm, &pm[l], m);
+      CHECK(dict_build(ctx, O, &co[l], &no[l]));
+      cr->dict_odd[S.l0 + l] = no[l];
+      ok = no[l] >= 1 && no[l] <= cap;
+    }
+    if (!ok) continue;
+    const CrDictPlan P = cr_dict_plan(m, S.q, S.lds_total, ne, no, cap);
+    if (!P.take) continue;
+    std::vector<double> tab((size_t)P.tab_words, 0.0);
+    std::vector<std::vector<double>> hfo(S.q), hlu(S.q);
+    std::vector<std::vector<int32_t>> hpm(S.q);
+    auto down = [&](void* dst, const void* src, size_t bytes) {
+      return hipMemcpyAsync(dst, src, bytes, hipMemcpyDeviceToHost, ctx->stream);
+    };
+    for (int l = 0; l < S.q; ++l) {
+      hfo[l].resize((size_t)no[l] * 2 * mm);
+      hlu[l].resize((size_t)no[l] * mm);
+      hpm[l].resize((size_t)no[l] * m);
+      HIPCHK(down(tab.data() + P.tab_e[l], fe[l].get(), (size_t)ne[l] * 2 * mm * sizeof(double)));
+      HIPCHK(down(hfo[l].data(), fo[l].get(), hfo[l].size() * sizeof(double)));
+      HIPCHK(down(hlu[l].data(), lu[l].get(), hlu[l].size() * sizeof(double)));
+      HIPCHK(down(hpm[l].data(), pm[l].get(), hpm[l].size() * sizeof(int32_t)));
+    }
+    HIPCHK(hipStreamSynchronize(ctx->stream));
+    for (int l = 0; l < S.q; ++l) cr_dict_pack_odd(m, no[l], hfo[l].data(), hlu[l].data(), hpm[l].data(), tab.data() + P.tab_o[l]);
+    CHECK(S.dict_tab.alloc(ctx, P.tab_words));
+    HIPCHK(hipMemcpyAsync(S.dict_tab, tab.data(), tab.size() * sizeof(double), hipMemcpyHostToDevice, ctx->stream));
+    const int64_t chunks = std::max<int64_t>(S.n_out, 1);
+    CHECK(S.dict_idx.alloc(ctx, chunks * P.idx_count, true));
+    for (int l = 0; l < S.q; ++l) {
+      const CrLevel& L = cr->lv[S.l0 + l];
+      const int shift = S.q - l - 1, cnt = 1 << shift;
+      LAUNCH(cr_dict_chunk_index_kernel, chunks * (cnt + 1), chunks, cnt + 1, shift, L.n_even, (const uint16_t*)ce[l],
+             S.dict_idx.get(), P.idx_count, P.idx_e[l]);
+      LAUNCH(cr_dict_chunk_index_kernel, chunks * cnt, chunks, cnt, shift, L.n_odd, (const uint16_t*)co[l], S.dict_idx.get(),
+             P.idx_count, P.idx_o[l]);
+    }
+    HIPCHK(hipStreamSynchronize(ctx->stream));
+    S.dict = P;
+  }
+  return AGGMG_OK;
+}
+
 __global__ __launch_bounds__(kSetupThreads) void probe_vector_kernel(int64_t n, double* __restrict__ w) {
   const int64_t i = (int64_t)blockIdx.x * kSetupThreads + threadIdx.x;
   if (i >= n) return;
@@ -1045,6 +1123,7 @@
   }
   CHECK(cr->ticket.alloc(ctx, 1, true));
   HIPCHK(hipStreamSynchronize(ctx->stream));
+  CHECK(setup_cr_dictionary(ctx, cr));
   cr->run = CrRun();
   for (const CrStage& S : cr->st) cr->run.st.push_back(cr_run_stage(S));
   cr->run.tail = cr_run_stage(cr->tail);
diff --git a/agglomerationmultigrid1d_amd/csrc/setup_kernels.hpp b/agglomerationmultigrid1d_amd/csrc/setup_kernels.hpp
--- a/agglomerationmultigrid1d_amd/csrc/setup_kernels.hpp
+++ b/agglomerationmultigrid1d_amd/csrc/setup_kernels.hpp
@@ -918,6 +918,18 @@
   }
 }
 
+__global__ __launch_bounds__(kSetupThreads) void cr_dict_chunk_index_kernel(int64_t n_chunks, int count, int shift,
+                                                                            int64_t n_rows, const uint16_t* __restrict__ cls,
+                                                                            uint16_t* __restrict__ out, int idx_count, int off) {
+  const int64_t i = (int64_t)blockIdx.x * kSetupThreads + threadIdx.x;
+  if (i >= n_chunks * count) return;
+  const int64_t c = i / count;
+  const int t = (int)(i - c * count);
+  int64_t g = (c << shift) + t;
+  if (g > n_rows - 1) g = n_rows - 1;
+  out[c * idx_count + off + t] = cls[g];
+}
+
 template <int M>
 __device__ __forceinline__ void lu_rowsolve_dev(const double (&F)[M][M], const int (&pm)[M], const double (&blk)[M][M],
                                                 double (&out)[M][M]) {
diff --git a/include/aggmg_hip.h b/include/aggmg_hip.h
--- a/include/aggmg_hip.h
+++ b/include/aggmg_hip.h
@@ -39,7 +39,10 @@
 #define AGGMG_OPT_CHAIN_MULTI 12
 #define AGGMG_OPT_ELEMENT_RECORDS_LDS 13
 #define AGGMG_OPT_PATCH_SCHWARZ_MULTI 14
+#define AGGMG_OPT_COARSE_DICTIONARY (15)
 int aggmg_set_option(aggmg_ctx* ctx, int option, int value);
+int aggmg_coarse_dictionary_launches(aggmg_ctx* ctx, int64_t* count);
+int aggmg_coarse_dictionary_cap(aggmg_ctx* ctx, int* cap, int* max_cap);
 int aggmg_element_record_lds_launches(aggmg_ctx* ctx, int64_t* count);
 int aggmg_element_record_lds_cap(aggmg_ctx* ctx, int* cap, int* max_cap);
 int aggmg_element_record_pack(int nclasses, const double* bsym, const double* qrow, const double* qmir, const double* dup,
@@ -183,6 +186,8 @@
                                  int* npost);
 int aggmg_hier_estimate_lambda_max(aggmg_ctx* ctx, aggmg_hier* h, int level, const double* v0, int iters,
                                    double* lambda_max);
+int aggmg_hier_coarse_dictionary(aggmg_ctx* ctx, const aggmg_hier* h, int capacity, int* nstages, int* taken,
+                                 int* first_level, int* nlevels, int* even_classes, int* odd_classes);
 int aggmg_hier_coarse_info(aggmg_ctx* ctx, const aggmg_hier* h, int* on_device, int* block_size,
                            double* cond_est);
 int aggmg_hier_coarse_probe(aggmg_ctx* ctx, const aggmg_hier* h, double* backward_error);
```

Result: faster. 542.1 billion DoF-updates/s (median of 6 runs) (+4.0%).
